# acappemin/Video-to-Audio-and-Piano-RP

Measured on AMD Instinct MI355X. Metric: mel-frames/sec (10s VGGSound shape, 32-step CFM, CFG 2.0), higher is better.
Workload: dtype bf16x3; 1 GPU; BASELINE.json configs[1]: 1 clip(s)/GPU x 750 latent frames x 128 ch, 32-point sway grid = 31 CFG evaluations (62 DiT forwards), T5 context 16 tokens, V2A zero roll; clips_per_gpu=1, global_clips=1, parallelism=clip-sharded x1, 1 all-gather, hipgraph=True, schedule=three streams, side_streams=True, cascade_passes=1

## Files before the change

include/v2a_cfm.h:

```cpp
#ifndef V2A_CFM_H
#define V2A_CFM_H

#include <stdint.h>

#ifdef __cplusplus
extern "C" {
#endif

typedef void* v2a_stream_t;

enum {
  V2A_F32 = 0,
  V2A_BF16 = 1,
  V2A_BF16_SPLIT = 2
};

enum {
  V2A_OK = 0,
  V2A_ERR_ARG = -1,
  V2A_ERR_LAUNCH = -2
};

int v2a_abi_version(void);
const char* v2a_last_error(void);

enum {
  V2A_EPI_STORE = 0,
  V2A_EPI_SIGMOID = 1,
  V2A_EPI_GEGLU = 2,
  V2A_EPI_RESID = 3,
  V2A_EPI_GATE_RESID = 4,
  V2A_EPI_GEGLU_TANH = 5,
  V2A_EPI_GELU = 6,
  V2A_EPI_SWIGLU = 7
};

typedef struct v2a_gemm_args {
  const void* a[3];
  int64_t lda[3];
  int32_t ka[3];
  int32_t nseg;
  int32_t a_dtype;
  const void* w;
  int64_t ldw;
  const float* bias;
  int32_t M, N;
  int32_t compute_dtype;
  int32_t epilogue;
  void* out;
  int64_t ldo;
  int32_t out_dtype;
  void* out_bf16;
  int64_t ld_out_bf16;
  const float* resid;
  int64_t ldr;
  const float* gate;
  const int32_t* step;
  int64_t gate_step_stride, gate_batch_stride;
  int32_t rows_per_batch;
  const float* rope_table;
  int32_t rope_cols, rope_pos_offset;
  int32_t relu;
  const int32_t* a_row_offset;
  const int32_t* a_ktile_offset;
  const int32_t* out_row_offset;
  int32_t tile_hint;
  const float* norm_gamma;
  int64_t norm_step_stride, norm_batch_stride;
  int32_t norm_switch_row, norm_switch_offset;
  float* norm_ssq;
  int64_t ld_norm_ssq;
  const float* row_ssq;
  int64_t ld_row_ssq;
  int32_t row_ssq_parts, row_norm_dim;
  int32_t out_bf16_split;
  int64_t a_lo_offset[3];
  int64_t out_bf16_lo_offset;
} v2a_gemm_args;

int v2a_gemm(const v2a_gemm_args* args, v2a_stream_t stream);
int v2a_gemm_args_size(void);

enum { V2A_GEMM_REGISTER_STAGED = 0, V2A_GEMM_RING = 1, V2A_GEMM_8PHASE = 2 };
typedef struct v2a_gemm_choice {
  int32_t family;
  int32_t split;
  int32_t bm, bn, bk;
  int32_t waves_m, waves_n;
  int32_t stages;
  int32_t tiles;
  int32_t xcd_gm, xcd_gn;
  int32_t vec_epi;
} v2a_gemm_choice;
int v2a_gemm_choose(const v2a_gemm_args* args, v2a_gemm_choice* choice);

typedef struct v2a_tuning {
  int32_t gemm_force_tile;
  int32_t gemm_k_rotation;
  int32_t gemm_8phase;
  int32_t gemm_8phase_min_tiles;
  int32_t dwconv_rows_per_wave;
  int32_t gemm_xcd_order_1x8;
  int32_t attn_one_group_from;
  int32_t reserved[1];
} v2a_tuning;
int v2a_set_tuning(const v2a_tuning* tuning);

int v2a_rmsnorm(const float* x, int64_t ldx, void* y, int64_t ldy, int32_t y_dtype,
                int64_t rows, int32_t d,
                const float* gamma, const int32_t* step, int64_t gamma_step_stride,
                int64_t gamma_batch_stride, int32_t rows_per_batch, v2a_stream_t stream);

int v2a_dwconv_silu_residual(const float* x, float* out, const float* wt, const float* bias,
                             int32_t B, int32_t N, int32_t d, int32_t ksize,
                             const int32_t* len, v2a_stream_t stream);
typedef struct v2a_dwconv_norm {
  void* out_bf16;
  int64_t ld_out_bf16;
  const float* norm_gamma;
  const int32_t* step;
  int64_t norm_step_stride, norm_batch_stride;
  float* norm_ssq;
  int64_t ld_norm_ssq;
  int32_t split;
  int32_t reserved;
} v2a_dwconv_norm;
int v2a_dwconv_silu_residual_norm(const float* x, float* out, const float* wt, const float* bias,
                                  int32_t B, int32_t N, int32_t d, int32_t ksize,
                                  const int32_t* len, const v2a_dwconv_norm* norm, v2a_stream_t stream);

int v2a_rope_inplace(void* qk, int32_t dtype, int64_t rows, int64_t row_stride, int32_t nheads,
                     int32_t rows_per_batch, int32_t pos_offset, const float* cs_table,
                     int32_t layout, v2a_stream_t stream);

typedef struct v2a_attn_args {
  const void *q, *k, *v, *gate;
  void* out;
  int64_t q_row_stride, k_row_stride, v_row_stride, gate_row_stride, out_row_stride;
  int64_t q_batch_stride, k_batch_stride, v_batch_stride, gate_batch_stride, out_batch_stride;
  int32_t B, H, Nq, Nk;
  const int32_t* kv_len;
  const int32_t* q_len;
  float scale, softclamp;
  int32_t dtype;
  int32_t out_split;
} v2a_attn_args;

int v2a_attention(const v2a_attn_args* args, v2a_stream_t stream);
int v2a_qproj_xattn(const v2a_gemm_args* gemm, const v2a_attn_args* attn, v2a_stream_t stream);

typedef struct v2a_xattn_prepare_args {
  const float* ctx_kv;
  int64_t ctx_ld;
  int32_t k_col, v_col;
  const float* wq;
  const float* wo;
  void* wqk;
  void* wvo;
  int32_t B, L, H, D, nc, KP;
} v2a_xattn_prepare_args;
int v2a_xattn_absorb_prepare(const v2a_xattn_prepare_args* args, v2a_stream_t stream);

typedef struct v2a_xattn_absorbed_args {
  const void* a;
  int64_t lda;
  int32_t K, M;
  const void* wqk;
  int64_t ldw, w_batch_stride;
  const float* gate_bias;
  void* out;
  int64_t ldo;
  int32_t rows_per_batch, B, H, KP;
  const int32_t* kv_len;
  const int32_t* q_len;
  float scale, softclamp;
  const float* row_ssq;
  int64_t ld_row_ssq;
  int32_t row_ssq_parts, row_norm_dim;
} v2a_xattn_absorbed_args;
int v2a_xattn_absorbed(const v2a_xattn_absorbed_args* args, v2a_stream_t stream);

int v2a_linear_small(const float* a, int64_t M, int32_t K, const float* wt, const float* bias,
                     const float* add, int32_t T, float* out, int64_t out_batch_stride,
                     int32_t row_off, int32_t d, int32_t dup_batch_offset,
                     const float* regs ,
                     void* out_bf16 , v2a_stream_t stream);

int v2a_fill_registers(float* out, int64_t out_batch_stride, const float* regs, int32_t B,
                       int32_t R, int32_t d, v2a_stream_t stream);

int v2a_time_cond(const float* t, int32_t S, const float* fourier_w, const float* wt,
                  const float* bias, float* out, int32_t d, v2a_stream_t stream);

int v2a_apg_reduce(const float* pred, double* apg, int32_t B, int32_t T, int32_t C,
                   int64_t pred_batch_stride, int32_t row_off,
                   const int32_t* valid_rows ,
                   v2a_stream_t stream);
int v2a_cfg_euler(float* y, const float* pred, int32_t B, int32_t T, int32_t C,
                  int64_t pred_batch_stride, int32_t row_off, float cfg_strength,
                  const float* dt, const int32_t* step, const double* apg,
                  float keep_parallel_frac, v2a_stream_t stream);
int v2a_split_bf16(const float* x, int64_t ldx, void* y, int64_t ldy, int64_t rows, int32_t d, v2a_stream_t stream);
int v2a_cast_bf16(const float* x, void* y, int64_t n, v2a_stream_t stream);
int v2a_step_advance(int32_t* step, v2a_stream_t stream);


int v2a_im2col(const float* x, int32_t B, int32_t H, int32_t W, int32_t C, int32_t kh, int32_t kw, int32_t stride,
               int32_t pad, int32_t Ho, int32_t Wo, void* col, int64_t ldo, int32_t out_dtype, int32_t window_t,
               int32_t window_first, v2a_stream_t stream);

int v2a_frames_pack(const float* frames, void* out, int32_t T, int32_t H, int32_t W, int32_t kw, int32_t stride, int32_t pad,
                    int32_t Wo, v2a_stream_t stream);
int v2a_frames_pack_split(const float* frames, void* out, int64_t lo_offset, int32_t T, int32_t H, int32_t W, int32_t kw,
                          int32_t stride, int32_t pad, int32_t Wo, v2a_stream_t stream);

int v2a_pool2d(const float* x, float* out, void* out_bf16, int32_t B, int32_t H, int32_t W, int32_t C, int32_t k,
               int32_t stride, int32_t pad, int32_t mode, int32_t Ho, int32_t Wo, int32_t in_border, int32_t out_border,
               v2a_stream_t stream);
int v2a_pool2d_split(const float* x, float* out, void* out_split, int64_t lo_offset, int32_t B, int32_t H, int32_t W, int32_t C,
                     int32_t k, int32_t stride, int32_t pad, int32_t mode, int32_t Ho, int32_t Wo, int32_t in_border,
                     int32_t out_border, v2a_stream_t stream);

typedef struct v2a_roll_head_args {
  const float *x2, *x3, *x4, *x5;
  int32_t B, P;
  const float *frb4_w1t, *frb4_b1, *frb4_w2t, *frb4_b2;
  const float *frb3_w1t, *frb3_b1, *frb3_w2t, *frb3_b2;
  const float *frb2_w1t, *frb2_b1, *frb2_w2t, *frb2_b2;
  const float *conv2_wt, *conv2_b;
  const float *fc_wt, *fc_b;
  int32_t notes;
  int32_t apply_sigmoid;
  float* out;
} v2a_roll_head_args;
int v2a_roll_head(const v2a_roll_head_args* args, v2a_stream_t stream);

int v2a_roll_expand(const float* roll, float* out, int32_t B, int32_t t, int32_t notes, int32_t rep, int32_t l,
                    v2a_stream_t stream);

int v2a_roll_expand_ratio(const float* roll, float* out, int32_t B, int32_t t, int32_t notes, int32_t rep, int32_t group, int32_t l,
                          v2a_stream_t stream);


int v2a_elu_pad(const float* x, float* out, int64_t T, int32_t C, int32_t pad, int32_t reflect, int32_t act,
                v2a_stream_t stream);

int v2a_lstm_layer(const float* gates_x, const float* w_hh, float* h, const float* resid, float* y, int32_t T, int32_t H,
                   int32_t* workspace, v2a_stream_t stream);

int v2a_lstm2(const float* gates_x0, const float* w_hh0, const float* w_ih1, const float* bias1, const float* w_hh1,
              const float* resid, float* y, int32_t T, int32_t H, int32_t* workspace, v2a_stream_t stream);


int v2a_elu_pad_lr(const float* x, float* out, int64_t T, int32_t C, int32_t pad_left, int32_t pad_right, int32_t act,
                   v2a_stream_t stream);

int v2a_encodec_stage0(const float* wave, const float* params, float* out, int64_t n, v2a_stream_t stream);


int v2a_t5_rmsnorm(const float* x, int64_t ldx, const int32_t* ids, int32_t vocab, float* resid, int64_t ldr, float* y, int64_t ldy,
                   int64_t rows, int32_t d, const float* w, float eps, v2a_stream_t stream);

typedef struct v2a_t5_attn_args {
  const float *q, *k, *v;
  float* out;
  int64_t q_row_stride, k_row_stride, v_row_stride, out_row_stride;
  int64_t q_batch_stride, k_batch_stride, v_batch_stride, out_batch_stride;
  int32_t B, H, N, d_kv;
  const float* bias;
  const int32_t* key_mask;
} v2a_t5_attn_args;
int v2a_t5_attention(const v2a_t5_attn_args* args, v2a_stream_t stream);

int v2a_gemm_skinny_f32(const v2a_gemm_args* args, v2a_stream_t stream);


int v2a_clip_resize_h(const uint8_t* frames, int32_t F, int32_t H, int32_t W, uint8_t* tmp, int32_t y0, int32_t rows, int32_t S,
                      const int32_t* bounds, const int32_t* coef, int32_t ksize, v2a_stream_t stream);
int v2a_clip_resize_v(const uint8_t* tmp, int32_t F, int32_t rows, int32_t S, int32_t P, const int32_t* bounds, const int32_t* coef,
                      int32_t ksize, const float* lut, void* patches, int64_t ldp, int32_t out_dtype, int64_t lo_offset, uint8_t* crop,
                      v2a_stream_t stream);
int v2a_clip_embed_init(float* h, int64_t ldh, int64_t rows, int32_t T, int32_t d, const float* cls, const float* pos,
                        v2a_stream_t stream);
int v2a_clip_layernorm(const float* x, int64_t ldx, void* y, int64_t ldy, int32_t y_dtype, int64_t rows, int32_t d, const float* gamma,
                       const float* beta, float eps, v2a_stream_t stream);
typedef struct v2a_clip_attn_args {
  const float *q, *k, *v;
  void* out;
  int64_t row_stride, batch_stride;
  int64_t out_row_stride, out_batch_stride;
  int32_t B, H, N, d_head;
  float scale;
  int32_t out_split;
} v2a_clip_attn_args;
int v2a_clip_attention(const v2a_clip_attn_args* args, v2a_stream_t stream);


int v2a_piano_resize_h(const uint8_t* frames, int32_t F, int32_t H, int32_t W, const int32_t* sel, int32_t n, uint8_t* tmp, int32_t ldt,
                       int32_t y0, int32_t rows, int32_t Wo, const int32_t* bounds, const int32_t* coef, int32_t ksize,
                       v2a_stream_t stream);
int v2a_piano_resize_v(const uint8_t* tmp, int32_t n, int32_t rows, int32_t ldt, int32_t Ho, int32_t Wo, const int32_t* bounds,
                       const int32_t* coef, int32_t ksize, const float* lut, float* out, v2a_stream_t stream);
int v2a_piano_resize_vt(const uint8_t* tmp, int32_t n, int32_t rows, int32_t ldt, int32_t Ho, int32_t Wo, const int32_t* bounds,
                        const int32_t* coef, int32_t ksize, const float* lut, float* out, v2a_stream_t stream);


int v2a_encodec_rvq_encode(const float* x, int64_t batch_stride, int64_t frame_stride, int64_t chan_stride, int32_t B, int32_t T,
                           const float* codebooks, const float* norms, int32_t S, int32_t Kc, int32_t D, int32_t n_q, int64_t* codes,
                           v2a_stream_t stream);
int v2a_encodec_rvq_decode(const int64_t* codes, int32_t n_q, int32_t B, int32_t T, const float* codebooks, int32_t S, int32_t Kc, int32_t D,
                           float* out, int64_t batch_stride, int64_t frame_stride, int64_t chan_stride, v2a_stream_t stream);


#define V2A_LOSS_MAX_PARTS 256

int v2a_cfm_interp(const float* x0, const float* x1, const float* t, const uint8_t* span, float* w, float* flow, float* cond, int32_t B,
                   int32_t T, int32_t C, v2a_stream_t stream);
int v2a_masked_sqerr(const float* pred, const float* target, const uint8_t* mask, int32_t B, int32_t T, int32_t C, double* scratch,
                     double* out, v2a_stream_t stream);
int v2a_roll_metrics(const float* roll, const float* midis, const uint8_t* mask, int32_t B, int32_t T, int32_t notes, double* scratch,
                     double* out, v2a_stream_t stream);


#define V2A_WAVE_MAX_PARTS 256
#define V2A_WAVE_LDS_BYTES (128 * 1024)
#define V2A_WAVE_TABLE_MAX (1 << 22)

int v2a_wave_resample(const float* x, int64_t L, const float* table, int32_t o, int32_t n, int32_t K, int32_t width, float* y,
                      int64_t out_len, void* parts, int32_t* n_parts, v2a_stream_t stream);
int v2a_wave_stats(const float* x, int64_t n, void* parts, int32_t* n_parts, v2a_stream_t stream);
int v2a_wave_normalize(const float* x, int64_t n, const void* parts, int32_t n_parts, float* out, int64_t n_out, float* stats,
                       v2a_stream_t stream);


int v2a_roll2midi_stem(const float* x, const float* wt, int32_t n, int32_t H, int32_t W, int32_t co, float* out, void* shadow,
                       int32_t shadow_mode, int64_t lo_offset, int64_t pitch, int32_t border, v2a_stream_t stream);
int v2a_leaky_shadow(float* x, void* shadow, int32_t shadow_mode, int64_t lo_offset, int32_t n, int32_t H, int32_t W, int32_t C,
                     int64_t pitch, int32_t border, v2a_stream_t stream);
int v2a_roll2midi_head(const float* u, int64_t u_pitch, int32_t nu, const float* d, int64_t d_pitch, int32_t nd, const float* w,
                       float bias, float threshold, int32_t n, int32_t H, int32_t W, int32_t border, float* logits, float* probs,
                       uint8_t* midi, v2a_stream_t stream);
int v2a_roll2midi_gate(float* x0, int64_t pitch0, int32_t C0, void* shadow0, int64_t lo_offset0, float* x1, int64_t pitch1, int32_t C1,
                       void* shadow1, int64_t lo_offset1, const float* w, float bias, int32_t shadow_mode, int32_t n, int32_t H, int32_t W,
                       int32_t border, float* logits, float* alpha, v2a_stream_t stream);


#define V2A_ROLL_NOTES_MAX_KEYS 128
#define V2A_ROLL_NOTES_TILE 256
#define V2A_ROLL_NOTES_MAX_FRAMES (1 << 24)

int v2a_roll_notes(const void* roll, int32_t elem_bytes, int64_t batch_stride, int64_t frame_stride, int64_t key_stride, float threshold,
                   int32_t B, int32_t T, int32_t keys, const int32_t* lens, int32_t* counts, int32_t* totals, int32_t* notes, int32_t cap,
                   int8_t* onset, v2a_stream_t stream);

#ifdef __cplusplus
}
#endif
#endif
```

video-to-audio-and-piano-rp_amd/_lib.py:

```python
from __future__ import annotations

import ctypes as C
import os
import subprocess
from typing import NamedTuple

import torch

_HERE = os.path.dirname(os.path.abspath(__file__))
LIB_PATH = os.path.join(_HERE, "libv2a_cfm.so")
CSRC = os.path.join(_HERE, "csrc")

F32, BF16, BF16_SPLIT = 0, 1, 2
EPI_STORE, EPI_SIGMOID, EPI_GEGLU, EPI_RESID, EPI_GATE_RESID = 0, 1, 2, 3, 4
EPI_GEGLU_TANH = 5
EPI_GELU = 6
EPI_SWIGLU = 7

_lib = None


class V2AError(RuntimeError):
    pass


class GemmArgs(C.Structure):
    _fields_ = [
        ("a", C.c_void_p * 3), ("lda", C.c_int64 * 3), ("ka", C.c_int32 * 3),
        ("nseg", C.c_int32), ("a_dtype", C.c_int32),
        ("w", C.c_void_p), ("ldw", C.c_int64), ("bias", C.c_void_p),
        ("M", C.c_int32), ("N", C.c_int32), ("compute_dtype", C.c_int32), ("epilogue", C.c_int32),
        ("out", C.c_void_p), ("ldo", C.c_int64), ("out_dtype", C.c_int32),
        ("out_bf16", C.c_void_p), ("ld_out_bf16", C.c_int64),
        ("resid", C.c_void_p), ("ldr", C.c_int64),
        ("gate", C.c_void_p), ("step", C.c_void_p),
        ("gate_step_stride", C.c_int64), ("gate_batch_stride", C.c_int64), ("rows_per_batch", C.c_int32),
        ("rope_table", C.c_void_p), ("rope_cols", C.c_int32), ("rope_pos_offset", C.c_int32), ("relu", C.c_int32),
        ("a_row_offset", C.c_void_p), ("a_ktile_offset", C.c_void_p), ("out_row_offset", C.c_void_p),
        ("tile_hint", C.c_int32),
        ("norm_gamma", C.c_void_p), ("norm_step_stride", C.c_int64), ("norm_batch_stride", C.c_int64),
        ("norm_switch_row", C.c_int32), ("norm_switch_offset", C.c_int32),
        ("norm_ssq", C.c_void_p), ("ld_norm_ssq", C.c_int64),
        ("row_ssq", C.c_void_p), ("ld_row_ssq", C.c_int64), ("row_ssq_parts", C.c_int32), ("row_norm_dim", C.c_int32),
        ("out_bf16_split", C.c_int32),
        ("a_lo_offset", C.c_int64 * 3), ("out_bf16_lo_offset", C.c_int64),
    ]


class GemmChoice(C.Structure):
    _fields_ = [(n, C.c_int32) for n in ("family", "split", "bm", "bn", "bk", "waves_m", "waves_n", "stages", "tiles", "xcd_gm", "xcd_gn",
                                         "vec_epi")]


GEMM_REGISTER_STAGED, GEMM_RING, GEMM_8PHASE = 0, 1, 2

TILE_128x128, TILE_8PHASE, TILE_128x128_8WAVES, TILE_128x64_8WAVES = 1, 6, 12, 14
SPLIT_TILE_8PHASE, SPLIT_TILE_128x256_K32 = 5, 6


class DwconvNorm(C.Structure):
    _fields_ = [("out_bf16", C.c_void_p), ("ld_out_bf16", C.c_int64), ("norm_gamma", C.c_void_p), ("step", C.c_void_p),
                ("norm_step_stride", C.c_int64), ("norm_batch_stride", C.c_int64), ("norm_ssq", C.c_void_p), ("ld_norm_ssq", C.c_int64),
                ("split", C.c_int32), ("reserved", C.c_int32)]


class Tuning(C.Structure):
    _fields_ = [("gemm_force_tile", C.c_int32), ("gemm_k_rotation", C.c_int32), ("gemm_8phase", C.c_int32),
                ("gemm_8phase_min_tiles", C.c_int32), ("dwconv_rows_per_wave", C.c_int32), ("gemm_xcd_order_1x8", C.c_int32),
                ("attn_one_group_from", C.c_int32), ("reserved", C.c_int32 * 1)]


class AttnArgs(C.Structure):
    _fields_ = [
        ("q", C.c_void_p), ("k", C.c_void_p), ("v", C.c_void_p), ("gate", C.c_void_p), ("out", C.c_void_p),
        ("q_row_stride", C.c_int64), ("k_row_stride", C.c_int64), ("v_row_stride", C.c_int64),
        ("gate_row_stride", C.c_int64), ("out_row_stride", C.c_int64),
        ("q_batch_stride", C.c_int64), ("k_batch_stride", C.c_int64), ("v_batch_stride", C.c_int64),
        ("gate_batch_stride", C.c_int64), ("out_batch_stride", C.c_int64),
        ("B", C.c_int32), ("H", C.c_int32), ("Nq", C.c_int32), ("Nk", C.c_int32),
        ("kv_len", C.c_void_p), ("q_len", C.c_void_p),
        ("scale", C.c_float), ("softclamp", C.c_float), ("dtype", C.c_int32), ("out_split", C.c_int32),
    ]


class XattnPrepareArgs(C.Structure):
    _fields_ = [("ctx_kv", C.c_void_p), ("ctx_ld", C.c_int64), ("k_col", C.c_int32), ("v_col", C.c_int32),
                ("wq", C.c_void_p), ("wo", C.c_void_p), ("wqk", C.c_void_p), ("wvo", C.c_void_p)] + \
               [(n, C.c_int32) for n in ("B", "L", "H", "D", "nc", "KP")]


class XattnAbsorbedArgs(C.Structure):
    _fields_ = [("a", C.c_void_p), ("lda", C.c_int64), ("K", C.c_int32), ("M", C.c_int32),
                ("wqk", C.c_void_p), ("ldw", C.c_int64), ("w_batch_stride", C.c_int64), ("gate_bias", C.c_void_p),
                ("out", C.c_void_p), ("ldo", C.c_int64),
                ("rows_per_batch", C.c_int32), ("B", C.c_int32), ("H", C.c_int32), ("KP", C.c_int32),
                ("kv_len", C.c_void_p), ("q_len", C.c_void_p), ("scale", C.c_float), ("softclamp", C.c_float),
                ("row_ssq", C.c_void_p), ("ld_row_ssq", C.c_int64), ("row_ssq_parts", C.c_int32), ("row_norm_dim", C.c_int32)]


class T5AttnArgs(C.Structure):
    _fields_ = [
        ("q", C.c_void_p), ("k", C.c_void_p), ("v", C.c_void_p), ("out", C.c_void_p),
        ("q_row_stride", C.c_int64), ("k_row_stride", C.c_int64), ("v_row_stride", C.c_int64), ("out_row_stride", C.c_int64),
        ("q_batch_stride", C.c_int64), ("k_batch_stride", C.c_int64), ("v_batch_stride", C.c_int64), ("out_batch_stride", C.c_int64),
        ("B", C.c_int32), ("H", C.c_int32), ("N", C.c_int32), ("d_kv", C.c_int32),
        ("bias", C.c_void_p), ("key_mask", C.c_void_p),
    ]


class ClipAttnArgs(C.Structure):
    _fields_ = [("q", C.c_void_p), ("k", C.c_void_p), ("v", C.c_void_p), ("out", C.c_void_p),
                ("row_stride", C.c_int64), ("batch_stride", C.c_int64), ("out_row_stride", C.c_int64), ("out_batch_stride", C.c_int64),
                ("B", C.c_int32), ("H", C.c_int32), ("N", C.c_int32), ("d_head", C.c_int32), ("scale", C.c_float), ("out_split", C.c_int32)]


class RollHeadArgs(C.Structure):
    _fields_ = ([(n, C.c_void_p) for n in ("x2", "x3", "x4", "x5")] + [("B", C.c_int32), ("P", C.c_int32)] +
                [(f"frb{i}_{n}", C.c_void_p) for i in (4, 3, 2) for n in ("w1t", "b1", "w2t", "b2")] +
                [(n, C.c_void_p) for n in ("conv2_wt", "conv2_b", "fc_wt", "fc_b")] +
                [("notes", C.c_int32), ("apply_sigmoid", C.c_int32), ("out", C.c_void_p)])


EXPORTS = [
    "v2a_abi_version", "v2a_last_error", "v2a_gemm", "v2a_gemm_args_size", "v2a_gemm_choose", "v2a_set_tuning", "v2a_rmsnorm", "v2a_dwconv_silu_residual", "v2a_dwconv_silu_residual_norm",
    "v2a_rope_inplace", "v2a_attention", "v2a_qproj_xattn", "v2a_linear_small", "v2a_fill_registers", "v2a_time_cond",
    "v2a_apg_reduce", "v2a_cfg_euler", "v2a_step_advance", "v2a_cast_bf16", "v2a_split_bf16",
    "v2a_im2col", "v2a_frames_pack", "v2a_pool2d", "v2a_roll_head", "v2a_roll_expand", "v2a_frames_pack_split", "v2a_pool2d_split",
    "v2a_elu_pad", "v2a_lstm_layer", "v2a_lstm2", "v2a_t5_rmsnorm", "v2a_t5_attention", "v2a_gemm_skinny_f32",
    "v2a_clip_resize_h", "v2a_clip_resize_v", "v2a_clip_embed_init", "v2a_clip_layernorm", "v2a_clip_attention",
    "v2a_elu_pad_lr", "v2a_encodec_stage0", "v2a_piano_resize_h", "v2a_piano_resize_v",
    "v2a_encodec_rvq_encode", "v2a_encodec_rvq_decode", "v2a_cfm_interp", "v2a_masked_sqerr", "v2a_roll_metrics",
    "v2a_wave_resample", "v2a_wave_stats", "v2a_wave_normalize",
    "v2a_roll2midi_stem", "v2a_leaky_shadow", "v2a_roll2midi_head", "v2a_roll2midi_gate",
    "v2a_xattn_absorb_prepare", "v2a_xattn_absorbed",
    "v2a_roll_expand_ratio", "v2a_piano_resize_vt",
    "v2a_roll_notes",
]


def build(force: bool = False, verbose: bool = False) -> str:
    if force:
        for f in os.listdir(os.path.join(CSRC, "build")) if os.path.isdir(os.path.join(CSRC, "build")) else []:
            os.remove(os.path.join(CSRC, "build", f))
    r = subprocess.run(["bash", os.path.join(CSRC, "build.sh")], capture_output=True, text=True)
    if verbose or r.returncode != 0:
        print(r.stdout[-4000:])
        print(r.stderr[-8000:])
    if r.returncode != 0:
        raise V2AError("hipcc build of libv2a_cfm.so failed")
    return LIB_PATH


ABI_VERSION = 9


def _declare(lib):
    vp, i32, i64, f32 = C.c_void_p, C.c_int32, C.c_int64, C.c_float
    lib.v2a_abi_version.restype = C.c_int
    lib.v2a_last_error.restype = C.c_char_p
    lib.v2a_gemm.argtypes = [C.POINTER(GemmArgs), vp]
    lib.v2a_gemm_args_size.restype = C.c_int
    lib.v2a_gemm_choose.argtypes = [C.POINTER(GemmArgs), C.POINTER(GemmChoice)]
    lib.v2a_set_tuning.argtypes = [C.POINTER(Tuning)]
    lib.v2a_attention.argtypes = [C.POINTER(AttnArgs), vp]
    lib.v2a_qproj_xattn.argtypes = [C.POINTER(GemmArgs), C.POINTER(AttnArgs), vp]
    lib.v2a_xattn_absorb_prepare.argtypes = [C.POINTER(XattnPrepareArgs), vp]
    lib.v2a_xattn_absorbed.argtypes = [C.POINTER(XattnAbsorbedArgs), vp]
    lib.v2a_rmsnorm.argtypes = [vp, i64, vp, i64, i32, i64, i32, vp, vp, i64, i64, i32, vp]
    lib.v2a_dwconv_silu_residual.argtypes = [vp, vp, vp, vp, i32, i32, i32, i32, vp, vp]
    lib.v2a_dwconv_silu_residual_norm.argtypes = [vp, vp, vp, vp, i32, i32, i32, i32, vp, C.POINTER(DwconvNorm), vp]
    lib.v2a_rope_inplace.argtypes = [vp, i32, i64, i64, i32, i32, i32, vp, i32, vp]
    lib.v2a_linear_small.argtypes = [vp, i64, i32, vp, vp, vp, i32, vp, i64, i32, i32, i32, vp, vp, vp]
    lib.v2a_fill_registers.argtypes = [vp, i64, vp, i32, i32, i32, vp]
    lib.v2a_time_cond.argtypes = [vp, i32, vp, vp, vp, vp, i32, vp]
    lib.v2a_apg_reduce.argtypes = [vp, vp, i32, i32, i32, i64, i32, vp, vp]
    lib.v2a_cfg_euler.argtypes = [vp, vp, i32, i32, i32, i64, i32, f32, vp, vp, vp, f32, vp]
    lib.v2a_step_advance.argtypes = [vp, vp]
    lib.v2a_cast_bf16.argtypes = [vp, vp, i64, vp]
    lib.v2a_split_bf16.argtypes = [vp, i64, vp, i64, i64, i32, vp]
    lib.v2a_im2col.argtypes = [vp, i32, i32, i32, i32, i32, i32, i32, i32, i32, i32, vp, i64, i32, i32, i32, vp]
    lib.v2a_frames_pack.argtypes = [vp, vp, i32, i32, i32, i32, i32, i32, i32, vp]
    lib.v2a_pool2d.argtypes = [vp, vp, vp, i32, i32, i32, i32, i32, i32, i32, i32, i32, i32, i32, i32, vp]
    lib.v2a_frames_pack_split.argtypes = [vp, vp, i64, i32, i32, i32, i32, i32, i32, i32, vp]
    lib.v2a_pool2d_split.argtypes = [vp, vp, vp, i64, i32, i32, i32, i32, i32, i32, i32, i32, i32, i32, i32, i32, vp]
    lib.v2a_roll_head.argtypes = [C.POINTER(RollHeadArgs), vp]
    lib.v2a_roll_expand.argtypes = [vp, vp, i32, i32, i32, i32, i32, vp]
    lib.v2a_roll_expand_ratio.argtypes = [vp, vp, i32, i32, i32, i32, i32, i32, vp]
    lib.v2a_elu_pad.argtypes = [vp, vp, i64, i32, i32, i32, i32, vp]
    lib.v2a_lstm_layer.argtypes = [vp, vp, vp, vp, vp, i32, i32, vp, vp]
    lib.v2a_lstm2.argtypes = [vp, vp, vp, vp, vp, vp, vp, i32, i32, vp, vp]
    lib.v2a_t5_rmsnorm.argtypes = [vp, i64, vp, i32, vp, i64, vp, i64, i64, i32, vp, f32, vp]
    lib.v2a_t5_attention.argtypes = [C.POINTER(T5AttnArgs), vp]
    lib.v2a_gemm_skinny_f32.argtypes = [C.POINTER(GemmArgs), vp]
    lib.v2a_clip_resize_h.argtypes = [vp, i32, i32, i32, vp, i32, i32, i32, vp, vp, i32, vp]
    lib.v2a_clip_resize_v.argtypes = [vp, i32, i32, i32, i32, vp, vp, i32, vp, vp, i64, i32, i64, vp, vp]
    lib.v2a_clip_embed_init.argtypes = [vp, i64, i64, i32, i32, vp, vp, vp]
    lib.v2a_clip_layernorm.argtypes = [vp, i64, vp, i64, i32, i64, i32, vp, vp, f32, vp]
    lib.v2a_clip_attention.argtypes = [C.POINTER(ClipAttnArgs), vp]
    lib.v2a_elu_pad_lr.argtypes = [vp, vp, i64, i32, i32, i32, i32, vp]
    lib.v2a_encodec_stage0.argtypes = [vp, vp, vp, i64, vp]
    lib.v2a_piano_resize_h.argtypes = [vp, i32, i32, i32, vp, i32, vp, i32, i32, i32, i32, vp, vp, i32, vp]
    lib.v2a_piano_resize_v.argtypes = [vp, i32, i32, i32, i32, i32, vp, vp, i32, vp, vp, vp]
    lib.v2a_piano_resize_vt.argtypes = lib.v2a_piano_resize_v.argtypes
    lib.v2a_encodec_rvq_encode.argtypes = [vp, i64, i64, i64, i32, i32, vp, vp, i32, i32, i32, i32, vp, vp]
    lib.v2a_encodec_rvq_decode.argtypes = [vp, i32, i32, i32, vp, i32, i32, i32, vp, i64, i64, i64, vp]
    lib.v2a_cfm_interp.argtypes = [vp, vp, vp, vp, vp, vp, vp, i32, i32, i32, vp]
    lib.v2a_masked_sqerr.argtypes = [vp, vp, vp, i32, i32, i32, vp, vp, vp]
    lib.v2a_roll_metrics.argtypes = [vp, vp, vp, i32, i32, i32, vp, vp, vp]
    lib.v2a_wave_resample.argtypes = [vp, i64, vp, i32, i32, i32, i32, vp, i64, vp, C.POINTER(i32), vp]
    lib.v2a_wave_stats.argtypes = [vp, i64, vp, C.POINTER(i32), vp]
    lib.v2a_wave_normalize.argtypes = [vp, i64, vp, i32, vp, i64, vp, vp]
    lib.v2a_roll2midi_stem.argtypes = [vp, vp, i32, i32, i32, i32, vp, vp, i32, i64, i64, i32, vp]
    lib.v2a_leaky_shadow.argtypes = [vp, vp, i32, i64, i32, i32, i32, i32, i64, i32, vp]
    lib.v2a_roll2midi_head.argtypes = [vp, i64, i32, vp, i64, i32, vp, f32, f32, i32, i32, i32, i32, vp, vp, vp, vp]
    lib.v2a_roll2midi_gate.argtypes = [vp, i64, i32, vp, i64, vp, i64, i32, vp, i64, vp, f32, i32, i32, i32, i32, i32, vp, vp, vp]
    lib.v2a_roll_notes.argtypes = [vp, i32, i64, i64, i64, f32, i32, i32, i32, vp, vp, vp, vp, i32, vp, vp]
    for name in EXPORTS:
        if name not in ("v2a_abi_version", "v2a_last_error", "v2a_gemm_args_size"):
            getattr(lib, name).restype = C.c_int


def lib():
    global _lib
    if _lib is None:
        if not os.path.exists(LIB_PATH):
            raise V2AError(f"{LIB_PATH} is missing: run `python -c 'import __graft_entry__ as g; g.build()'` "
                           "(hipcc --offload-arch=gfx950).  There is no CPU fallback for the sampler.")
        _lib = C.CDLL(LIB_PATH)
        _declare(_lib)
        if _lib.v2a_abi_version() != ABI_VERSION:
            raise V2AError("libv2a_cfm.so reports ABI version %d, this binding was written for %d: rebuild (csrc/build.sh)"
                           % (_lib.v2a_abi_version(), ABI_VERSION))
        if _lib.v2a_gemm_args_size() != C.sizeof(GemmArgs):
            raise V2AError("libv2a_cfm.so was built with sizeof(v2a_gemm_args) = %d, this binding mirrors %d bytes: rebuild "
                           "(csrc/build.sh)" % (_lib.v2a_gemm_args_size(), C.sizeof(GemmArgs)))
    return _lib


def set_tuning(force_tile: int = -1, k_rotation: bool = False, eight_phase: int | None = None, eight_phase_min_tiles: int = 0,
               dwconv_rows_per_wave: int = 0, xcd_order_1x8: bool = False, attn_one_group_from: int = 0, reserved: int = 0):
    if (force_tile == -1 and not k_rotation and eight_phase is None and eight_phase_min_tiles == 0 and dwconv_rows_per_wave == 0
            and not xcd_order_1x8 and attn_one_group_from == 0 and not reserved):
        check(lib().v2a_set_tuning(None))
        return
    t = Tuning(force_tile, 1 if k_rotation else 0, 1 if eight_phase is None else eight_phase, eight_phase_min_tiles, dwconv_rows_per_wave,
               1 if xcd_order_1x8 else 0, attn_one_group_from, (C.c_int32 * 1)(reserved))
    check(lib().v2a_set_tuning(C.byref(t)))


def check(rc: int):
    if rc != 0:
        raise V2AError(f"v2a_cfm call failed ({rc}): {lib().v2a_last_error().decode()}")


def stream_ptr() -> int:
    return torch.cuda.current_stream().cuda_stream


def dt_code(t: torch.dtype) -> int:
    if t == torch.float32:
        return F32
    if t == torch.bfloat16:
        return BF16
    raise V2AError(f"unsupported dtype {t}")


def _p(t):
    return 0 if t is None else t.data_ptr()


class Operand(NamedTuple):
    t: torch.Tensor
    ld: int
    k: int
    lo: int = 0


def split_planes(w):
    w = w.float()
    hi = w.bfloat16()
    return torch.cat([hi, (w - hi.float()).bfloat16()], 1)


_prof = None


class KernelProfiler:

    def __init__(self, shapes: bool = False, inner: int = 1, external: bool = False):
        self.recs = []
        self.shapes = shapes
        self.inner = inner
        self.external = external
        self.marks, self.end, self.tot = [], None, {}

    def launch(self, key, flops, nbytes, call):
        if self.external:
            e = torch.cuda.Event(enable_timing=True, external=True)
            e.record()
            self.marks.append((key, flops, nbytes, e))
            call()
            return
        n = self.inner if key.startswith("gemm") else 1
        s, e = torch.cuda.Event(enable_timing=True), torch.cuda.Event(enable_timing=True)
        s.record()
        for _ in range(n):
            call()
        e.record()
        self.recs.append((key, flops, nbytes, s, e, n))

    def close(self):
        self.end = torch.cuda.Event(enable_timing=True, external=True)
        self.end.record()

    def collect(self):
        for i, (key, flops, nbytes, e) in enumerate(self.marks):
            nxt = self.marks[i + 1][3] if i + 1 < len(self.marks) else self.end
            a = self.tot.setdefault(key, dict(launches=0, ms=0.0, flops=0.0, bytes=0.0))
            a["launches"] += 1
            a["ms"] += e.elapsed_time(nxt)
            a["flops"] += flops
            a["bytes"] += nbytes

    def summary(self):
        torch.cuda.synchronize()
        if self.external:
            return self.tot
        agg = {}
        for key, flops, nbytes, s, e, n in self.recs:
            a = agg.setdefault(key, dict(launches=0, ms=0.0, flops=0.0, bytes=0.0))
            a["launches"] += 1
            a["ms"] += s.elapsed_time(e) / n
            a["flops"] += flops
            a["bytes"] += nbytes
        return agg


def set_profiler(p):
    global _prof
    _prof = p


def _launch(key, flops, nbytes, call):
    if _prof is None:
        check(call())
    else:
        _prof.launch(key, flops, nbytes, lambda: check(call()))


_EPI_NAMES = {0: "store", 1: "sigmoid", 2: "geglu", 3: "resid", 4: "gate_resid", 5: "geglu_tanh", 6: "gelu", 7: "swiglu"}



def gemm(a_segs, w, out, **kw):
    g, key, flops, nbytes = gemm_args(a_segs, w, out, **kw)
    _launch(key, flops, nbytes, lambda: lib().v2a_gemm(C.byref(g), stream_ptr()))


def gemm_choice(a_segs, w, out, **kw) -> GemmChoice:
    c = GemmChoice()
    check(lib().v2a_gemm_choose(C.byref(gemm_args(a_segs, w, out, **kw)[0]), C.byref(c)))
    return c


def gemm_args(a_segs, w, out, *, M, N, compute, epilogue=EPI_STORE, bias=None, resid=None, gate=None,
         step=None, gate_step_stride=0, gate_batch_stride=0, rows_per_batch=0, ldo=None, ldr=None,
         out_bf16=None, ld_out_bf16=None, rope_table=None, rope_cols=0, rope_pos_offset=0, relu=False,
         a_row_offset=None, a_ktile_offset=None, out_row_offset=None, tile_hint=0,
         norm_gamma=None, norm_step_stride=0, norm_batch_stride=0, norm_switch_row=0, norm_switch_offset=0, norm_ssq=None,
         row_ssq=None, row_norm_dim=0, out_bf16_split=False, a_split=False, out_split=False, out_bf16_lo_offset=0):
    g = GemmArgs()
    a_segs = [Operand(*seg) for seg in a_segs]
    for i, s in enumerate(a_segs):
        g.a[i], g.lda[i], g.ka[i], g.a_lo_offset[i] = s.t.data_ptr(), s.ld, s.k, s.lo
    g.nseg = len(a_segs)
    g.a_dtype = BF16_SPLIT if a_split else dt_code(a_segs[0].t.dtype)
    g.w = w.data_ptr()
    g.ldw = w.stride(0)
    g.bias = _p(bias)
    g.M, g.N = M, N
    g.compute_dtype = compute
    g.epilogue = epilogue
    g.out = out.data_ptr()
    g.ldo = ldo if ldo is not None else out.stride(-2)
    g.out_dtype = BF16_SPLIT if out_split else dt_code(out.dtype)
    g.out_bf16 = _p(out_bf16)
    g.ld_out_bf16 = (ld_out_bf16 if ld_out_bf16 is not None else g.ldo) if out_bf16 is not None else 0
    g.resid = _p(resid)
    g.ldr = (ldr if ldr is not None else (resid.stride(-2) if resid is not None else 0))
    g.gate = _p(gate)
    g.step = _p(step)
    g.gate_step_stride = gate_step_stride
    g.gate_batch_stride = gate_batch_stride
    g.rows_per_batch = rows_per_batch
    g.rope_table = _p(rope_table)
    g.rope_cols, g.rope_pos_offset = rope_cols, rope_pos_offset
    g.relu = 1 if relu else 0
    g.a_row_offset, g.a_ktile_offset, g.out_row_offset = _p(a_row_offset), _p(a_ktile_offset), _p(out_row_offset)
    g.tile_hint = tile_hint if compute == BF16 and g.a_dtype in (BF16, BF16_SPLIT) and epilogue != EPI_SIGMOID else 0
    g.norm_gamma = _p(norm_gamma)
    g.norm_step_stride, g.norm_batch_stride = norm_step_stride, norm_batch_stride
    g.norm_switch_row, g.norm_switch_offset = norm_switch_row, norm_switch_offset
    g.norm_ssq = _p(norm_ssq)
    g.ld_norm_ssq = norm_ssq.stride(-2) if norm_ssq is not None else 0
    g.row_ssq = _p(row_ssq)
    g.ld_row_ssq = row_ssq.stride(-2) if row_ssq is not None else 0
    g.row_ssq_parts = row_norm_dim // 32 if row_ssq is not None else 0
    g.row_norm_dim = row_norm_dim
    g.out_bf16_split = 1 if out_bf16_split else 0
    g.out_bf16_lo_offset = out_bf16_lo_offset
    K = sum(s.k for s in a_segs)
    key = "gemm<%s,%s,%s,%s>" % ("bf16" if compute == BF16 else "f32", "a_f32" if g.a_dtype == F32 else ("a_split" if a_split else "a_bf16"),
                                 _EPI_NAMES[epilogue], "f32" if g.out_dtype == F32 else "bf16")
    esz = 2 if compute == BF16 else 4
    nbytes = M * K * (4 if g.a_dtype == F32 else 2) + N * K * esz + M * (N // 2 if epilogue in (EPI_GEGLU, EPI_SWIGLU) else N) * out.element_size()
    nbytes += (M * N * 4 if resid is not None else 0) + (M * N * 2 if out_bf16 is not None else 0)
    if g.tile_hint:
        key = key[:-1] + ",tile%d>" % (g.tile_hint - 1)
    if _prof is not None and _prof.shapes:
        key += " %dx%dx%d" % (M, N, K)
    return g, key, (6.0 if a_split else 2.0) * M * N * K, nbytes * (2 if a_split else 1)


def rmsnorm(x, y, *, rows, d, gamma, step=None, gamma_step_stride=0, gamma_batch_stride=0, rows_per_batch=0,
            ldx=None, ldy=None, split=False):
    ydt = BF16_SPLIT if split else dt_code(y.dtype)
    if split:
        ldy = ldy or 2 * d
    _launch("rmsnorm<%s>" % ("f32" if y.dtype == torch.float32 else ("bf16x2" if split else "bf16")), 0.0,
            rows * d * (4 + y.element_size() * (2 if split else 1)),
            lambda: lib().v2a_rmsnorm(x.data_ptr(), ldx or d, y.data_ptr(), ldy or d, ydt, rows, d,
                                      gamma.data_ptr(), _p(step), gamma_step_stride, gamma_batch_stride, rows_per_batch,
                                      stream_ptr()))


def _dwconv_norm(norm, d):
    n = DwconvNorm()
    n.out_bf16, n.ld_out_bf16 = norm["out_bf16"].data_ptr(), norm.get("ld_out_bf16", d)
    n.norm_gamma, n.step = norm["gamma"].data_ptr(), _p(norm.get("step"))
    n.norm_step_stride, n.norm_batch_stride = norm.get("step_stride", 0), norm.get("batch_stride", 0)
    n.norm_ssq, n.ld_norm_ssq = norm["ssq"].data_ptr(), norm["ssq"].stride(-2)
    n.split = 1 if norm.get("split") else 0
    if n.split:
        n.ld_out_bf16 = norm.get("ld_out_bf16", 2 * d)
    return n


def dwconv(x, out, wt, bias, *, B, N, d, ksize, lens=None, norm=None):
    if norm is None:
        _launch("dwconv", 2.0 * B * N * d * ksize, B * N * d * 8,
                lambda: lib().v2a_dwconv_silu_residual(x.data_ptr(), out.data_ptr(), wt.data_ptr(), bias.data_ptr(),
                                                       B, N, d, ksize, _p(lens), stream_ptr()))
        return
    n = _dwconv_norm(norm, d)
    _launch("dwconv+norm", 2.0 * B * N * d * ksize, B * N * d * (12 if n.split else 10),
            lambda: lib().v2a_dwconv_silu_residual_norm(x.data_ptr(), out.data_ptr(), wt.data_ptr(), bias.data_ptr(),
                                                        B, N, d, ksize, _p(lens), C.byref(n), stream_ptr()))


def rope(qk, *, rows, row_stride, nheads, rows_per_batch, pos_offset, table, layout):
    _launch("rope<%s>" % ("f32" if qk.dtype == torch.float32 else "bf16"), 0.0, rows * nheads * 64 * 2 * qk.element_size(),
            lambda: lib().v2a_rope_inplace(qk.data_ptr(), dt_code(qk.dtype), rows, row_stride, nheads, rows_per_batch,
                                           pos_offset, table.data_ptr(), layout, stream_ptr()))


def attention(q, k, v, gate, out, **kw):
    a, key, flops, nbytes = attention_args(q, k, v, gate, out, **kw)
    _launch(key, flops, nbytes, lambda: lib().v2a_attention(C.byref(a), stream_ptr()))


def attention_args(q, k, v, gate, out, *, strides, B, H, Nq, Nk, kv_len=None, q_len=None, scale, softclamp, dtype, out_split=False):
    a = AttnArgs()
    a.q, a.k, a.v, a.gate, a.out = q, k, v, gate, out
    (a.q_row_stride, a.k_row_stride, a.v_row_stride, a.gate_row_stride, a.out_row_stride,
     a.q_batch_stride, a.k_batch_stride, a.v_batch_stride, a.gate_batch_stride, a.out_batch_stride) = strides
    a.B, a.H, a.Nq, a.Nk = B, H, Nq, Nk
    a.kv_len, a.q_len = _p(kv_len), _p(q_len)
    a.scale, a.softclamp, a.dtype = scale, softclamp, dtype
    a.out_split = 1 if out_split else 0
    esz = 2 if dtype == BF16 else 4
    return a, "attention<%s>" % {BF16: "bf16", F32: "f32", BF16_SPLIT: "bf16x3"}[dtype], 4.0 * B * H * Nq * Nk * 64, B * H * 64 * (2 * Nq + 2 * Nk) * esz


def qproj_xattn(a, lda, K, w, *, bias, M, N, rows_per_batch, k, v, out, kv_strides, out_strides, B, H, Nk, kv_len=None, q_len=None,
                scale, softclamp, rope_table=None, rope_cols=0, rope_pos_offset=0, row_ssq=None, row_norm_dim=0, split=False):
    g = GemmArgs()
    g.a[0], g.lda[0], g.ka[0], g.nseg = a.data_ptr(), lda, K, 1
    g.compute_dtype = BF16
    g.a_dtype = BF16_SPLIT if split else BF16
    g.w, g.ldw = w.data_ptr(), w.stride(0)
    g.bias = _p(bias)
    g.M, g.N = M, N
    g.epilogue = EPI_STORE
    g.out_dtype = F32 if split else BF16
    g.rows_per_batch = rows_per_batch
    g.rope_table = _p(rope_table)
    g.rope_cols, g.rope_pos_offset = rope_cols, rope_pos_offset
    g.row_ssq = _p(row_ssq)
    g.ld_row_ssq = row_ssq.stride(-2) if row_ssq is not None else 0
    g.row_ssq_parts = row_norm_dim // 32 if row_ssq is not None else 0
    g.row_norm_dim = row_norm_dim
    t = AttnArgs()
    t.k, t.v, t.out = k, v, out
    t.k_row_stride, t.v_row_stride, t.k_batch_stride, t.v_batch_stride = kv_strides
    t.out_row_stride, t.out_batch_stride = out_strides
    t.B, t.H, t.Nq, t.Nk = B, H, rows_per_batch, Nk
    t.kv_len, t.q_len = _p(kv_len), _p(q_len)
    t.scale, t.softclamp, t.dtype = scale, softclamp, (BF16_SPLIT if split else BF16)
    t.out_split = 1 if split else 0
    _launch("qproj_xattn<%s>" % ("bf16x3" if split else "bf16"), (3.0 if split else 1.0) * (2.0 * M * (H * 65) * K + 4.0 * B * H * rows_per_batch * Nk * 64),
            M * K * 2 + H * 65 * K * 2 + M * H * 64 * 2 + 2 * B * Nk * H * 64 * 2,
            lambda: lib().v2a_qproj_xattn(C.byref(g), C.byref(t), stream_ptr()))


def xattn_kp(nc):
    return 16 if nc <= 16 else 32


def xattn_absorb_prepare(ctx_kv, wq, wo, wqk, wvo, *, B, L, H, D, nc, KP, k_col, v_col):
    a = XattnPrepareArgs()
    a.ctx_kv, a.ctx_ld, a.k_col, a.v_col = ctx_kv.data_ptr(), ctx_kv.stride(-2), k_col, v_col
    a.wq, a.wo, a.wqk, a.wvo = wq.data_ptr(), wo.data_ptr(), wqk.data_ptr(), wvo.data_ptr()
    a.B, a.L, a.H, a.D, a.nc, a.KP = B, L, H, D, nc, KP
    _launch("xattn_absorb_prepare", 4.0 * B * L * H * KP * 64 * D,
            L * (2 * H * 64 + H) * D * 4 + B * L * ((H * KP + H) * D + D * H * KP) * 4 + 2 * B * nc * L * H * 64 * 4,
            lambda: lib().v2a_xattn_absorb_prepare(C.byref(a), stream_ptr()))


def xattn_absorbed(a, lda, K, wqk, out, *, ldw, w_batch_stride, ldo, M, rows_per_batch, B, H, KP, kv_len, q_len=None, gate_bias=None,
                   scale, softclamp, row_ssq=None, row_norm_dim=0):
    g = XattnAbsorbedArgs()
    g.a, g.lda, g.K, g.M = a.data_ptr(), lda, K, M
    g.wqk, g.ldw, g.w_batch_stride, g.gate_bias = wqk.data_ptr(), ldw, w_batch_stride, _p(gate_bias)
    g.out, g.ldo = out.data_ptr(), ldo
    g.rows_per_batch, g.B, g.H, g.KP = rows_per_batch, B, H, KP
    g.kv_len, g.q_len = _p(kv_len), _p(q_len)
    g.scale, g.softclamp = scale, softclamp
    g.row_ssq = _p(row_ssq)
    g.ld_row_ssq = row_ssq.stride(-2) if row_ssq is not None else 0
    g.row_ssq_parts = row_norm_dim // 32 if row_ssq is not None else 0
    g.row_norm_dim = row_norm_dim
    n = H * KP + H
    _launch("xattn_absorbed<bf16x3>", 6.0 * M * n * K, (M * K + B * n * K + M * H * KP) * 4,
            lambda: lib().v2a_xattn_absorbed(C.byref(g), stream_ptr()))


def linear_small(a, wt, bias, add, out, *, M, K, T, out_batch_stride, row_off, d, dup=0, regs=None, out_bf16=None):
    _launch("linear_small", 2.0 * M * K * d, M * (K + d) * 4,
            lambda: lib().v2a_linear_small(a.data_ptr(), M, K, wt.data_ptr(), _p(bias), _p(add), T, out.data_ptr(),
                                           out_batch_stride, row_off, d, dup, _p(regs), _p(out_bf16), stream_ptr()))


def fill_registers(out, regs, *, B, R, d, out_batch_stride):
    check(lib().v2a_fill_registers(out.data_ptr(), out_batch_stride, regs.data_ptr(), B, R, d, stream_ptr()))


def time_cond(t, fourier_w, wt, bias, out, *, S, d):
    check(lib().v2a_time_cond(t.data_ptr(), S, fourier_w.data_ptr(), wt.data_ptr(), bias.data_ptr(),
                              out.data_ptr(), d, stream_ptr()))


def apg_reduce(pred, apg, *, B, T, C_, pred_batch_stride, row_off, valid_rows=None):
    check(lib().v2a_apg_reduce(pred.data_ptr(), apg.data_ptr(), B, T, C_, pred_batch_stride, row_off, _p(valid_rows), stream_ptr()))


def cfg_euler(y, pred, *, B, T, C_, pred_batch_stride, row_off, cfg_strength, dt, step=None, apg=None, keep=0.0):
    _launch("cfg_euler", 0.0, 16.0 * B * T * C_,
            lambda: lib().v2a_cfg_euler(y.data_ptr(), pred.data_ptr(), B, T, C_, pred_batch_stride, row_off,
                                        float(cfg_strength), dt.data_ptr(), _p(step), _p(apg), float(keep), stream_ptr()))


def step_advance(step):
    check(lib().v2a_step_advance(step.data_ptr(), stream_ptr()))


def split_bf16(x, y, *, rows, d, ldx=None, ldy=None):
    _launch("split_bf16", 0.0, rows * d * 8, lambda: lib().v2a_split_bf16(x.data_ptr(), ldx or d, y.data_ptr(), ldy or 2 * d, rows, d, stream_ptr()))


def cast_bf16(x, y):
    _launch("cast_bf16", 0.0, x.numel() * 6, lambda: lib().v2a_cast_bf16(x.data_ptr(), y.data_ptr(), x.numel(), stream_ptr()))


def im2col(x, col, *, B, H, W, C_, kh, kw, stride, pad, Ho, Wo, ldo, window_t=0, window_first=0):
    K = kh * kw * C_
    _launch("im2col<%s>" % ("f32" if col.dtype == torch.float32 else "bf16"), 0.0, B * Ho * Wo * (4.0 * K + col.element_size() * ldo),
            lambda: lib().v2a_im2col(x.data_ptr(), B, H, W, C_, kh, kw, stride, pad, Ho, Wo, col.data_ptr(), ldo,
                                     dt_code(col.dtype), window_t, window_first, stream_ptr()))


def frames_pack(frames, out, *, T, H, W, kw, stride, pad, Wo):
    _launch("frames_pack", 0.0, 4.0 * T * H * W + 32.0 * (T + 4) * Wo * (H + 2 * pad),
            lambda: lib().v2a_frames_pack(frames.data_ptr(), out.data_ptr(), T, H, W, kw, stride, pad, Wo, stream_ptr()))


def frames_pack_split(frames, out, *, lo_offset, T, H, W, kw, stride, pad, Wo):
    _launch("frames_pack_split", 0.0, 4.0 * T * H * W + 64.0 * (T + 4) * Wo * (H + 2 * pad),
            lambda: lib().v2a_frames_pack_split(frames.data_ptr(), out.data_ptr(), lo_offset, T, H, W, kw, stride, pad, Wo, stream_ptr()))


def pool2d(x, out, *, B, H, W, C_, k, stride, pad, mode, Ho, Wo, out_bf16=None, in_border=0, out_border=0):
    _launch("pool2d", 0.0, 4.0 * B * C_ * (H * W + Ho * Wo),
            lambda: lib().v2a_pool2d(x.data_ptr(), out.data_ptr(), _p(out_bf16), B, H, W, C_, k, stride, pad, mode, Ho, Wo,
                                     in_border, out_border, stream_ptr()))


def pool2d_split(x, out, out_split, *, lo_offset, B, H, W, C_, k, stride, pad, mode, Ho, Wo, in_border=0, out_border=0):
    _launch("pool2d_split", 0.0, 4.0 * B * C_ * (H * W + 2 * Ho * Wo),
            lambda: lib().v2a_pool2d_split(x.data_ptr(), out.data_ptr(), out_split.data_ptr(), lo_offset, B, H, W, C_, k, stride, pad,
                                           mode, Ho, Wo, in_border, out_border, stream_ptr()))


def roll_head(args: "RollHeadArgs"):
    _launch("roll_head", 0.0, 4.0 * args.B * args.P * (3 * 128 + 64), lambda: lib().v2a_roll_head(C.byref(args), stream_ptr()))


def roll_expand(roll, out, *, B, t, notes, rep, l):
    check(lib().v2a_roll_expand(roll.data_ptr(), out.data_ptr(), B, t, notes, rep, l, stream_ptr()))


def roll_expand_ratio(roll, out, *, B, t, notes, rep, group, l):
    check(lib().v2a_roll_expand_ratio(roll.data_ptr(), out.data_ptr(), B, t, notes, rep, group, l, stream_ptr()))


SH_NONE, SH_BF16, SH_SPLIT = 0, 1, 2


def roll2midi_stem(x, wt, out, shadow, *, n, H, W, co, shadow_mode, lo_offset, pitch, border):
    _launch("roll2midi_stem", 18.0 * n * H * W * co, n * H * W * (4.0 + co * (4 + 2 * shadow_mode)),
            lambda: lib().v2a_roll2midi_stem(x.data_ptr(), wt.data_ptr(), n, H, W, co, out.data_ptr(), _p(shadow), shadow_mode, lo_offset,
                                             pitch, border, stream_ptr()))


def leaky_shadow(x, shadow, *, n, H, W, C_, shadow_mode, lo_offset, pitch, border):
    _launch("leaky_shadow", 0.0, n * H * W * C_ * (8.0 + 2 * shadow_mode),
            lambda: lib().v2a_leaky_shadow(x.data_ptr(), _p(shadow), shadow_mode, lo_offset, n, H, W, C_, pitch, border, stream_ptr()))


def roll2midi_head(u, d, w, *, u_pitch, nu, d_pitch, nd, bias, threshold, n, H, W, border, logits=None, probs=None, midi=None):
    _launch("roll2midi_head", 2.0 * n * H * W * (nu + nd), n * H * W * (4.0 * (nu + nd) + 9),
            lambda: lib().v2a_roll2midi_head(u.data_ptr(), u_pitch, nu, d.data_ptr(), d_pitch, nd, w.data_ptr(), float(bias), float(threshold),
                                             n, H, W, border, _p(logits), _p(probs), _p(midi), stream_ptr()))


def roll2midi_gate(seg0, seg1, w, *, bias, shadow_mode, n, H, W, border, logits=None, alpha=None):
    x0, p0, c0, s0, l0 = seg0
    x1, p1, c1, s1, l1 = seg1 if seg1 is not None else (None, 0, 0, None, 0)
    _launch("roll2midi_gate", 2.0 * n * H * W * (c0 + c1), n * H * W * (c0 + c1) * (8.0 + 2 * shadow_mode) + 4.0 * (c0 + c1),
            lambda: lib().v2a_roll2midi_gate(x0.data_ptr(), p0, c0, _p(s0), l0, _p(x1), p1, c1, _p(s1), l1, w.data_ptr(), float(bias),
                                             shadow_mode, n, H, W, border, _p(logits), _p(alpha), stream_ptr()))


ROLL_NOTES_MAX_KEYS, ROLL_NOTES_TILE, ROLL_NOTES_MAX_FRAMES = 128, 256, 1 << 24


def roll_notes(roll, counts, totals, notes, *, strides, B, T, keys, cap, threshold=0.0, lens=None, onset=None):
    _launch("roll_notes<%s>" % ("f32" if roll.dtype == torch.float32 else "u8"), 0.0, 2.0 * B * T * keys * roll.element_size(),
            lambda: lib().v2a_roll_notes(roll.data_ptr(), roll.element_size(), strides[0], strides[1], strides[2], float(threshold), B, T, keys,
                                         _p(lens), counts.data_ptr(), totals.data_ptr(), _p(notes), cap, _p(onset), stream_ptr()))


def elu_pad(x, out, *, T, C_, pad, reflect, act=True):
    _launch("elu_pad", 0.0, 4.0 * C_ * (2 * T + pad),
            lambda: lib().v2a_elu_pad(x.data_ptr(), out.data_ptr(), T, C_, pad, 1 if reflect else 0, 1 if act else 0, stream_ptr()))


def elu_pad_lr(x, out, *, T, C_, pad_left, pad_right, act=True):
    _launch("elu_pad_lr", 0.0, 4.0 * C_ * (2 * T + pad_left + pad_right),
            lambda: lib().v2a_elu_pad_lr(x.data_ptr(), out.data_ptr(), T, C_, pad_left, pad_right, 1 if act else 0, stream_ptr()))


ENCODEC_STAGE0_PARAMS = 3376


def encodec_stage0(wave, params, out, *, n):
    _launch("encodec_stage0", 2.0 * n * 3744, 4.0 * n * 33,
            lambda: lib().v2a_encodec_stage0(wave.data_ptr(), params.data_ptr(), out.data_ptr(), n, stream_ptr()))


def encodec_rvq_encode(x, strides, codebooks, norms, codes, *, B, T, n_q):
    S, Kc, D = codebooks.shape
    _launch("encodec_rvq_encode", 2.0 * B * T * n_q * Kc * D, 4.0 * (B * T * D + n_q * Kc * D * -(-B * T // 16)) + 8.0 * n_q * B * T,
            lambda: lib().v2a_encodec_rvq_encode(x.data_ptr(), strides[0], strides[1], strides[2], B, T, codebooks.data_ptr(), norms.data_ptr(),
                                                 S, Kc, D, n_q, codes.data_ptr(), stream_ptr()))


def encodec_rvq_decode(codes, codebooks, out, strides, *, B, T, n_q):
    S, Kc, D = codebooks.shape
    _launch("encodec_rvq_decode", 1.0 * B * T * n_q * D, B * T * (4.0 * D * (n_q + 1) + 8.0 * n_q),
            lambda: lib().v2a_encodec_rvq_decode(codes.data_ptr(), n_q, B, T, codebooks.data_ptr(), S, Kc, D, out.data_ptr(),
                                                 strides[0], strides[1], strides[2], stream_ptr()))


LOSS_MAX_PARTS = 256


def cfm_interp(x0, x1, t, span, w, flow, cond=None):
    B, T, C_ = x1.shape
    _launch("cfm_interp", 4.0 * B * T * C_, 4.0 * B * T * C_ * (4 if cond is None else 5),
            lambda: lib().v2a_cfm_interp(x0.data_ptr(), x1.data_ptr(), t.data_ptr(), _p(span), w.data_ptr(), flow.data_ptr(), _p(cond),
                                         B, T, C_, stream_ptr()))


def masked_sqerr(pred, target, mask, out):
    B, T, C_ = pred.shape
    scratch = torch.empty(LOSS_MAX_PARTS * 2, dtype=torch.float64, device=pred.device)
    _launch("masked_sqerr", 3.0 * B * T * C_, 8.0 * B * T * C_,
            lambda: lib().v2a_masked_sqerr(pred.data_ptr(), target.data_ptr(), mask.data_ptr(), B, T, C_, scratch.data_ptr(), out.data_ptr(),
                                           stream_ptr()))


def roll_metrics(roll, midis, mask, out):
    B, T, notes = roll.shape
    scratch = torch.empty(LOSS_MAX_PARTS * 6, dtype=torch.float64, device=roll.device)
    _launch("roll_metrics", 5.0 * B * T * notes, 16.0 * B * T * notes,
            lambda: lib().v2a_roll_metrics(roll.data_ptr(), midis.data_ptr(), mask.data_ptr(), B, T, notes, scratch.data_ptr(), out.data_ptr(),
                                           stream_ptr()))


def lstm_layer(gates_x, w_hh, h, workspace, *, T, H, resid=None, y=None):
    _launch("lstm_layer", 2.0 * T * 4 * H * H, 4.0 * T * 6 * H,
            lambda: lib().v2a_lstm_layer(gates_x.data_ptr(), w_hh.data_ptr(), h.data_ptr(), _p(resid), _p(y), T, H,
                                         workspace.data_ptr(), stream_ptr()))


def lstm2(gates_x0, w_hh0, w_ih1, bias1, w_hh1, y, workspace, *, T, H, resid=None):
    _launch("lstm2", 2.0 * T * 4 * H * H * 3, 4.0 * T * 6 * H,
            lambda: lib().v2a_lstm2(gates_x0.data_ptr(), w_hh0.data_ptr(), w_ih1.data_ptr(), bias1.data_ptr(), w_hh1.data_ptr(),
                                    _p(resid), y.data_ptr(), T, H, workspace.data_ptr(), stream_ptr()))


def t5_rmsnorm(x, y, w, *, rows, d, eps, ids=None, vocab=0, resid=None, ldx=None, ldy=None):
    _launch("t5_rmsnorm%s" % ("+gather" if ids is not None else ""), 0.0, rows * d * (12 if ids is not None else 8),
            lambda: lib().v2a_t5_rmsnorm(x.data_ptr(), ldx or d, _p(ids), vocab, _p(resid), d, y.data_ptr(), ldy or d, rows, d,
                                         w.data_ptr(), float(eps), stream_ptr()))


def t5_attention(qkv, out, bias, key_mask, *, B, H, N, inner):
    a = T5AttnArgs()
    base, ld = qkv.data_ptr(), qkv.stride(0)
    a.q, a.k, a.v, a.out = base, base + 4 * inner, base + 8 * inner, out.data_ptr()
    a.q_row_stride = a.k_row_stride = a.v_row_stride = ld
    a.out_row_stride = out.stride(0)
    a.q_batch_stride = a.k_batch_stride = a.v_batch_stride = N * ld
    a.out_batch_stride = N * out.stride(0)
    a.B, a.H, a.N, a.d_kv = B, H, N, 64
    a.bias, a.key_mask = bias.data_ptr(), key_mask.data_ptr()
    _launch("t5_attention", 4.0 * B * H * N * N * 64, 4.0 * B * N * (4 * inner),
            lambda: lib().v2a_t5_attention(C.byref(a), stream_ptr()))


def gemm_skinny(a, w, out, *, M, N, K, epilogue=EPI_STORE, resid=None, bias=None):
    g = GemmArgs()
    g.a[0], g.lda[0], g.ka[0], g.nseg = a.data_ptr(), a.stride(0), K, 1
    g.a_dtype = g.compute_dtype = g.out_dtype = F32
    g.w, g.ldw = w.data_ptr(), w.stride(0)
    g.bias = _p(bias)
    g.M, g.N, g.epilogue = M, N, epilogue
    g.out, g.ldo = out.data_ptr(), out.stride(0)
    g.resid, g.ldr = _p(resid), (resid.stride(0) if resid is not None else 0)
    key = "gemm_skinny<f32,%s>" % _EPI_NAMES[epilogue]
    if _prof is not None and _prof.shapes:
        key += " %dx%dx%d" % (M, N, K)
    nbytes = 4.0 * (M * K + N * K + M * (N // 2 if epilogue == EPI_GEGLU_TANH else N) * (2 if resid is not None else 1))
    _launch(key, 2.0 * M * N * K, nbytes, lambda: lib().v2a_gemm_skinny_f32(C.byref(g), stream_ptr()))
```

video-to-audio-and-piano-rp_amd/csrc/rowops.hip:

```cpp
#include "v2a_common.h"
#include <utility>

namespace v2a_detail { extern int g_dwconv_rows_per_wave; extern int g_dwconv_stream; }

thread_local char v2a_err_buf[512] = {0};

extern "C" int v2a_abi_version(void) { return 9; }
extern "C" const char* v2a_last_error(void) { return v2a_err_buf; }

namespace {

template <typename OutT, int VPL , bool SPLIT = false >
__global__ __launch_bounds__(256) void rmsnorm_kernel(const float* __restrict__ x, int64_t ldx, OutT* __restrict__ y,
                                                      int64_t ldy, int64_t rows, int d, const float* gamma,
                                                      const int32_t* step, int64_t gss, int64_t gbs, int rpb) {
  const int lane = threadIdx.x & 63;
  const int64_t row = (int64_t)blockIdx.x * 4 + (threadIdx.x >> 6);
  if (row >= rows) return;
  const float* xr = x + row * ldx;
  const float* g = step_vec(gamma, step, gss, gbs, row / rpb);
  const int nvec = d >> 2;
  f32x4 v[VPL];
  float ss = 0.f;
#pragma unroll
// ... 182 lines not shown
                                                        int B, int N, int d, const int32_t* len, int P, int walkers, v2a_dwconv_norm nrm) {
  const int CB = gridDim.x;
  const int flat = blockIdx.y * CB + blockIdx.x;
  const int xcd = flat & 7, slot = flat >> 3;
  const int cblk = slot % CB, walker = slot / CB;
  dwconv_body<KS, TN, NORM>(x, out, wt, bias, B, N, d, len, P, walkers, nrm, xcd, cblk, walker);
}

template <int KS, bool NORM, int NCW>
__global__ __launch_bounds__(64 * (NCW + 1)) void dwconv_stream_kernel(const float* __restrict__ x, float* __restrict__ out,
                                                            const float* __restrict__ wt, const float* __restrict__ bias,
                                                            int B, int N, int d, const int32_t* len, int SEG, int nseg, int CB,
                                                            v2a_dwconv_norm nrm) {
  constexpr int TO = 16 / NCW;
  constexpr int HALF = KS / 2, CH = 16, RING_ROWS = 128, WIN = TO + KS - 1;
  constexpr int KR = 24;
  static_assert(HALF < CH && WIN <= 3 * CH, "window must fit three chunks");
  extern __shared__ __attribute__((aligned(16))) char ring[];
  char* tapl = ring + RING_ROWS * 1024;
  const int lane = threadIdx.x & 63;
  const int wave = __builtin_amdgcn_readfirstlane(threadIdx.x >> 6);
  int item = blockIdx.x;
  const int cblk = item % CB;
  item /= CB;
  const int seg = item % nseg, b = item / nseg;
  const int p0 = seg * SEG, p1 = min(p0 + SEG, N);
  const int nch = (p1 - p0 + CH - 1) / CH;
  const int w0 = p0 - CH;
  const int c4 = cblk * 64 + lane;
  const bool cok = c4 * 4 < d;
  const int cc = cok ? c4 : d / 4 - 1;
  const int L = len ? min(len[b], N) : N;
  const float* xb = x + (int64_t)b * N * d;

  if (wave == NCW) {
    const uint32_t loff = (uint32_t)cc * 16u;
    auto issue = [&](int j) {
#pragma unroll
      for (int r = 0; r < CH; ++r) {
        int row = w0 + CH * j + r;
        row = row < 0 ? 0 : (row >= N ? N - 1 : row);
        const char* src = reinterpret_cast<const char*>(xb + (int64_t)row * d) + loff;
        __builtin_amdgcn_global_load_lds((const __attribute__((address_space(1))) void*)src,
                                         (__attribute__((address_space(3))) void*)(ring + (((CH * j + r) & (RING_ROWS - 1)) << 10)), 16, 0, 0);
      }
    };
    const int last = nch + 1;
    issue(0);
    issue(1);
    issue(2);
    asm volatile("s_waitcnt vmcnt(0)" ::: "memory");
    __builtin_amdgcn_s_barrier();
    for (int j = 3; j <= 5; ++j)
      if (j <= last) issue(j);
    for (int i = 1; i < nch; ++i) {
      if (i + 4 <= last) asm volatile("s_waitcnt vmcnt(32)" ::: "memory");
      else asm volatile("s_waitcnt vmcnt(0)" ::: "memory");
      __builtin_amdgcn_s_barrier();
      if (i + 5 <= last) issue(i + 5);
    }
    return;
  }

  for (int k = KR + wave; k < KS; k += NCW)
    *reinterpret_cast<f32x4*>(tapl + (k - KR) * 1024 + lane * 16) = *reinterpret_cast<const f32x4*>(wt + (int64_t)k * d + 4 * cc);
  f32x4 tap[KR];
#pragma unroll
  for (int k = 0; k < KR; ++k) tap[k] = *reinterpret_cast<const f32x4*>(wt + (int64_t)k * d + 4 * cc);
  const f32x4 bv = *reinterpret_cast<const f32x4*>(bias + 4 * cc);
  const float* gmp = NORM ? step_vec(nrm.norm_gamma, nrm.step, nrm.norm_step_stride, nrm.norm_batch_stride, b) + 4 * cc : nullptr;
  float* ob = out + (int64_t)b * N * d;
  const char* lbase = ring + lane * 16;
  const char* tbase = tapl + lane * 16;
  asm volatile("s_waitcnt lgkmcnt(0)" ::: "memory");
  for (int i = 0; i < nch; ++i) {
    __builtin_amdgcn_s_barrier();
    const int q0 = p0 + CH * i + TO * wave;
    const int r0 = q0 - HALF;
    const int rr0 = r0 - w0;
    f32x4 acc[TO];
#pragma unroll
    for (int t = 0; t < TO; ++t) acc[t] = bv;
    auto fma_row = [&](auto jc, const f32x4& v) {
      constexpr int j = decltype(jc)::value;
#pragma unroll
      for (int t = 0; t < TO; ++t) {
        constexpr int dummy = 0; (void)dummy;
        const int k = j - t;
        if (k >= 0 && k < KS) {
          const f32x4 w = k < KR ? tap[k < KR ? k : 0] : *reinterpret_cast<const f32x4*>(tbase + ((k < KR ? 0 : k - KR) << 10));
          acc[t] = w * v + acc[t];
        }
      }
    };
    if (r0 >= 0 && r0 + WIN <= L) {
      constexpr int RB = 8;
      auto batch = [&](auto b0c) {
        constexpr int B0 = decltype(b0c)::value;
        f32x4 v[RB];
        [&]<int... U>(std::integer_sequence<int, U...>) {
          ((B0 + U < WIN ? (void)(v[U] = *reinterpret_cast<const f32x4*>(lbase + (((rr0 + B0 + U) & (RING_ROWS - 1)) << 10))) : (void)0), ...);
        }(std::make_integer_sequence<int, RB>{});
        __builtin_amdgcn_sched_barrier(0);
        [&]<int... U>(std::integer_sequence<int, U...>) {
          ((B0 + U < WIN ? fma_row(std::integral_constant<int, (B0 + U < WIN ? B0 + U : 0)>{}, v[U]) : (void)0), ...);
        }(std::make_integer_sequence<int, RB>{});
        __builtin_amdgcn_sched_barrier(0);
      };
      [&]<int... Bk>(std::integer_sequence<int, Bk...>) {
        (batch(std::integral_constant<int, Bk * RB>{}), ...);
      }(std::make_integer_sequence<int, (WIN + RB - 1) / RB>{});
    } else {
      [&]<int... J>(std::integer_sequence<int, J...>) {
        ((r0 + J >= 0 && r0 + J < L
              ? fma_row(std::integral_constant<int, J>{}, *reinterpret_cast<const f32x4*>(lbase + (((rr0 + J) & (RING_ROWS - 1)) << 10)))
              : (void)0), ...);
      }(std::make_integer_sequence<int, WIN>{});
    }
    if (cok) {
      f32x4 gm = {1.f, 1.f, 1.f, 1.f};
      if constexpr (NORM) gm = *reinterpret_cast<const f32x4*>(gmp);
#pragma unroll
      for (int t = 0; t < TO; ++t) {
        const int n = q0 + t;
        if (n < p1) {
          f32x4 o = *reinterpret_cast<const f32x4*>(lbase + (((rr0 + HALF + t) & (RING_ROWS - 1)) << 10));
          if (n < L) {
#pragma unroll
            for (int e = 0; e < 4; ++e) o[e] += acc[t][e] * __builtin_amdgcn_rcpf(1.0f + __expf(-acc[t][e]));
          }
          *reinterpret_cast<f32x4*>(ob + (int64_t)n * d + 4 * cc) = o;
          if constexpr (NORM) {
            const int64_t row = (int64_t)b * N + n;
            bf16x4 obf;
#pragma unroll
            for (int e = 0; e < 4; ++e) obf[e] = (bf16_t)(o[e] * gm[e]);
            *reinterpret_cast<bf16x4*>(reinterpret_cast<bf16_t*>(nrm.out_bf16) + row * nrm.ld_out_bf16 + 4 * cc) = obf;
            if (nrm.split) {
              bf16x4 ol;
#pragma unroll
              for (int e = 0; e < 4; ++e) ol[e] = (bf16_t)(o[e] * gm[e] - (float)obf[e]);
              *reinterpret_cast<bf16x4*>(reinterpret_cast<bf16_t*>(nrm.out_bf16) + row * nrm.ld_out_bf16 + d + 4 * cc) = ol;
            }
            const float ss = octet_sum(o[0] * o[0] + o[1] * o[1] + o[2] * o[2] + o[3] * o[3]);
            if ((lane & 7) == 0) nrm.norm_ssq[row * nrm.ld_norm_ssq + (cc >> 3)] = ss;
          }
        }
      }
    }
  }
}

template <typename T>
__global__ __launch_bounds__(256) void rope_kernel(T* __restrict__ qk, int64_t rows, int64_t row_stride, int nheads,
                                                   int rpb, int pos_offset, const float* __restrict__ cs, int layout) {
  const int64_t idx = (int64_t)blockIdx.x * blockDim.x + threadIdx.x;
  const int64_t per_row = (int64_t)nheads * 8;
  if (idx >= rows * per_row) return;
  const int64_t row = idx / per_row;
  const int rem = (int)(idx % per_row);
  const int head = rem >> 3, quad = rem & 7;
  const int pos = pos_offset + (int)(row % rpb);
  T* base = qk + row * row_stride + head * 64;
  const float* c = cs + ((int64_t)pos * 32 + quad * 4) * 2;
  float a[4], b[4];
  if (layout == 0) {
#pragma unroll
    for (int i = 0; i < 4; ++i) {
      a[i] = to_f32(base[quad * 8 + 2 * i]);
      b[i] = to_f32(base[quad * 8 + 2 * i + 1]);
    }
  } else {
#pragma unroll
    for (int i = 0; i < 4; ++i) {
      a[i] = to_f32(base[quad * 4 + i]);
      b[i] = to_f32(base[32 + quad * 4 + i]);
    }
  }
#pragma unroll
  for (int i = 0; i < 4; ++i) {
    const float co = c[2 * i], si = c[2 * i + 1];
    const float ra = a[i] * co - b[i] * si;
    const float rb = b[i] * co + a[i] * si;
    a[i] = ra;
    b[i] = rb;
  }
  if (layout == 0) {
#pragma unroll
    for (int i = 0; i < 4; ++i) {
      base[quad * 8 + 2 * i] = from_f32<T>(a[i]);
      base[quad * 8 + 2 * i + 1] = from_f32<T>(b[i]);
    }
  } else {
#pragma unroll
    for (int i = 0; i < 4; ++i) {
      base[quad * 4 + i] = from_f32<T>(a[i]);
      base[32 + quad * 4 + i] = from_f32<T>(b[i]);
    }
  }
}

template <int ROWS>
__global__ __launch_bounds__(256) void linear_small_kernel(const float* __restrict__ a, int K, const float* __restrict__ wt,
                                                           const float* __restrict__ bias, const float* __restrict__ add,
                                                           int T, float* __restrict__ out, int64_t obs, int row_off, int d,
                                                           int dup, const float* __restrict__ regs, bf16_t* __restrict__ out2) {
  extern __shared__ __attribute__((aligned(16))) char smem_raw[];
  typedef float f32x2 __attribute__((ext_vector_type(2)));
  f32x2* as = reinterpret_cast<f32x2*>(smem_raw);
  const int b = blockIdx.y;
  const int fill = regs ? row_off : 0;
  const int rr0 = blockIdx.x * ROWS;
  for (int i = threadIdx.x; i < ROWS * K; i += blockDim.x) {
    const int t = rr0 + i / K - fill;
    const float v = (t >= 0 && t < T) ? a[((int64_t)b * T + t) * K + (i % K)] : 0.f;
    as[i] = f32x2{v, v};
  }
  __syncthreads();
  for (int n = threadIdx.x * 4; n < d; n += blockDim.x * 4) {
    f32x2 acc2[ROWS][2];
#pragma unroll
    for (int r = 0; r < ROWS; ++r) acc2[r][0] = acc2[r][1] = f32x2{0.f, 0.f};
#pragma unroll 8
    for (int k = 0; k < K; ++k) {
      const f32x4 w = *reinterpret_cast<const f32x4*>(wt + (int64_t)k * d + n);
      const f32x2 w0 = {w[0], w[1]}, w1 = {w[2], w[3]};
#pragma unroll
      for (int r = 0; r < ROWS; ++r) {
        const f32x2 aa = as[r * K + k];
        acc2[r][0] += aa * w0;
        acc2[r][1] += aa * w1;
      }
    }
    f32x4 acc[ROWS];
#pragma unroll
    for (int r = 0; r < ROWS; ++r) acc[r] = f32x4{acc2[r][0][0], acc2[r][0][1], acc2[r][1][0], acc2[r][1][1]};
    f32x4 bv = {0.f, 0.f, 0.f, 0.f};
    if (bias) bv = *reinterpret_cast<const f32x4*>(bias + n);
#pragma unroll
    for (int r = 0; r < ROWS; ++r) {
      const int rr = rr0 + r;
      if (rr >= fill + T) break;
      f32x4 v;
      int orow;
      if (rr < fill) {
        v = *reinterpret_cast<const f32x4*>(regs + (int64_t)rr * d + n);
        orow = rr;
      } else {
        const int t = rr - fill;
        v = acc[r];
#pragma unroll
        for (int e = 0; e < 4; ++e) v[e] += bv[e];
        if (add) {
          const f32x4 ad = *reinterpret_cast<const f32x4*>(add + (int64_t)t * d + n);
#pragma unroll
          for (int e = 0; e < 4; ++e) v[e] += ad[e];
        }
        orow = row_off + t;
      }
      bf16x4 o2;
#pragma unroll
      for (int e = 0; e < 4; ++e) o2[e] = (bf16_t)v[e];
      for (int h = 0; h < (dup > 0 ? 2 : 1); ++h) {
        const int64_t off = (int64_t)(b + h * dup) * obs + (int64_t)orow * d + n;
        *reinterpret_cast<f32x4*>(out + off) = v;
        if (out2) *reinterpret_cast<bf16x4*>(out2 + off) = o2;
      }
    }
  }
}

__global__ void fill_registers_kernel(float* __restrict__ out, int64_t obs, const float* __restrict__ regs, int B, int R,
                                      int d) {
  const int64_t idx = (int64_t)blockIdx.x * blockDim.x + threadIdx.x;
  const int64_t per = (int64_t)R * d;
  if (idx >= per * B) return;
  const int64_t b = idx / per, r = idx % per;
  out[b * obs + r] = regs[r];
}

__global__ __launch_bounds__(256) void time_cond_kernel(const float* __restrict__ t, const float* __restrict__ fw,
                                                        const float* __restrict__ wt, const float* __restrict__ bias,
                                                        float* __restrict__ out, int d) {
  extern __shared__ __attribute__((aligned(16))) char smem_raw[];
  float* e = reinterpret_cast<float*>(smem_raw);
  const int s = blockIdx.x;
  const float ts = t[s];
  const int half = d / 2;
  if (threadIdx.x == 0) e[0] = ts;
  for (int i = threadIdx.x; i < half; i += blockDim.x) {
    const float f = ts * fw[i] * 2.0f * 3.14159265358979323846f;
    e[1 + i] = sinf(f);
    e[1 + half + i] = cosf(f);
  }
  __syncthreads();
  const int n = blockIdx.y * blockDim.x + threadIdx.x;
  if (n >= d) return;
  float acc = bias[n];
#pragma unroll 8
  for (int k = 0; k < d + 1; ++k) acc += e[k] * wt[(int64_t)k * d + n];
  out[(int64_t)s * d + n] = silu_f(acc);
}

__global__ __launch_bounds__(256) void cfg_euler_kernel(float* __restrict__ y, const float* __restrict__ pred, int B,
                                                        int T, int C, int64_t pbs, int row_off, float s,
                                                        const float* __restrict__ dt, const int32_t* step,
                                                        const double* apg, float keep) {
  const int64_t idx4 = (int64_t)blockIdx.x * blockDim.x + threadIdx.x;
  const int64_t per_b = (int64_t)T * C;
  const int64_t total4 = (int64_t)B * per_b / 4;
  if (idx4 >= total4) return;
  const int64_t e = idx4 * 4;
  const int64_t b = e / per_b, r = e % per_b;
  const float h = dt[step ? step[0] : 0];
  const f32x4 pc = *reinterpret_cast<const f32x4*>(pred + b * pbs + (int64_t)row_off * C + r);
  const f32x4 pn = *reinterpret_cast<const f32x4*>(pred + (b + B) * pbs + (int64_t)row_off * C + r);
  f32x4 yv = *reinterpret_cast<const f32x4*>(y + e);
  float coef = 0.f;
  if (apg) {
    const double dot = apg[2 * b], nn = apg[2 * b + 1];
    const double nrm = sqrt(nn) > 1e-12 ? sqrt(nn) : 1e-12;
    coef = (float)(dot / (nrm * nrm));
  }
#pragma unroll
  for (int j = 0; j < 4; ++j) {
    float upd = pc[j] - pn[j];
    if (apg) {
      const float par = coef * pc[j];
      upd = (upd - par) + par * keep;
    }
    yv[j] += h * (pc[j] + upd * s);
  }
  *reinterpret_cast<f32x4*>(y + e) = yv;
}

__global__ __launch_bounds__(256) void apg_reduce_kernel(const float* __restrict__ pred, double* __restrict__ apg, int B,
                                                         int T, int C, int64_t pbs, int row_off, const int32_t* __restrict__ valid_rows) {
  const int b = blockIdx.y;
  int rows = T;
  if (valid_rows) rows = min(T, max(0, valid_rows[0]));
  const int64_t per_b = (int64_t)rows * C;
  double dot = 0.0, nn = 0.0;
  const float* pc = pred + (int64_t)b * pbs + (int64_t)row_off * C;
  const float* pn = pred + (int64_t)(b + B) * pbs + (int64_t)row_off * C;
  for (int64_t i = (int64_t)blockIdx.x * blockDim.x + threadIdx.x; i < per_b; i += (int64_t)gridDim.x * blockDim.x) {
    const double c = pc[i], n = pn[i];
    dot += (c - n) * c;
    nn += c * c;
  }
  __shared__ double sd[256], sn[256];
  sd[threadIdx.x] = dot;
  sn[threadIdx.x] = nn;
  __syncthreads();
  for (int o = 128; o > 0; o >>= 1) {
    if (threadIdx.x < o) {
      sd[threadIdx.x] += sd[threadIdx.x + o];
      sn[threadIdx.x] += sn[threadIdx.x + o];
    }
    __syncthreads();
  }
  if (threadIdx.x == 0) {
    atomicAdd(&apg[2 * b], sd[0]);
    atomicAdd(&apg[2 * b + 1], sn[0]);
  }
}

__global__ void step_advance_kernel(int32_t* step) { step[0] += 1; }

__global__ __launch_bounds__(256) void split_bf16_kernel(const float* __restrict__ x, int64_t ldx, bf16_t* __restrict__ y, int64_t ldy,
                                                         int64_t rows, int d) {
  const int64_t i = (int64_t)blockIdx.x * blockDim.x + threadIdx.x;
  const int per = d >> 2;
  if (i >= rows * per) return;
  const int64_t r = i / per;
  const int c = (int)(i % per) * 4;
  const f32x4 v = *reinterpret_cast<const f32x4*>(x + r * ldx + c);
  bf16x4 hi, lo;
#pragma unroll
  for (int j = 0; j < 4; ++j) {
    hi[j] = (bf16_t)v[j];
    lo[j] = (bf16_t)(v[j] - (float)hi[j]);
  }
  *reinterpret_cast<bf16x4*>(y + r * ldy + c) = hi;
  *reinterpret_cast<bf16x4*>(y + r * ldy + d + c) = lo;
}

__global__ __launch_bounds__(256) void cast_bf16_kernel(const float* __restrict__ x, bf16_t* __restrict__ y, int64_t n4) {
  const int64_t i = (int64_t)blockIdx.x * blockDim.x + threadIdx.x;
  if (i >= n4) return;
  const f32x4 v = *reinterpret_cast<const f32x4*>(x + 4 * i);
  bf16x4 o;
#pragma unroll
  for (int j = 0; j < 4; ++j) o[j] = (bf16_t)v[j];
  *reinterpret_cast<bf16x4*>(y + 4 * i) = o;
}

}

extern "C" int v2a_rmsnorm(const float* x, int64_t ldx, void* y, int64_t ldy, int32_t y_dtype, int64_t rows, int32_t d,
                           const float* gamma, const int32_t* step, int64_t gss, int64_t gbs, int32_t rpb,
                           v2a_stream_t stream) {
  V2A_REQUIRE(x && y && gamma, "v2a_rmsnorm: null pointer");
  V2A_REQUIRE(rows > 0 && d > 0 && d % 4 == 0 && d <= 2048, "v2a_rmsnorm: d=%d (need d %% 4 == 0, d <= 2048)", d);
  V2A_REQUIRE(ldx % 4 == 0 && ldy % 4 == 0 && gss % 4 == 0 && gbs % 4 == 0, "v2a_rmsnorm: strides must be multiples of 4");
  V2A_REQUIRE(y_dtype == V2A_F32 || y_dtype == V2A_BF16 || y_dtype == V2A_BF16_SPLIT, "v2a_rmsnorm: y dtype %d", y_dtype);
  V2A_REQUIRE(y_dtype != V2A_BF16_SPLIT || ldy >= 2 * (int64_t)d, "v2a_rmsnorm: split output needs ldy >= 2*d");
  if (rpb <= 0) rpb = (int32_t)rows;
  hipStream_t s = (hipStream_t)stream;
  const dim3 grid((unsigned)((rows + 3) / 4)), block(256);
  const int vpl = (d / 4 + 63) / 64;
#define V2A_RMS(OT, V) \
  hipLaunchKernelGGL((rmsnorm_kernel<OT, V>), grid, block, 0, s, x, ldx, (OT*)y, ldy, rows, d, gamma, step, gss, gbs, rpb)
  if (y_dtype == V2A_BF16_SPLIT) {
#define V2A_RMS_S(V) hipLaunchKernelGGL((rmsnorm_kernel<bf16_t, V, true>), grid, block, 0, s, x, ldx, (bf16_t*)y, ldy, rows, d, gamma, step, gss, gbs, rpb)
    if (vpl <= 1) V2A_RMS_S(1); else if (vpl <= 2) V2A_RMS_S(2); else if (vpl <= 3) V2A_RMS_S(3); else if (vpl <= 4) V2A_RMS_S(4);
    else if (vpl <= 5) V2A_RMS_S(5); else if (vpl <= 6) V2A_RMS_S(6); else V2A_RMS_S(8);
#undef V2A_RMS_S
  } else if (y_dtype == V2A_F32) {
    if (vpl <= 1) V2A_RMS(float, 1); else if (vpl <= 2) V2A_RMS(float, 2); else if (vpl <= 3) V2A_RMS(float, 3); else if (vpl <= 4) V2A_RMS(float, 4);
    else if (vpl <= 5) V2A_RMS(float, 5); else if (vpl <= 6) V2A_RMS(float, 6); else V2A_RMS(float, 8);
  } else {
    if (vpl <= 1) V2A_RMS(bf16_t, 1); else if (vpl <= 2) V2A_RMS(bf16_t, 2); else if (vpl <= 3) V2A_RMS(bf16_t, 3); else if (vpl <= 4) V2A_RMS(bf16_t, 4);
    else if (vpl <= 5) V2A_RMS(bf16_t, 5); else if (vpl <= 6) V2A_RMS(bf16_t, 6); else V2A_RMS(bf16_t, 8);
  }
#undef V2A_RMS
  return v2a_check_launch("v2a_rmsnorm");
}

static int dwconv_launch(const float* x, float* out, const float* wt, const float* bias, int32_t B, int32_t N, int32_t d, int32_t ksize,
                         const int32_t* len, const v2a_dwconv_norm* norm, v2a_stream_t stream) {
  V2A_REQUIRE(x && out && wt && bias, "v2a_dwconv: null pointer");
  V2A_REQUIRE(x != out, "v2a_dwconv: out must not alias x (halo reads)");
  V2A_REQUIRE(ksize == 31, "v2a_dwconv: kernel_size %d (only 31 is built, x3:726)", ksize);
  V2A_REQUIRE(d % 4 == 0 && B > 0 && N > 0, "v2a_dwconv: B=%d N=%d d=%d", B, N, d);
  if (norm)
    V2A_REQUIRE(norm->out_bf16 && norm->norm_gamma && norm->norm_ssq && d % 32 == 0 && norm->ld_out_bf16 % 4 == 0 && norm->ld_out_bf16 >= d &&
                    ((uintptr_t)norm->out_bf16 & 7) == 0 && ((uintptr_t)norm->norm_gamma & 15) == 0 && norm->norm_step_stride % 4 == 0 &&
                    norm->norm_batch_stride % 4 == 0 && norm->ld_norm_ssq >= d / 32 && (!norm->split || norm->ld_out_bf16 >= 2 * (int64_t)d),
                "v2a_dwconv: the folded norm needs out_bf16, norm_gamma, norm_ssq, d %% 32 == 0 (d=%d) and aligned rows", d);
  const int cb = (d / 4 + 63) / 64;
  hipStream_t s = (hipStream_t)stream;
  {
    int nseg = (256 + B * cb - 1) / (B * cb);
    nseg = nseg < 1 ? 1 : nseg;
    int SEG = ((N + nseg - 1) / nseg + 15) / 16 * 16;
    if (SEG < 96) SEG = 96;
    nseg = (N + SEG - 1) / SEG;
    const int64_t blocks = (int64_t)B * cb * nseg;
    const int64_t rounds = (blocks + 255) / 256;
    if (v2a_detail::g_dwconv_stream && blocks >= 192 && blocks * 100 >= rounds * 256 * 97 && SEG <= 256) {
      const v2a_dwconv_norm none{};
      constexpr size_t smem = (128 + 31 - 24) * 1024;
      if (norm) {
        static std::atomic<uint64_t> lds_set{0};
        if (int rc = v2a_enable_lds(reinterpret_cast<const void*>(dwconv_stream_kernel<31, true, 8>), smem, lds_set, "v2a_dwconv(stream)")) return rc;
        hipLaunchKernelGGL((dwconv_stream_kernel<31, true, 8>), dim3((unsigned)blocks), dim3(576), smem, s, x, out, wt, bias, B, N, d, len, SEG, nseg, cb, *norm);
      } else {
        static std::atomic<uint64_t> lds_set{0};
        if (int rc = v2a_enable_lds(reinterpret_cast<const void*>(dwconv_stream_kernel<31, false, 8>), smem, lds_set, "v2a_dwconv(stream)")) return rc;
        hipLaunchKernelGGL((dwconv_stream_kernel<31, false, 8>), dim3((unsigned)blocks), dim3(576), smem, s, x, out, wt, bias, B, N, d, len, SEG, nseg, cb, none);
      }
      return v2a_check_launch("v2a_dwconv_silu_residual(stream)");
    }
  }
  const int TN = norm ? 4 : v2a_detail::g_dwconv_rows_per_wave;
  const int P = (N + 4 * TN - 1) / (4 * TN);
  const int items = P * B, ipx = (items + 7) / 8;
  const int cap = max(1, (TN == 4 ? 3 : 2) * 256 / 8 / cb);
  const int rounds = (ipx + cap - 1) / cap;
  const int walkers = (ipx + rounds - 1) / rounds;
  V2A_REQUIRE(walkers >= 1 && (int64_t)walkers * 8 <= 65535 && (int64_t)walkers * rounds * 8 >= items,
              "v2a_dwconv: grid does not cover the work (items=%d walkers=%d rounds=%d)", items, walkers, rounds);
  dim3 grid(cb, walkers * 8), block(256);
  const v2a_dwconv_norm none{};
  auto launchable = [&](const void* kern, std::atomic<uint64_t>& done, const char* what) -> int {
    int dev = 0;
    if (hipGetDevice(&dev) != hipSuccess) dev = 0;
    const uint64_t bit = 1ull << (dev & 63);
    if (done.load(std::memory_order_acquire) & bit) return V2A_OK;
    hipFuncAttributes fa{};
    const hipError_t e = hipFuncGetAttributes(&fa, kern);
    if (e != hipSuccess) return v2a_fail(V2A_ERR_LAUNCH, "v2a_dwconv(%s): hipFuncGetAttributes: %s", what, hipGetErrorString(e));
    if (fa.maxThreadsPerBlock < 256 || fa.sharedSizeBytes > 64 * 1024)
      return v2a_fail(V2A_ERR_ARG, "v2a_dwconv(%s): kernel variant not launchable with 256 threads (max threads %d, %d VGPRs, %zu bytes of LDS)", what,
                      fa.maxThreadsPerBlock, fa.numRegs, (size_t)fa.sharedSizeBytes);
    done.fetch_or(bit, std::memory_order_release);
    return V2A_OK;
  };
  if (norm) {
    static std::atomic<uint64_t> ok{0};
    if (int rc = launchable(reinterpret_cast<const void*>(dwconv_kernel<31, 4, true>), ok, "rows 4, folded norm")) return rc;
    hipLaunchKernelGGL((dwconv_kernel<31, 4, true>), grid, block, 0, s, x, out, wt, bias, B, N, d, len, P, walkers, *norm);
  } else if (TN == 6) {
    static std::atomic<uint64_t> ok{0};
    if (int rc = launchable(reinterpret_cast<const void*>(dwconv_kernel<31, 6, false>), ok, "rows 6")) return rc;
    hipLaunchKernelGGL((dwconv_kernel<31, 6, false>), grid, block, 0, s, x, out, wt, bias, B, N, d, len, P, walkers, none);
  } else {
    static std::atomic<uint64_t> ok{0};
    if (int rc = launchable(reinterpret_cast<const void*>(dwconv_kernel<31, 4, false>), ok, "rows 4")) return rc;
    hipLaunchKernelGGL((dwconv_kernel<31, 4, false>), grid, block, 0, s, x, out, wt, bias, B, N, d, len, P, walkers, none);
  }
  return v2a_check_launch("v2a_dwconv_silu_residual");
}

extern "C" int v2a_dwconv_silu_residual(const float* x, float* out, const float* wt, const float* bias, int32_t B,
                                        int32_t N, int32_t d, int32_t ksize, const int32_t* len, v2a_stream_t stream) {
  return dwconv_launch(x, out, wt, bias, B, N, d, ksize, len, nullptr, stream);
}

extern "C" int v2a_dwconv_silu_residual_norm(const float* x, float* out, const float* wt, const float* bias, int32_t B, int32_t N, int32_t d,
                                             int32_t ksize, const int32_t* len, const v2a_dwconv_norm* norm, v2a_stream_t stream) {
  V2A_REQUIRE(norm != nullptr, "v2a_dwconv_silu_residual_norm: null norm arguments");
  return dwconv_launch(x, out, wt, bias, B, N, d, ksize, len, norm, stream);
}

extern "C" int v2a_rope_inplace(void* qk, int32_t dtype, int64_t rows, int64_t row_stride, int32_t nheads,
                                int32_t rpb, int32_t pos_offset, const float* cs, int32_t layout, v2a_stream_t stream) {
  V2A_REQUIRE(qk && cs, "v2a_rope: null pointer");
  V2A_REQUIRE(rows > 0 && nheads > 0 && rpb > 0, "v2a_rope: rows=%lld nheads=%d rpb=%d", (long long)rows, nheads, rpb);
  V2A_REQUIRE(layout == 0 || layout == 1, "v2a_rope: layout %d", layout);
  const int64_t total = rows * nheads * 8;
  dim3 grid((unsigned)((total + 255) / 256)), block(256);
  hipStream_t s = (hipStream_t)stream;
  if (dtype == V2A_F32)
    hipLaunchKernelGGL((rope_kernel<float>), grid, block, 0, s, (float*)qk, rows, row_stride, nheads, rpb, pos_offset, cs, layout);
  else if (dtype == V2A_BF16)
    hipLaunchKernelGGL((rope_kernel<bf16_t>), grid, block, 0, s, (bf16_t*)qk, rows, row_stride, nheads, rpb, pos_offset, cs, layout);
  else
    return v2a_fail(V2A_ERR_ARG, "v2a_rope: dtype %d", dtype);
  return v2a_check_launch("v2a_rope_inplace");
}

extern "C" int v2a_linear_small(const float* a, int64_t M, int32_t K, const float* wt, const float* bias,
                                const float* add, int32_t T, float* out, int64_t obs, int32_t row_off, int32_t d,
                                int32_t dup, const float* regs, void* out_bf16, v2a_stream_t stream) {
  V2A_REQUIRE(a && wt && out, "v2a_linear_small: null pointer");
  V2A_REQUIRE(M > 0 && K > 0 && K <= 2048 && T > 0 && d > 0 && d % 4 == 0 && M % T == 0, "v2a_linear_small: M=%lld K=%d T=%d d=%d",
              (long long)M, K, T, d);
  V2A_REQUIRE(obs % 4 == 0 && (((uintptr_t)out | (uintptr_t)wt | (uintptr_t)bias | (uintptr_t)add | (uintptr_t)regs) & 15) == 0 &&
                  ((uintptr_t)out_bf16 & 7) == 0, "v2a_linear_small: 16-byte alignment");
  const int rows = (regs ? row_off : 0) + T;
  const int64_t nb8 = (int64_t)((rows + 7) / 8) * (M / T);
  if (nb8 >= 512) {
    const size_t smem = 2 * 8 * (size_t)K * sizeof(float);
    if (smem > 64 * 1024) {
      static std::atomic<uint64_t> lds_set{0};
      if (int rc = v2a_enable_lds(reinterpret_cast<const void*>(linear_small_kernel<8>), 2 * 8 * 2048 * sizeof(float), lds_set, "v2a_linear_small")) return rc;
    }
    dim3 grid((unsigned)((rows + 7) / 8), (unsigned)(M / T)), block(256);
    hipLaunchKernelGGL((linear_small_kernel<8>), grid, block, smem, (hipStream_t)stream, a, K, wt, bias, add,
                       T, out, obs, row_off, d, dup, regs, (bf16_t*)out_bf16);
  } else {
    dim3 grid((unsigned)((rows + 1) / 2), (unsigned)(M / T)), block(256);
    hipLaunchKernelGGL((linear_small_kernel<2>), grid, block, 2 * 2 * K * sizeof(float), (hipStream_t)stream, a, K, wt, bias, add,
                       T, out, obs, row_off, d, dup, regs, (bf16_t*)out_bf16);
  }
  return v2a_check_launch("v2a_linear_small");
}

extern "C" int v2a_fill_registers(float* out, int64_t obs, const float* regs, int32_t B, int32_t R, int32_t d,
                                  v2a_stream_t stream) {
  V2A_REQUIRE(out && regs && B > 0 && R > 0 && d > 0, "v2a_fill_registers: bad args");
  const int64_t total = (int64_t)B * R * d;
  hipLaunchKernelGGL(fill_registers_kernel, dim3((unsigned)((total + 255) / 256)), dim3(256), 0, (hipStream_t)stream, out,
                     obs, regs, B, R, d);
  return v2a_check_launch("v2a_fill_registers");
}

extern "C" int v2a_time_cond(const float* t, int32_t S, const float* fw, const float* wt, const float* bias, float* out,
                             int32_t d, v2a_stream_t stream) {
  V2A_REQUIRE(t && fw && wt && bias && out, "v2a_time_cond: null pointer");
  V2A_REQUIRE(S > 0 && d > 0 && d % 2 == 0, "v2a_time_cond: S=%d d=%d", S, d);
  hipLaunchKernelGGL(time_cond_kernel, dim3(S, (d + 255) / 256), dim3(256), (d + 1) * sizeof(float), (hipStream_t)stream, t, fw,
                     wt, bias, out, d);
  return v2a_check_launch("v2a_time_cond");
}

extern "C" int v2a_apg_reduce(const float* pred, double* apg, int32_t B, int32_t T, int32_t C, int64_t pbs,
                              int32_t row_off, const int32_t* valid_rows, v2a_stream_t stream) {
  V2A_REQUIRE(pred && apg && B > 0 && T > 0 && C > 0, "v2a_apg_reduce: bad args");
  hipStream_t s = (hipStream_t)stream;
  hipError_t e = hipMemsetAsync(apg, 0, sizeof(double) * 2 * B, s);
  if (e != hipSuccess) return v2a_fail(V2A_ERR_LAUNCH, "v2a_apg_reduce memset: %s", hipGetErrorString(e));
  const int64_t per_b = (int64_t)T * C;
  int chunks = (int)((per_b + 256 * 8 - 1) / (256 * 8));
  if (chunks > 64) chunks = 64;
  hipLaunchKernelGGL(apg_reduce_kernel, dim3(chunks, B), dim3(256), 0, s, pred, apg, B, T, C, pbs, row_off, valid_rows);
  return v2a_check_launch("v2a_apg_reduce");
}

extern "C" int v2a_cfg_euler(float* y, const float* pred, int32_t B, int32_t T, int32_t C, int64_t pbs, int32_t row_off,
                             float cfg_strength, const float* dt, const int32_t* step, const double* apg, float keep,
                             v2a_stream_t stream) {
  V2A_REQUIRE(y && pred && dt, "v2a_cfg_euler: null pointer");
  V2A_REQUIRE(B > 0 && T > 0 && C > 0 && C % 4 == 0 && pbs % 4 == 0, "v2a_cfg_euler: B=%d T=%d C=%d", B, T, C);
  const int64_t total4 = (int64_t)B * T * C / 4;
  hipLaunchKernelGGL(cfg_euler_kernel, dim3((unsigned)((total4 + 255) / 256)), dim3(256), 0, (hipStream_t)stream, y, pred,
                     B, T, C, pbs, row_off, cfg_strength, dt, step, apg, keep);
  return v2a_check_launch("v2a_cfg_euler");
}

extern "C" int v2a_step_advance(int32_t* step, v2a_stream_t stream) {
  V2A_REQUIRE(step, "v2a_step_advance: null pointer");
  hipLaunchKernelGGL(step_advance_kernel, dim3(1), dim3(1), 0, (hipStream_t)stream, step);
  return v2a_check_launch("v2a_step_advance");
}

extern "C" int v2a_split_bf16(const float* x, int64_t ldx, void* y, int64_t ldy, int64_t rows, int32_t d, v2a_stream_t stream) {
  V2A_REQUIRE(x && y && rows > 0 && d > 0 && d % 4 == 0, "v2a_split_bf16: bad args (d %% 4 must be 0)");
  V2A_REQUIRE(ldx % 4 == 0 && ldy % 4 == 0 && ldy >= 2 * (int64_t)d && ((uintptr_t)x & 15) == 0 && ((uintptr_t)y & 7) == 0,
              "v2a_split_bf16: strides / alignment (ldy >= 2*d)");
  const int64_t n4 = rows * (d / 4);
  hipLaunchKernelGGL(split_bf16_kernel, dim3((unsigned)((n4 + 255) / 256)), dim3(256), 0, (hipStream_t)stream, x, ldx, (bf16_t*)y, ldy, rows, d);
  return v2a_check_launch("v2a_split_bf16");
}

extern "C" int v2a_cast_bf16(const float* x, void* y, int64_t n, v2a_stream_t stream) {
  V2A_REQUIRE(x && y && n > 0 && n % 4 == 0, "v2a_cast_bf16: bad args (n %% 4 must be 0)");
  hipLaunchKernelGGL(cast_bf16_kernel, dim3((unsigned)((n / 4 + 255) / 256)), dim3(256), 0, (hipStream_t)stream, x, (bf16_t*)y, n / 4);
  return v2a_check_launch("v2a_cast_bf16");
}
```

video-to-audio-and-piano-rp_amd/dit.py:

```python
from __future__ import annotations

import math
import os
from collections import OrderedDict
from dataclasses import dataclass, asdict
from typing import NamedTuple

import torch

from . import _lib as L

NOTES = 51


@dataclass
class DiTConfig:
    dim: int = 1024
    dim_text: int = 1280
    dim_frames: int = 512
    depth: int = 12
    heads: int = 16
    dim_head: int = 64
    frames_heads: int = 8
    ff_mult: int = 4
    kernel_size: int = 31
    num_registers: int = 32
    num_channels: int = 128
    notes: int = NOTES
    max_seq_len: int = 8192
    dim_context: int | None = None
    cond_proj_in: bool = False

    @property
    def ctx_dim(self):
        return self.dim if self.dim_context is None else self.dim_context

    def to_dict(self):
        return asdict(self)


def _ru(x, m):
    return (x + m - 1) // m * m


class _Stream(NamedTuple):
    x: torch.Tensor
    sh: L.Operand | None

    @property
    def op(self):
        return self.sh if self.sh is not None else L.Operand(self.x, self.x.shape[-1], self.x.shape[-1])


class _Wide(NamedTuple):
    whole: L.Operand
    x: L.Operand
    skip: L.Operand


def pack_weight(w, dev, cd, split=False):
    if not split:
        return w.float().to(dev, cd).contiguous()
    return L.split_planes(w).contiguous().to(dev)


class _Attn:

    def __init__(self, sd, prefix, dim, heads, dh, cd, dev, cross=False, split=False):
        inner = heads * dh
        wq, wk, wv = sd[f"{prefix}.to_q.weight"], sd[f"{prefix}.to_k.weight"], sd[f"{prefix}.to_v.weight"]
        wg, bg = sd[f"{prefix}.to_v_head_gate.weight"], sd[f"{prefix}.to_v_head_gate.bias"]
        self.heads, self.inner = heads, inner
        parts = [wq, wg] if cross else [wq, wk, wv, wg]
        n = sum(p.shape[0] for p in parts)
        self.n_pad = _ru(n, 16)
        w = torch.zeros(self.n_pad, dim, dtype=torch.float32)
        w[:n] = torch.cat([p.float() for p in parts], 0)
        b = torch.zeros(self.n_pad, dtype=torch.float32)
        self.gate_col = n - heads
        b[self.gate_col:n] = bg.float()
        self.w_in = pack_weight(w, dev, cd, split)
        self.b_in = b.to(dev)
        self.w_out = pack_weight(sd[f"{prefix}.to_out.weight"], dev, cd, split)
        self.wk, self.wv = (wk, wv) if cross else (None, None)
        self.wq32, self.wo32 = (torch.cat([wq.float(), wg.float()], 0), sd[f"{prefix}.to_out.weight"].float()) if cross and split else (None, None)


class _FF:

    def __init__(self, sd, prefix, dim, cd, dev, split=False):
        w1, b1 = sd[f"{prefix}.ff.0.proj.weight"].float(), sd[f"{prefix}.ff.0.proj.bias"].float()
        inner = w1.shape[0] // 2
        assert inner % 16 == 0
        self.inner = inner
        wv, wg = w1[:inner].reshape(inner // 16, 1, 16, dim), w1[inner:].reshape(inner // 16, 1, 16, dim)
        self.w1 = pack_weight(torch.cat([wv, wg], 1).reshape(2 * inner, dim), dev, cd, split)
        bv, bgt = b1[:inner].reshape(inner // 16, 1, 16), b1[inner:].reshape(inner // 16, 1, 16)
        self.b1 = torch.cat([bv, bgt], 1).reshape(2 * inner).to(dev).contiguous()
        self.w2 = pack_weight(sd[f"{prefix}.ff.2.weight"], dev, cd, split)
        self.b2 = sd[f"{prefix}.ff.2.bias"].float().to(dev).contiguous()


class _Conv:
    def __init__(self, sd, prefix, dev):
        w = sd[f"{prefix}.dw_conv1d.0.weight"].float()
        self.k = w.shape[-1]
        self.wt = w[:, 0, :].t().contiguous().to(dev)
        self.b = sd[f"{prefix}.dw_conv1d.0.bias"].float().to(dev).contiguous()


class PackedWeights:

    def __init__(self, cfg: DiTConfig, sd: dict, dev, cd: torch.dtype, split: bool = False):
        c = cfg
        pk = lambda w: pack_weight(w, dev, cd, split)
        T = "transformer"
        f32 = lambda k: sd[k].float().to(dev).contiguous()
        self.pos_emb = f32(f"{T}.abs_pos_emb.weight")
        self.regs = f32(f"{T}.registers")
        self.text_regs = f32(f"{T}.text_registers")
        self.frames_regs = f32(f"{T}.frames_registers")
        self.fourier_w = f32(f"{T}.time_cond_mlp.0.weights")
        self.time_wt = sd[f"{T}.time_cond_mlp.1.weight"].float().t().contiguous().to(dev)
        self.time_b = f32(f"{T}.time_cond_mlp.1.bias")
        self.final_g = f32(f"{T}.final_norm.g")
        self.pin_wt = sd["proj_in.weight"].float().t().contiguous().to(dev)
        self.pin_b = f32("proj_in.bias")
        self.pf_wt = sd["proj_frames.weight"].float().t().contiguous().to(dev)
        self.pf_b = f32("proj_frames.bias")
        self.pred_w = pk(sd["to_pred.weight"])
        self.pred_b = f32("to_pred.bias")
        if c.cond_proj_in:
            wc = sd["cond_proj_in.weight"].float()
            self.cond_k = _ru(c.num_channels, 64)
            wp = torch.zeros(wc.shape[0], self.cond_k)
            wp[:, :c.num_channels] = wc
            self.cond_w = pk(wp)
            self.cond_b = (sd["cond_proj_in.bias"].float() if "cond_proj_in.bias" in sd else torch.zeros(wc.shape[0])).to(dev).contiguous()
        self.layers = []
        ng, gw, gb, kw, vw = [], [], [], [], []
        for i in range(c.depth):
            P = f"{T}.layers.{i}"
            ly = {}
            if i >= c.depth // 2:
                ly["skip"] = pk(sd[f"{P}.0.0.weight"])
                if cd == torch.bfloat16:
                    ws = sd[f"{P}.0.0.weight"].double()
                    w1 = sd[f"{P}.1.5.text_frames_to_audio.weight"].double()
                    wsx, wss = ws[:, :c.dim], ws[:, c.dim:]
                    fused = torch.cat([wsx @ w1[:, :c.dim] + wsx, wss, wsx @ w1[:, c.dim:c.dim + c.dim_text], wsx @ w1[:, c.dim + c.dim_text:]], 1)
                    ly["x_skip"] = pk(fused.float())
            ly["a_conv"] = _Conv(sd, f"{P}.0.1", dev)
            ly["a_attn"] = _Attn(sd, f"{P}.0.3", c.dim, c.heads, c.dim_head, cd, dev, split=split)
            ly["a_attn2"] = _Attn(sd, f"{P}.0.6", c.dim, c.heads, c.dim_head, cd, dev, cross=True, split=split)
            ly["a_ff"] = _FF(sd, f"{P}.0.9", c.dim, cd, dev, split)
            ng += [sd[f"{P}.0.2.to_gamma.weight"], sd[f"{P}.0.5.to_gamma.weight"], sd[f"{P}.0.8.to_gamma.weight"]]
            gw += [sd[f"{P}.0.4.to_gamma.weight"], sd[f"{P}.0.7.to_gamma.weight"], sd[f"{P}.0.10.to_gamma.weight"]]
            gb += [sd[f"{P}.0.4.to_gamma.bias"], sd[f"{P}.0.7.to_gamma.bias"], sd[f"{P}.0.10.to_gamma.bias"]]
            kw.append(ly["a_attn2"].wk)
            vw.append(ly["a_attn2"].wv)
            ly["t_conv"] = _Conv(sd, f"{P}.1.0", dev)
            ly["t_g1"] = f32(f"{P}.1.1.g")
            ly["t_attn"] = _Attn(sd, f"{P}.1.2", c.dim_text, c.heads, c.dim_head, cd, dev, split=split)
            ly["t_g2"] = f32(f"{P}.1.3.g")
            ly["t_ff"] = _FF(sd, f"{P}.1.4", c.dim_text, cd, dev, split)
            ly["x_tfa"] = pk(sd[f"{P}.1.5.text_frames_to_audio.weight"])
            if i != c.depth - 1:
                ly["x_at"] = pk(sd[f"{P}.1.5.audio_to_text.weight"])
                ly["x_af"] = pk(sd[f"{P}.1.5.audio_to_frames.weight"])
            ly["f_conv"] = _Conv(sd, f"{P}.2.0", dev)
            ly["f_g1"] = f32(f"{P}.2.1.g")
            ly["f_attn"] = _Attn(sd, f"{P}.2.2", c.dim_frames, c.frames_heads, c.dim_head, cd, dev, split=split)
            ly["f_g2"] = f32(f"{P}.2.3.g")
            ly["f_ff"] = _FF(sd, f"{P}.2.4", c.dim_frames, cd, dev, split)
            self.layers.append(ly)
        self.norm_gamma_w = torch.cat([w.float() for w in ng], 0).to(dev).contiguous()
        self.norm_gamma_b = torch.ones(self.norm_gamma_w.shape[0], device=dev)
        self.gate_w = torch.cat([w.float() for w in gw], 0).to(dev).contiguous()
        self.gate_b = torch.cat([b.float() for b in gb], 0).to(dev).contiguous()
        self.ctx_kv_w = pk(torch.cat([w.float() for w in kw] + [w.float() for w in vw], 0))
        self.xattn_wq = self.xattn_wo = None
        if split:
            self.xattn_wq = torch.stack([ly["a_attn2"].wq32 for ly in self.layers]).to(dev).contiguous()
            self.xattn_wo = torch.stack([ly["a_attn2"].wo32 for ly in self.layers]).to(dev).contiguous()
        for ly in self.layers:
            ly["a_attn2"].wk = ly["a_attn2"].wv = ly["a_attn2"].wq32 = ly["a_attn2"].wo32 = None


SHIPPED_WIDTHS = (1024, 1280, 512, 4)
_R2, _R3 = "profiles/r02 A/B runs (DESIGN.md appendix A, `scripts/gpu_ci.sh sidetiles`)", "profiles/r03_tile_sweep.txt"
_R5 = "profiles/r05_bf16x3_tile_sweeps.txt"
_W8, _NARROW, _PH8 = L.TILE_128x128_8WAVES, L.TILE_128x64_8WAVES, L.TILE_8PHASE
_S_PH8, _S_FAT = L.SPLIT_TILE_8PHASE, L.SPLIT_TILE_128x256_K32
TUNED_TILES = {
    ("bf16", 0, SHIPPED_WIDTHS): {
        ("t", "cross"): (_W8, _R3), ("t", "out"): (_W8, _R3), ("t", "ff2"): (_W8, _R3), ("t", "ff1"): (_PH8, _R2),
        ("f", "cross"): (_W8, _R3), ("f", "out"): (_W8, _R3), ("f", "ff2"): (_W8, _R3), ("f", "ff1"): (_PH8, _R2), ("f", "qkv"): (_PH8, _R2),
        ("a", "x_tfa"): (_NARROW, _R3), ("a", "skip"): (_NARROW, _R3), ("a", "out"): (_NARROW, _R3), ("a", "out2"): (_NARROW, _R3),
        ("a", "ff2"): (_NARROW, _R3), ("a", "qkv"): (L.TILE_128x128, _R2), ("a", "ff1"): (_PH8, _R2),
    },
    ("bf16", 1, SHIPPED_WIDTHS): {},
    ("bf16", 2, SHIPPED_WIDTHS): {},
    ("bf16x3", 0, SHIPPED_WIDTHS): {("a", "qkv"): (_S_PH8, "profiles/r04_bf16x3_qkv_8phase_ab.txt"), ("t", "qkv"): (_S_PH8, "profiles/r04_bf16x3_qkv_8phase_ab.txt"),
                                    ("f", "qkv"): (_S_PH8, _R5), ("f", "ff1"): (_S_PH8, _R5), ("f", "cross"): (_S_FAT, _R5), ("f", "out"): (_S_FAT, _R5),
                                    ("f", "ff2"): (_S_FAT, _R5)},
    ("bf16x3", 2, SHIPPED_WIDTHS): {},
}


def tuned_tiles(mode: str, regime: int, widths) -> dict:
    return {k: v[0] for k, v in TUNED_TILES.get((mode, regime, tuple(widths)), {}).items()}


_STREAMS: dict = {}


def process_streams(dev):
    dev = torch.device(dev)
    key = (dev.type, dev.index if dev.index is not None else torch.cuda.current_device())
    s = _STREAMS.get(key)
    if s is None:
        s = _STREAMS[key] = tuple(torch.cuda.Stream(device=dev) for _ in range(3))
        assert len({x.cuda_stream for x in s}) == 3
    return s


class DiTEngine:

    def __init__(self, cfg: DiTConfig, state_dict: dict, device="cuda", compute: str = "bf16",
                 rope_layout: str = "interleaved", rope_cross: bool = False,
                 zero_masked_queries: bool = True, softclamp: float = 50.0, multi_stream: bool = True):
        assert compute in ("bf16", "fp32", "bf16x3")
        self.split = compute == "bf16x3"
        self.multi_stream = multi_stream
        self.side_tile = 0 if multi_stream else -1
        self.fuse_skip = True
        widths = (cfg.dim, cfg.dim_text, cfg.dim_frames, cfg.ff_mult)
        one_clip = tuned_tiles("bf16", 0, widths)
        self.side_tiles = {k: v for k, v in one_clip.items() if not (k[0] == "a" and v == _NARROW)}
        self.main_tile = _NARROW if any(k[0] == "a" and v == _NARROW for k, v in one_clip.items()) else -1
        self.big_tiles = tuned_tiles("bf16", 2, widths)
        self.split_tiles = tuned_tiles("bf16x3", 0, widths)
        self.split_big_tiles = tuned_tiles("bf16x3", 2, widths)
        self.fold_norm = True
        self.fold_gemm_all = False
        self.fuse_xattn = True
        self.absorb_xattn = os.environ.get("V2A_ABSORB_XATTN", "1") != "0"
        self.cross_on_main = False
        self.interleave_capture = False
        self._fuse_rope = compute != "fp32" and rope_layout == "interleaved"
        assert cfg.dim_head == 64, "kernels are built for dim_head = 64 (x3:717)"
        self.cfg = cfg
        self.dev = torch.device(device)
        self.cd = torch.float32 if compute == "fp32" else torch.bfloat16
        self.cdc = L.F32 if compute == "fp32" else L.BF16
        self.ad = torch.bfloat16 if compute == "bf16" else torch.float32
        self.adc = {"bf16": L.BF16, "fp32": L.F32, "bf16x3": L.BF16_SPLIT}[compute]
        self.rope_layout = {"interleaved": 0, "half": 1}[rope_layout]
        self.rope_cross = rope_cross
        self.zero_masked_queries = zero_masked_queries
        self.softclamp = float(softclamp)
        L.lib()
        self.W = PackedWeights(cfg, state_dict, self.dev, self.cd, self.split)
        self.plans: OrderedDict = OrderedDict()
        self.max_plans = 4
        self.plan = None

    def setup(self, B: int, T: int, nc: int, S: int, cfg_mode: bool = True):
        key = (B, T, nc, S, cfg_mode)
        p = self.plans.get(key)
        if p is not None:
            self.plans.move_to_end(key)
            self.plan = p
            self._alloc_absorbed(p)
            return p
        c, dev, cd = self.cfg, self.dev, self.cd
        R = c.num_registers
        N = T + R
        if T > c.max_seq_len:
            raise ValueError(f"{T} latent frames exceed max_seq_len = {c.max_seq_len} of the position table")
        Bt = 2 * B if cfg_mode else B
        rows = Bt * N
        e = lambda *s, dt=torch.float32: torch.empty(*s, dtype=dt, device=dev)
        p = dict(key=key, B=B, Bt=Bt, T=T, N=N, nc=nc, S=S, rows=rows, cfg_mode=cfg_mode, graphs={})
        D, Dt, Df = c.dim, c.dim_text, c.dim_frames
        w2 = 2 if self.split else 1
        bf = cd == torch.bfloat16

        def stream(d):
            return _Stream(e(Bt, N, d), L.Operand(e(Bt, N, w2 * d, dt=cd), w2 * d, d) if bf else None)

        ld, lo = w2 * 2 * D, 2 * D if self.split else 0
        wide = [e(Bt, N, ld, dt=cd) for _ in range(c.depth // 2)] if bf else []
        p["wide"] = [_Wide(L.Operand(w, ld, 2 * D, lo), L.Operand(w[..., :D], ld, D, lo), L.Operand(w[..., D:2 * D], ld, D, lo)) for w in wide]
        p["skips"] = [_Stream(e(Bt, N, D), p["wide"][j].skip if bf else None) for j in range(c.depth // 2)]
        p["xA"], p["xB"], p["xS"] = stream(D), stream(D), e(Bt, N, D)
        p["tA"], p["tB"], p["t0"], p["tL0"] = stream(Dt), stream(Dt), e(Bt, N, Dt), stream(Dt)
        p["fA"], p["fB"], p["f0"], p["fL0"] = stream(Df), stream(Df), e(Bt, N, Df), stream(Df)
        W0 = self.W.layers[0]
        for s, d, attn, ff in (("a", D, W0["a_attn"], W0["a_ff"]), ("t", Dt, W0["t_attn"], W0["t_ff"]),
                               ("f", Df, W0["f_attn"], W0["f_ff"])):
            p[f"hn_{s}"] = e(rows, w2 * d, dt=cd)
            p[f"ssq_{s}"] = torch.zeros(rows, (d // 32 + 3) // 4 * 4, device=dev)
            p[f"qkv_{s}"] = e(rows, attn.n_pad, dt=self.ad)
            p[f"ao_{s}"] = e(rows, w2 * attn.inner, dt=cd)
            p[f"ffh_{s}"] = e(rows, w2 * ff.inner, dt=cd)
        p["q2"] = e(B * N, W0["a_attn2"].n_pad, dt=self.ad)
        inner = c.heads * c.dim_head
        p["ctx_kv"] = e(B * nc, 2 * c.depth * inner, dt=self.ad)
        p["xattn_kp"] = 0
        self._alloc_absorbed(p)
        p["ctx"] = e(B * nc, w2 * c.ctx_dim, dt=cd)
        p["ctx_len"] = torch.full((B,), nc, dtype=torch.int32, device=dev)
        p["pred"] = e(Bt, N, c.num_channels)
        p["tc"] = e(S, D)
        p["norm_tab"] = e(S, c.depth, 3, D)
        p["gate_tab"] = e(S, c.depth, 3, D)
        p["t_pts"] = e(S)
        p["dt"] = e(S)
        p["step"] = torch.zeros(1, dtype=torch.int32, device=dev)
        p["apg"] = torch.zeros(2 * B, dtype=torch.float64, device=dev)
        p["valid_T"] = torch.full((1,), T, dtype=torch.int32, device=dev)
        p["seq_len"] = torch.full((Bt,), N, dtype=torch.int32, device=dev)
        p["ragged"] = False
        inv = 1.0 / (10000 ** (torch.arange(0, c.dim_head, 2).float() / c.dim_head))
        ang = torch.arange(N + nc).float()[:, None] * inv[None, :]
        p["rope"] = torch.stack((ang.cos(), ang.sin()), -1).contiguous().to(dev)
        p["per_sample_t"] = False
        p["has_cond"] = False
        if c.cond_proj_in:
            p["condbuf"] = torch.zeros(B * N, w2 * self.W.cond_k, dtype=cd, device=dev)
            p["padd"] = e(T, D)
        if self.dev.type == "cuda" and self.multi_stream:
            p["st"], p["sf"], _ = process_streams(self.dev)
        self.plan = p
        self.plans[key] = p
        while len(self.plans) > max(1, self.max_plans):
            self.plans.popitem(last=False)
        return p

    def launch_signature(self):
        p = self.plan
        return (p["ragged"], p["has_cond"], p["per_sample_t"], self.multi_stream, self.side_tile, tuple(sorted(self.side_tiles.items())),
                tuple(sorted(self.big_tiles.items())), tuple(sorted(self.split_tiles.items())), tuple(sorted(self.split_big_tiles.items())), self.main_tile, self.fold_norm, self.fold_gemm_all, self.fuse_skip, self.fuse_xattn, self.cross_on_main,
                self.interleave_capture, self.rope_cross, self.zero_masked_queries, self.absorb_xattn, p["xattn_kp"])

    def _rows(self, t):
        return L.Operand(t, t.stride(-2), t.shape[-1] // (2 if self.split else 1))

    def _mm(self, segs, W, out, shadow=None, **kw):
        if shadow is not None:
            kw.update(out_bf16=shadow.t, ld_out_bf16=shadow.ld)
            if self.split:
                kw.update(out_bf16_split=True, out_bf16_lo_offset=shadow.lo)
        if self.split:
            return L.gemm(segs, W, out, compute=L.BF16, a_split=True, **kw)
        return L.gemm(segs, W, out, compute=self.cdc, **kw)

    def _norm_plain(self, x, hn, rows, d, g):
        L.rmsnorm(x, hn, rows=rows, d=d, gamma=g, split=self.split)

    def _norm_ada(self, x, hn, rows, d, layer, slot):
        p = self.plan
        tab = p["norm_tab"][0, layer, slot]
        ss = p["norm_tab"].stride(0)
        if p["per_sample_t"]:
            L.rmsnorm(x, hn, rows=rows, d=d, gamma=tab, gamma_batch_stride=ss, rows_per_batch=p["N"], split=self.split)
        else:
            L.rmsnorm(x, hn, rows=rows, d=d, gamma=tab, step=p["step"], gamma_step_stride=ss, rows_per_batch=p["N"], split=self.split)

    def _fuse_skip(self):
        return self.fuse_skip and self.cd == torch.bfloat16 and "x_skip" in self.W.layers[-1]

    def _fold(self):
        c = self.cfg
        return (self.fold_norm and self.cd == torch.bfloat16
                and all(d % 32 == 0 and d <= 1280 for d in (c.dim, c.dim_text, c.dim_frames)))

    def _regime(self):
        c = self.cfg
        tiles = -(-self.plan["rows"] // 128) * max(1, c.dim // 128)
        return 0 if tiles <= 140 else (1 if tiles <= 281 else 2)

    def _tuned_dims(self):
        c = self.cfg
        return ("bf16", 0, (c.dim, c.dim_text, c.dim_frames, c.ff_mult)) in TUNED_TILES

    def _fold_gemm(self):
        return self._fold() and (self._regime() < 2 or self.fold_gemm_all)

    def _nprod_ada(self, layer, slot, switch_row=0):
        p, D = self.plan, self.cfg.dim
        ss = p["norm_tab"].stride(0)
        kw = dict(norm_gamma=p["norm_tab"][0, layer, slot], norm_ssq=p["ssq_a"], shadow=self._rows(p["hn_a"]))
        kw["norm_batch_stride" if p["per_sample_t"] else "norm_step_stride"] = ss
        if switch_row:
            kw.update(norm_switch_row=switch_row, norm_switch_offset=D)
        return kw

    def _ncons(self, s, d):
        return dict(row_ssq=self.plan[f"ssq_{s}"], row_norm_dim=d) if self._fold() else {}

    def _gate_kw(self, layer, slot):
        p = self.plan
        tab = p["gate_tab"][0, layer, slot]
        ss = p["gate_tab"].stride(0)
        if p["per_sample_t"]:
            return dict(gate=tab, gate_batch_stride=ss, rows_per_batch=p["N"])
        return dict(gate=tab, step=p["step"], gate_step_stride=ss, rows_per_batch=p["N"])

    def _self_attn(self, A: _Attn, x, s, nseq, d, out_kw, in_kw={}):
        p = self.plan
        N, rows = p["N"], nseq * p["N"]
        hn, qkv, ao = p[f"hn_{s}"], p[f"qkv_{s}"], p[f"ao_{s}"]
        if self._fuse_rope:
            self._mm([self._rows(hn)], A.w_in, qkv, M=rows, N=A.n_pad, bias=A.b_in, ldo=A.n_pad,
                     rope_table=p["rope"], rope_cols=2 * A.inner, rope_pos_offset=0, rows_per_batch=N, **in_kw)
        else:
            self._mm([self._rows(hn)], A.w_in, qkv, M=rows, N=A.n_pad, bias=A.b_in, ldo=A.n_pad, **in_kw)
            L.rope(qkv, rows=rows, row_stride=A.n_pad, nheads=2 * A.heads, rows_per_batch=N, pos_offset=0,
                   table=p["rope"], layout=self.rope_layout)
        es = qkv.element_size()
        base = qkv.data_ptr()
        lens = p["seq_len"] if p["ragged"] else None
        aw = ao.stride(-2)
        L.attention(base, base + A.inner * es, base + 2 * A.inner * es, base + A.gate_col * es, ao.data_ptr(),
                    strides=(A.n_pad, A.n_pad, A.n_pad, A.n_pad, aw,
                             N * A.n_pad, N * A.n_pad, N * A.n_pad, N * A.n_pad, N * aw),
                    B=nseq, H=A.heads, Nq=N, Nk=N, kv_len=lens,
                    q_len=lens if self.zero_masked_queries else None,
                    scale=self.cfg.dim_head ** -0.5, softclamp=self.softclamp, dtype=self.adc, out_split=self.split)
        self._mm([self._rows(ao)], A.w_out, x, M=rows, N=d, resid=x, ldo=d, ldr=d, **out_kw)

    def _ff(self, Fw: _FF, x, s, nseq, d, out_kw, in_kw={}):
        p = self.plan
        rows = nseq * p["N"]
        hn, ffh = p[f"hn_{s}"], p[f"ffh_{s}"]
        self._mm([self._rows(hn)], Fw.w1, ffh, M=rows, N=2 * Fw.inner, epilogue=L.EPI_GEGLU, bias=Fw.b1, ldo=ffh.stride(-2),
                 **(dict(out_split=True) if self.split else {}), **in_kw)
        self._mm([self._rows(ffh)], Fw.w2, x, M=rows, N=d, bias=Fw.b2, resid=x, ldo=d, ldr=d, **out_kw)

    def _tile_hint(self, stream, op):
        r = self._regime()
        if self.split:
            return (self.split_big_tiles if r == 2 else self.split_tiles).get((stream, op), 0)
        side = stream != "a"
        if side and self.side_tile < 0:
            return 0
        if r == 2:
            return self.big_tiles.get((stream, op), -1) + 1
        if r == 1 or not self._tuned_dims():
            return self.side_tile + 1 if side else 0
        narrow = self.main_tile if op in ("x_tfa", "skip", "out", "out2", "ff2") else -1
        return max(self.side_tiles.get((stream, op), self.side_tile if side else narrow), -1) + 1

    def _side_block(self, ly, s, src, dst, nseq, d, parts=(0, 1, 2)):
        p = self.plan
        N, rows = p["N"], nseq * p["N"]
        lens = p["seq_len"] if p["ragged"] else None
        cv = ly[f"{s}_conv"]
        hq, ho, h1, h2 = (self._tile_hint(s, op) for op in ("qkv", "out", "ff1", "ff2"))
        fold, fold2 = self._fold(), self._fold_gemm()
        hn, ssq = p[f"hn_{s}"], p[f"ssq_{s}"]
        nc = self._ncons(s, d)
        cons = dict(tile_hint=hq, **nc)
        cons2 = dict(tile_hint=h1, **(nc if fold2 else {}))
        x = dst.x
        if 0 in parts:
            if fold:
                L.dwconv(src, x, cv.wt, cv.b, B=nseq, N=N, d=d, ksize=cv.k, lens=lens,
                         norm=dict(out_bf16=hn, ld_out_bf16=hn.stride(-2), gamma=ly[f"{s}_g1"], ssq=ssq, split=self.split))
            else:
                L.dwconv(src, x, cv.wt, cv.b, B=nseq, N=N, d=d, ksize=cv.k, lens=lens)
                self._norm_plain(x, hn, rows, d, ly[f"{s}_g1"])
        if 1 in parts:
            prod = dict(shadow=self._rows(hn), norm_gamma=ly[f"{s}_g2"], norm_ssq=ssq) if fold2 else {}
            self._self_attn(ly[f"{s}_attn"], x, s, nseq, d, dict(epilogue=L.EPI_RESID, tile_hint=ho, **prod), cons)
        if 2 in parts:
            if not fold2:
                self._norm_plain(x, hn, rows, d, ly[f"{s}_g2"])
            self._ff(ly[f"{s}_ff"], x, s, nseq, d, dict(epilogue=L.EPI_RESID, tile_hint=h2, shadow=dst.sh), cons2)

    def _absorb(self, B, N, nc):
        c = self.cfg
        A2 = self.W.layers[0]["a_attn2"]
        return (self.absorb_xattn and self.split and not self.rope_cross and 0 < nc <= 32 and (c.heads * L.xattn_kp(nc)) % 64 == 0
                and c.dim % 512 == 0 and c.dim <= 2048 and A2.gate_col == A2.inner and B * -(-N // 64) * A2.heads <= 704)

    def _alloc_absorbed(self, p):
        c = self.cfg
        if p["xattn_kp"] or not self._absorb(p["B"], p["N"], p["nc"]):
            return
        kp = p["xattn_kp"] = L.xattn_kp(p["nc"])
        e = lambda *s: torch.empty(*s, dtype=self.cd, device=self.dev)
        p["wqk"] = e(p["B"], c.depth, c.heads * kp + c.heads, 2 * c.dim)
        p["wvo"] = e(p["B"], c.depth, c.dim, 2 * c.heads * kp)
        p["xp"] = e(p["B"] * p["N"], 2 * c.heads * kp)

    def _audio_cross_attention_absorbed(self, i, ly, x, nctx, cons2, fold2, lens):
        p, c = self.plan, self.cfg
        N, D, H, kp = p["N"], c.dim, c.heads, p["xattn_kp"]
        A2 = ly["a_attn2"]
        r2 = nctx * N
        if not fold2:
            self._norm_ada(x, p["hn_a"], r2, D, i, 1)
        nk = dict(row_ssq=cons2["row_ssq"], row_norm_dim=cons2["row_norm_dim"]) if cons2 else {}
        wqk, wvo, xp = p["wqk"], p["wvo"], p["xp"]
        L.xattn_absorbed(p["hn_a"], p["hn_a"].stride(-2), D, wqk[0, i], xp, ldw=wqk.stride(-2), w_batch_stride=wqk.stride(0), ldo=xp.stride(-2),
                         M=r2, rows_per_batch=N, B=nctx, H=H, KP=kp, kv_len=p["ctx_len"], q_len=lens if self.zero_masked_queries else None,
                         gate_bias=A2.b_in[A2.gate_col:], scale=c.dim_head ** -0.5, softclamp=self.softclamp, **nk)
        xr, hn = x.reshape(-1, D), p["hn_a"]
        for b in range(nctx):
            rows = slice(b * N, (b + 1) * N)
            kw = dict(self._gate_kw(i, 1))
            if fold2:
                kw.update(self._nprod_ada(i, 2))
                kw.update(norm_ssq=p["ssq_a"][rows], shadow=self._rows(hn[rows]))
            if p["per_sample_t"]:
                kw["gate"] = p["gate_tab"][b, i, 1]
                if fold2:
                    kw["norm_gamma"] = p["norm_tab"][b, i, 2]
            self._mm([self._rows(xp[rows])], wvo[b, i], xr[rows], M=N, N=D, resid=xr[rows], ldo=D, ldr=D, epilogue=L.EPI_GATE_RESID,
                     tile_hint=self._tile_hint("a", "out2"), **kw)

    def _audio_cross_attention(self, i, ly, x, nctx, cons2, fold2, lens):
        p, c, W = self.plan, self.cfg, self.W
        N, D = p["N"], c.dim
        if p["xattn_kp"] and self.absorb_xattn:
            return self._audio_cross_attention_absorbed(i, ly, x, nctx, cons2, fold2, lens)
        inner = c.heads * c.dim_head
        nkv = 2 * c.depth * inner
        r2 = nctx * N
        A2 = ly["a_attn2"]
        if not fold2:
            self._norm_ada(x, p["hn_a"], r2, D, i, 1)
        q2 = p["q2"]
        es = q2.element_size()
        kb = p["ctx_kv"].data_ptr() + i * inner * es
        vb = p["ctx_kv"].data_ptr() + (c.depth + i) * inner * es
        aw = p["ao_a"].stride(-2)
        one_launch = (self.fuse_xattn and self.adc in (L.BF16, L.BF16_SPLIT) and nctx * -(-N // 64) * A2.heads <= 704 and p["nc"] <= 64 and D % 512 == 0
                      and A2.gate_col == A2.inner and (self._fuse_rope or not self.rope_cross))
        if one_launch:
            rk = dict(rope_table=p["rope"], rope_cols=A2.inner, rope_pos_offset=0) if self.rope_cross else {}
            nk = dict(row_ssq=cons2["row_ssq"], row_norm_dim=cons2["row_norm_dim"]) if cons2 else {}
            L.qproj_xattn(p["hn_a"], p["hn_a"].stride(-2), D, A2.w_in, bias=A2.b_in, M=r2, N=A2.n_pad, rows_per_batch=N,
                          k=kb, v=vb, out=p["ao_a"].data_ptr(), split=self.split,
                          kv_strides=(nkv, nkv, p["nc"] * nkv, p["nc"] * nkv), out_strides=(aw, N * aw), B=nctx, H=A2.heads, Nk=p["nc"],
                          kv_len=p["ctx_len"], q_len=lens if self.zero_masked_queries else None, scale=c.dim_head ** -0.5,
                          softclamp=self.softclamp, **rk, **nk)
        elif self.rope_cross and self._fuse_rope:
            self._mm([self._rows(p["hn_a"])], A2.w_in, q2, M=r2, N=A2.n_pad, bias=A2.b_in, ldo=A2.n_pad, rope_table=p["rope"],
                     rope_cols=A2.inner, rope_pos_offset=0, rows_per_batch=N, tile_hint=self._tile_hint("a", "q2"), **cons2)
        else:
            self._mm([self._rows(p["hn_a"])], A2.w_in, q2, M=r2, N=A2.n_pad, bias=A2.b_in, ldo=A2.n_pad,
                     tile_hint=self._tile_hint("a", "q2"), **cons2)
            if self.rope_cross:
                L.rope(q2, rows=r2, row_stride=A2.n_pad, nheads=A2.heads, rows_per_batch=N, pos_offset=0,
                       table=p["rope"], layout=self.rope_layout)
        if not one_launch:
            L.attention(q2.data_ptr(), kb, vb, q2.data_ptr() + A2.gate_col * es, p["ao_a"].data_ptr(),
                        strides=(A2.n_pad, nkv, nkv, A2.n_pad, aw,
                                 N * A2.n_pad, p["nc"] * nkv, p["nc"] * nkv, N * A2.n_pad, N * aw),
                        B=nctx, H=A2.heads, Nq=N, Nk=p["nc"], kv_len=p["ctx_len"],
                        q_len=lens if self.zero_masked_queries else None,
                        scale=c.dim_head ** -0.5, softclamp=self.softclamp, dtype=self.adc, out_split=self.split)
        self._mm([self._rows(p["ao_a"])], A2.w_out, x, M=r2, N=D, resid=x, ldo=D, ldr=D, epilogue=L.EPI_GATE_RESID,
                 tile_hint=self._tile_hint("a", "out2"), **self._gate_kw(i, 1), **(self._nprod_ada(i, 2) if fold2 else {}))

    def prepare(self, text, frames_roll, context, context_mask, t_points, *, lens=None,
                drop_text=None, drop_ctx=None, dt=None, step_cond=None, rope_len=None, rope_ctx_len=None):
        p, c, W, dev = self.plan, self.cfg, self.W, self.dev
        B, Bt, T, N, nc, S = p["B"], p["Bt"], p["T"], p["N"], p["nc"], p["S"]
        R, D, Dt, Df = c.num_registers, c.dim, c.dim_text, c.dim_frames
        assert text.shape == (B, T, Dt) and frames_roll.shape == (B, T, c.notes) and context.shape == (B, nc, c.ctx_dim)
        p["valid_T"].fill_(T if rope_len is None else min(T, int(rope_len) - R))
        p["t_pts"].copy_(t_points.to(dev, torch.float32))
        if dt is not None:
            p["dt"].copy_(dt.to(dev, torch.float32))
        p["step"].zero_()
        L.time_cond(p["t_pts"], W.fourier_w, W.time_wt, W.time_b, p["tc"], S=S, d=D)
        nt = c.depth * 3 * D
        L.gemm([(p["tc"], D, D)], W.norm_gamma_w, p["norm_tab"], M=S, N=nt, compute=L.F32, bias=W.norm_gamma_b, ldo=nt)
        L.gemm([(p["tc"], D, D)], W.gate_w, p["gate_tab"], M=S, N=nt, compute=L.F32, epilogue=L.EPI_SIGMOID,
               bias=W.gate_b, ldo=nt)
        if lens is not None and not bool((torch.as_tensor(lens) == T).all()):
            sl = (torch.as_tensor(lens).to(torch.int32) + R).to(dev)
            p["seq_len"].copy_(sl.repeat(Bt // B))
            p["ragged"] = True
        else:
            p["seq_len"].fill_(N)
            p["ragged"] = False
        if drop_text is None:
            drop_text = [False] * B + [True] * (Bt - B)
        if drop_ctx is None:
            drop_ctx = [False] * B
        L.fill_registers(p["t0"], W.text_regs, B=Bt, R=R, d=Dt, out_batch_stride=N * Dt)
        L.fill_registers(p["f0"], W.frames_regs, B=Bt, R=R, d=Df, out_batch_stride=N * Df)
        tx = text.to(dev, torch.float32)
        for s in range(Bt):
            if drop_text[s]:
                p["t0"][s, R:].zero_()
            else:
                p["t0"][s, R:].copy_(tx[s % B])
        fr = frames_roll.to(dev, torch.float32).contiguous()
        L.linear_small(fr, W.pf_wt, W.pf_b, None, p["f0"], M=B * T, K=c.notes, T=T, out_batch_stride=N * Df,
                       row_off=R, d=Df, dup=(B if Bt > B else 0))
        p["has_cond"] = step_cond is not None
        if step_cond is not None:
            assert c.cond_proj_in, "step_cond needs cond_proj_in weights (E2TTS(if_cond_proj_in=True))"
            assert step_cond.shape == (B, T, c.num_channels)
            cb = torch.zeros(B, N, W.cond_k, device=dev)
            cb[:, R:, :c.num_channels] = step_cond.to(dev, torch.float32)
            cb = cb.reshape(B * N, W.cond_k)
            if self.split:
                L.split_bf16(cb, p["condbuf"], rows=B * N, d=W.cond_k)
            else:
                p["condbuf"].copy_(cb)
            p["padd"].copy_(W.pos_emb[:T] + W.cond_b)
        cx = context.to(dev, torch.float32).clone()
        for b in range(B):
            if drop_ctx[b]:
                cx[b] = 0
        if self.split:
            L.split_bf16(cx.reshape(B * nc, -1).contiguous(), p["ctx"], rows=B * nc, d=c.ctx_dim)
        else:
            p["ctx"].copy_(cx.reshape(B * nc, -1))
        cm = context_mask.to(torch.bool).cpu()
        cl = cm.sum(-1).to(torch.int32)
        assert bool((cm == (torch.arange(nc)[None] < cl[:, None])).all()), "context_mask must be a prefix mask"
        p["ctx_len"].copy_(cl)
        inner = c.heads * c.dim_head
        nkv = 2 * c.depth * inner
        self._mm([self._rows(p["ctx"])], W.ctx_kv_w, p["ctx_kv"], M=B * nc, N=nkv, ldo=nkv)
        if self.rope_cross:
            off = (N if rope_len is None else int(rope_len)) - (nc if rope_ctx_len is None else int(rope_ctx_len))
            assert 0 <= off and off + nc <= p["rope"].shape[0], (off, nc, N)
            L.rope(p["ctx_kv"], rows=B * nc, row_stride=nkv, nheads=c.depth * c.heads, rows_per_batch=nc,
                   pos_offset=off, table=p["rope"], layout=self.rope_layout)
        if p["xattn_kp"] and self.absorb_xattn:
            L.xattn_absorb_prepare(p["ctx_kv"], W.xattn_wq, W.xattn_wo, p["wqk"], p["wvo"], B=B, L=c.depth, H=c.heads, D=D, nc=nc,
                                   KP=p["xattn_kp"], k_col=0, v_col=c.depth * inner)
        ly = W.layers[0]
        self._side_block(ly, "t", p["t0"], p["tL0"], Bt, Dt)
        self._side_block(ly, "f", p["f0"], p["fL0"], Bt, Df)

    def embed(self, y):
        p, c, W = self.plan, self.cfg, self.W
        B, Bt, T, N, D = p["B"], p["Bt"], p["T"], p["N"], c.dim
        x = p["xA"]
        L.linear_small(y, W.pin_wt, W.pin_b, p["padd"] if p["has_cond"] else W.pos_emb, x.x, M=B * T, K=c.num_channels, T=T,
                       out_batch_stride=N * D, row_off=c.num_registers, d=D, dup=(B if Bt > B else 0),
                       regs=W.regs, out_bf16=None if self.split or x.sh is None else x.sh.t)
        if self.split:
            L.split_bf16(x.x, x.sh.t, rows=Bt * N, d=D)
        if p["has_cond"]:
            self._mm([self._rows(p["condbuf"])], W.cond_w, x.x, M=B * N, N=D, epilogue=L.EPI_RESID, resid=x.x,
                     ldo=D, ldr=D, shadow=x.sh)

    def forward(self, n_ctx_seqs: int | None = None):
        p, c, W = self.plan, self.cfg, self.W
        B, Bt, N, rows = p["B"], p["Bt"], p["N"], p["rows"]
        D, Dt, Df = c.dim, c.dim_text, c.dim_frames
        nctx = B if n_ctx_seqs is None else n_ctx_seqs
        lens = p["seq_len"] if p["ragged"] else None
        half = c.depth // 2
        fz = self._fuse_skip()
        inner = c.heads * c.dim_head
        nkv = 2 * c.depth * inner
        xc, xo = p["xA"], p["xB"]
        tc_, fc_ = p["tL0"], p["fL0"]
        tbuf, fbuf = [p["tA"], p["tB"]], [p["fA"], p["fB"]]

        main = torch.cuda.current_stream() if self.dev.type == "cuda" else None
        st, sf = (p.get("st"), p.get("sf")) if main is not None else (None, None)
        multi = st is not None

        class _On:
            def __init__(self, s):
                self.s = s
            def __enter__(self):
                if multi:
                    self.ctx = torch.cuda.stream(self.s)
                    self.ctx.__enter__()
            def __exit__(self, *a):
                if multi:
                    self.ctx.__exit__(*a)

        def rec(stream):
            if not multi:
                return None
            e = torch.cuda.Event()
            e.record(stream)
            return e

        def wait(stream, *evs):
            if multi:
                for e in evs:
                    if e is not None:
                        stream.wait_event(e)

        eT = eF = None
        eA = rec(main) if not self.cross_on_main else None
        for i, ly in enumerate(W.layers):
            last = i == c.depth - 1
            wait(main, eT, eF)
            xn = p["skips"][i] if i < half else xo
            ax, at_, af_ = xc.op, tc_.op, fc_.op
            fused = fz and i >= half
            if fused:
                wd = p["wide"][c.depth - 1 - i]
                ax = wd.x
                self._mm([wd.whole, at_, af_], ly["x_skip"], p["xS"], M=rows, N=D, ldo=D, tile_hint=self._tile_hint("a", "x_tfa"))
            else:
                self._mm([ax, at_, af_], ly["x_tfa"], xn.x, M=rows, N=D, epilogue=L.EPI_RESID, resid=xc.x, ldo=D, ldr=D,
                         shadow=xn.sh, tile_hint=self._tile_hint("a", "x_tfa"))
            if not last:
                nxt = W.layers[i + 1]
                on_side = multi and not self.cross_on_main
                hint_t = self._tile_hint("t", "cross") if on_side else 0
                hint = self._tile_hint("f", "cross") if on_side else 0
                def cross_t():
                    self._mm([ax, at_], ly["x_at"], tbuf[0].x, M=rows, N=Dt,
                             epilogue=L.EPI_RESID, resid=tc_.x, ldo=Dt, ldr=Dt, tile_hint=hint_t)
                def cross_f():
                    self._mm([ax, af_], ly["x_af"], fbuf[0].x, M=rows, N=Df,
                             epilogue=L.EPI_RESID, resid=fc_.x, ldo=Df, ldr=Df, tile_hint=hint)
                if self.cross_on_main or not multi:
                    cross_t()
                    cross_f()
                    eX = rec(main)
                else:
                    eX = rec(main)
                    with _On(st):
                        wait(st, eA)
                        cross_t()
                    with _On(sf):
                        wait(sf, eA)
                        cross_f()
            src = xn.x if i < half else p["xS"]
            if i >= half and not fused:
                self._mm([xn.op, p["skips"][c.depth - 1 - i].op], ly["skip"], src, M=rows, N=D, ldo=D, tile_hint=self._tile_hint("a", "skip"))
            cv = ly["a_conv"]
            fold, fold2 = self._fold(), self._fold_gemm()
            cons = self._ncons("a", D)
            cons2 = cons if fold2 else {}
            x = xo.x
            r2 = nctx * N
            prod1 = {}
            if fold:
                ps, ss = p["per_sample_t"], p["norm_tab"].stride(0)
                L.dwconv(src, x, cv.wt, cv.b, B=Bt, N=N, d=D, ksize=cv.k, lens=lens,
                         norm=dict(out_bf16=p["hn_a"], ld_out_bf16=p["hn_a"].stride(-2), gamma=p["norm_tab"][0, i, 0], ssq=p["ssq_a"],
                                   split=self.split, **(dict(batch_stride=ss) if ps else dict(step=p["step"], step_stride=ss))))
            else:
                L.dwconv(src, x, cv.wt, cv.b, B=Bt, N=N, d=D, ksize=cv.k, lens=lens)
                self._norm_ada(x, p["hn_a"], rows, D, i, 0)
            if fold2:
                prod1 = self._nprod_ada(i, 1, switch_row=r2 if r2 < rows else 0) if nctx > 0 else self._nprod_ada(i, 2)
            self._self_attn(ly["a_attn"], x, "a", Bt, D, dict(epilogue=L.EPI_GATE_RESID, tile_hint=self._tile_hint("a", "out"),
                                                            **self._gate_kw(i, 0), **prod1), dict(tile_hint=self._tile_hint("a", "qkv"), **cons))
            if not last and self.interleave_capture:
                for part in (0, 1):
                    with _On(st):
                        if part == 0:
                            wait(st, eX)
                        self._side_block(nxt, "t", tbuf[0].x, tbuf[1], Bt, Dt, (part,))
                    with _On(sf):
                        if part == 0:
                            wait(sf, eX)
                        self._side_block(nxt, "f", fbuf[0].x, fbuf[1], Bt, Df, (part,))
            if nctx > 0:
                self._audio_cross_attention(i, ly, x, nctx, cons2, fold2, lens)
            if not fold2:
                self._norm_ada(x, p["hn_a"], rows, D, i, 2)
            xsh = dict(shadow=p["wide"][c.depth - 2 - i].x if (fz and half <= i + 1 < c.depth) else xo.sh)
            if last and fold2:
                xsh = dict(shadow=self._rows(p["hn_a"]), norm_gamma=W.final_g, norm_ssq=p["ssq_a"])
            self._ff(ly["a_ff"], x, "a", Bt, D, dict(epilogue=L.EPI_GATE_RESID, tile_hint=self._tile_hint("a", "ff2"), **self._gate_kw(i, 2), **xsh),
                     dict(tile_hint=self._tile_hint("a", "ff1"), **cons2))
            if not last:
                if not self.cross_on_main:
                    eA = rec(main)
                rest = (2,) if self.interleave_capture else (0, 1, 2)
                with _On(st):
                    if not self.interleave_capture:
                        wait(st, eX)
                    self._side_block(nxt, "t", tbuf[0].x, tbuf[1], Bt, Dt, rest)
                    eT = rec(st)
                with _On(sf):
                    if not self.interleave_capture:
                        wait(sf, eX)
                    self._side_block(nxt, "f", fbuf[0].x, fbuf[1], Bt, Df, rest)
                    eF = rec(sf)
                tc_, fc_ = tbuf[1], fbuf[1]
            xc, xo = xo, xc
        if self._fold_gemm():
            self._mm([self._rows(p["hn_a"])], W.pred_w, p["pred"], M=rows, N=c.num_channels, bias=W.pred_b, ldo=c.num_channels,
                     **self._ncons("a", D))
        else:
            L.rmsnorm(xc.x, p["hn_a"], rows=rows, d=D, gamma=W.final_g, split=self.split)
            self._mm([self._rows(p["hn_a"])], W.pred_w, p["pred"], M=rows, N=c.num_channels, bias=W.pred_b, ldo=c.num_channels)
        return p["pred"]

    def euler_step(self, y, cfg_strength: float, remove_parallel_component: bool = False, keep_parallel_frac: float = 0.0):
        p, c = self.plan, self.cfg
        self.embed(y)
        self.forward()
        kw = dict(B=p["B"], T=p["T"], C_=c.num_channels, pred_batch_stride=p["N"] * c.num_channels, row_off=c.num_registers)
        apg = None
        if remove_parallel_component:
            L.apg_reduce(p["pred"], p["apg"], valid_rows=p["valid_T"], **kw)
            apg = p["apg"]
        L.cfg_euler(y, p["pred"], cfg_strength=cfg_strength, dt=p["dt"], step=p["step"], apg=apg, keep=keep_parallel_frac, **kw)
        L.step_advance(p["step"])
```

video-to-audio-and-piano-rp_amd/e2tts.py:

```python
from __future__ import annotations

import os
from collections import namedtuple
from pathlib import Path
from typing import Callable

import numpy as np
import torch

from . import _lib as L
from .clip import CLIPImageEncoder
from .dinov2 import DINOv2ImageEncoder
from .dit import DiTConfig, DiTEngine, NOTES, process_streams

IMAGE_ENCODERS = {"clip_vit": CLIPImageEncoder, "dinov2": DINOv2ImageEncoder}

LossBreakdown = namedtuple("LossBreakdown", ["flow", "velocity_consistency", "a", "b"])
E2TTSReturn = namedtuple("E2TTS", ["loss", "cond", "pred_flow", "pred_data", "loss_breakdown"])
_IncompatibleKeys = namedtuple("_IncompatibleKeys", ["missing_keys", "unexpected_keys"])
_V2R_PREFIX = "video2roll_net."


def lens_to_mask(t: torch.Tensor, length: int | None = None) -> torch.Tensor:
    if length is None:
# ... 426 lines not shown
        self._clip = enc
        return enc

    def _encode_video_frames(self, clips) -> list:
        out = [None] * len(clips)
        groups: dict[tuple, list[int]] = {}
        arrs = {}
        for i, c in enumerate(clips):
            if c is None:
                continue
            fr = c[0] if torch.is_tensor(c[0]) else torch.from_numpy(np.ascontiguousarray(c[0]))
            arrs[i] = fr
            groups.setdefault(tuple(fr.shape[1:]), []).append(i)
        for idx in groups.values():
            emb = self._clip(torch.cat([arrs[i] for i in idx], 0)).cpu()
            o = 0
            for i in idx:
                n = arrs[i].shape[0]
                out[i] = (emb[o:o + n], float(clips[i][1]))
                o += n
        return out

    def _get_context(self, prompt, context, context_mask, b, video_drop_prompt=None):
        if context is None:
            if prompt is None:
                raise ValueError("pass `prompt` (with text_encoder_fn) or precomputed `context`/`context_mask`")
            if self.text_encoder_fn is not None:
                context, context_mask = self.text_encoder_fn(list(prompt))
            elif getattr(self, "_t5", None) is not None:
                prompts = list(prompt)
                if video_drop_prompt is not None:
                    prompts = ["the sound of X X" if video_drop_prompt[i] else p for i, p in enumerate(prompts)]
                context, context_mask = self._t5(prompts)
            else:
                raise NotImplementedError("FLAN-T5 encoding is outside the accelerated path (SURVEY 8): supply "
                                          "`context`/`context_mask` or construct with text_encoder_fn=")
        if context_mask is None:
            context_mask = torch.ones(context.shape[:2], dtype=torch.bool)
        assert context.shape[0] == b
        return context, context_mask

    def _clip_conditioning(self, text, video_paths, video_frames, batch: int, n: int):
        cfgm = self.cfg
        if video_paths is not None and self.video_encoder_fn is not None:
            return self.video_encoder_fn(video_paths, n)
        if video_paths is not None:
            from .features import encode_video_cached, feature_cache_path
            encoder_fn = None
            if video_frames is not None:
                if self._clip is None:
                    raise RuntimeError("video_frames needs the CLIP image encoder: call load_image_encoder first")
                if len(video_frames) != len(video_paths):
                    raise ValueError(f"video_frames: {len(video_frames)} entries for {len(video_paths)} video_paths")
                plain = [vp[0] if isinstance(vp, tuple) else vp for vp in video_paths]
                todo = [fr if vp is not None and fr is not None and not os.path.exists(feature_cache_path(vp, self.video_encoder)) else None
                        for vp, fr in zip(plain, video_frames)]
                done = {vp: e for vp, e in zip(plain, self._encode_video_frames(todo)) if e is not None}
                def encoder_fn(vp):
                    if vp not in done:
                        raise FileNotFoundError(f"{feature_cache_path(vp, self.video_encoder)}: no cached CLIP features and no frames for {vp}")
                    return done[vp]
            return encode_video_cached(video_paths, n, dim=cfgm.dim_text, video_encoder=self.video_encoder,
                                       sampling_rate=self.sampling_rate or 24000, frame_size=self.frame_size, encoder_fn=encoder_fn)
        if video_frames is not None:
            if self._clip is None:
                raise RuntimeError("video_frames needs the CLIP image encoder: call load_image_encoder first")
            if len(video_frames) != batch:
                raise ValueError(f"video_frames: {len(video_frames)} entries for a batch of {batch}")
            from .features import resample_clip_features
            rows = []
            for e in self._encode_video_frames(list(video_frames)):
                rows.append(torch.zeros(n, cfgm.dim_text) if e is None else
                            resample_clip_features(e[0], e[1], n, sampling_rate=self.sampling_rate or 24000,
                                                   frame_size=self.frame_size))
            return torch.stack(rows, 0)
        if torch.is_tensor(text) and text.ndim == 3:
            return text
        raise NotImplementedError("pass video_paths (with cached .npz CLIP features), text_embed= (b, n, dim_text) "
                                  "or video_encoder_fn=")

    @torch.no_grad()
    def transformer_with_pred_head(self, x, cond=None, times=None, mask=None, text=None, frames_embed=None,
                                   prompt=None, video_drop_prompt=None, audio_drop_prompt=None,
                                   drop_audio_cond: bool | None = None, drop_text_cond: bool | None = None,
                                   drop_text_prompt: bool | None = None, return_drop_conditions=False,
                                   *, context=None, context_mask=None):
        if cond is not None and not self.cfg.cond_proj_in:
            raise NotImplementedError("cond != None needs cond_proj_in (E2TTS(if_cond_proj_in=True), x3:1365): with the shipped "
                                      "configuration (predict.py:144) the reference has no such layer either (x3:2034)")
        if self.training:
            raise NotImplementedError("training-time random condition dropping is out of scope")
        b, n, _ = x.shape
        dtc, dtp = bool(drop_text_cond), bool(drop_text_prompt)
        eng = self.engine()
        context, context_mask = self._get_context(prompt, context, context_mask, b, video_drop_prompt)
        times = torch.as_tensor(times, dtype=torch.float32)
        if times.ndim == 0:
            times = times.repeat(b)
        eng.setup(b, n, context.shape[1], b, cfg_mode=False)
        p = eng.plan
        p["per_sample_t"] = True
        lens = None if mask is None else _mask_to_lens(mask)
        if frames_embed is None:
            frames_embed = torch.zeros(b, n, self.cfg.notes)
        drop_ctx = [dtp or bool(video_drop_prompt is not None and video_drop_prompt[i]) for i in range(b)]
        step_cond = None
        if cond is not None:
            step_cond = cond.detach().to(torch.float32).clone()
            for i in range(b):
                if bool(drop_audio_cond) or (audio_drop_prompt is not None and audio_drop_prompt[i]):
                    step_cond[i] = 0
        eng.prepare(text, frames_embed, context, context_mask, times, lens=lens,
                    drop_text=[dtc] * b, drop_ctx=drop_ctx, step_cond=step_cond)
        eng.embed(x.to(self._device, torch.float32).contiguous())
        pred = eng.forward(n_ctx_seqs=b)
        out = pred[:, self.cfg.num_registers:, :].to(x.device).clone()
        p["per_sample_t"] = False
        if return_drop_conditions:
            return out, [bool(drop_audio_cond)] * b, dtc, [dtp] * b
        return out

    @torch.no_grad()
    def cfg_transformer_with_pred_head(self, *args, cfg_strength: float = 1.0, remove_parallel_component: bool = True,
                                       keep_parallel_frac: float = 0.0, **kwargs):
        pred = self.transformer_with_pred_head(*args, drop_audio_cond=False, drop_text_cond=False, drop_text_prompt=False, **kwargs)
        if cfg_strength < 1e-5:
            return pred
        null = self.transformer_with_pred_head(*args, drop_audio_cond=True, drop_text_cond=True, drop_text_prompt=True, **kwargs)
        upd = pred - null
        if remove_parallel_component:
            shp = upd.shape
            xd, yd = upd.reshape(shp[0], -1).double(), pred.reshape(shp[0], -1).double()
            unit = torch.nn.functional.normalize(yd, dim=-1)
            par = (xd * unit).sum(-1, keepdim=True) * unit
            upd = ((xd - par) + par * keep_parallel_frac).reshape(shp).to(pred.dtype)
        return pred + upd * cfg_strength

    @torch.no_grad()
    def forward(self, inp, *, text=None, times=None, lens=None, velocity_consistency_model=None, velocity_consistency_delta=1e-3,
                prompt=None, video_drop_prompt=None, audio_drop_prompt=None, val=False, video_paths=None, frames=None, midis=None,
                x0=None, text_embed=None, context=None, context_mask=None, frames_embed=None, video_frames=None):
        if not val:
            raise NotImplementedError("forward(val=False) is the training step (random spans, random condition dropping, gradients): "
                                      "out of scope, only the validation pass val=True is built")
        if velocity_consistency_model is not None:
            raise NotImplementedError("velocity_consistency_model: the velocity consistency loss is a training term (x3:2508-2536)")
        has_cond = not self.audiocond_drop_prob > 1.0
        if has_cond and self.audiocond_snr is not None:
            raise NotImplementedError("audiocond_snr: the reference adds fresh device noise to the audio condition (x3:2115-2125, 2406)")
        self.eval()
        if inp.ndim == 2:
            if self.mel_spec is None:
                raise NotImplementedError("a raw-wave `inp` needs mel_spec_module, which the shipped config does not set "
                                          "(load_audio_encoder sets the Encodec encoder)")
            inp = self.mel_spec(inp).permute(0, 2, 1)
            assert inp.shape[-1] == self.num_channels, (tuple(inp.shape), self.num_channels)
        b, n = inp.shape[:2]
        out_device, dev, C_ = inp.device, self._device, self.num_channels
        if text_embed is None:
            text_embed = self._clip_conditioning(text, video_paths, video_frames, b, n)
        lens = torch.full((b,), n, dtype=torch.long) if lens is None else torch.as_tensor(lens).cpu().long()
        mask = lens_to_mask(lens, n)
        span = val_span_mask(lens, n)
        mask_u8, span_u8 = mask.to(dev, torch.uint8).contiguous(), span.to(dev, torch.uint8).contiguous()
        x1 = inp.detach().to(dev, torch.float32).contiguous()
        if x0 is None:
            x0 = torch.randn(b, n, C_, device=dev, generator=torch.Generator(device=dev).manual_seed(0))
        x0 = x0.to(dev, torch.float32).contiguous()
        assert x0.shape == x1.shape == (b, n, C_), (tuple(x0.shape), tuple(x1.shape))
        if times is None:
            times = torch.rand(b)
        times = torch.as_tensor(times, dtype=torch.float32).cpu()
        times = times.repeat(b) if times.ndim == 0 else times
        assert times.shape == (b,), tuple(times.shape)
        w, flow = torch.empty_like(x1), torch.empty_like(x1)
        cond = torch.empty_like(x1) if has_cond else None
        L.cfm_interp(x0, x1, times.to(dev), span_u8 if has_cond else None, w, flow, cond)
        stats = torch.zeros(8, dtype=torch.float64, device=dev)
        roll = torch.zeros(b, n, self.cfg.notes, device=dev)
        if frames is not None or frames_embed is not None:
            if midis is None:
                raise ValueError("forward: `frames` needs `midis` (bf, n, NOTES), the MIDI ground truth of the same clips")
            if frames_embed is None:
                frames_embed = (self.frames_encoder_fn or self.encode_frames)(frames, n)
            fe = frames_embed.to(dev, torch.float32).contiguous()
            md = midis.to(dev, torch.float32).contiguous()
            bf = fe.shape[0]
            if not (0 < bf <= b and fe.shape == md.shape == (bf, n, self.cfg.notes)):
                raise ValueError(f"forward: roll {tuple(fe.shape)} and midis {tuple(md.shape)}, expected (bf <= {b}, {n}, {self.cfg.notes})")
            L.roll_metrics(fe, md, mask_u8[b - bf:], stats[2:])
            roll[b - bf:] = fe
        pred = self.transformer_with_pred_head(w, cond, times=times, mask=mask, text=text_embed, frames_embed=roll, prompt=prompt,
                                               video_drop_prompt=video_drop_prompt, audio_drop_prompt=audio_drop_prompt,
                                               drop_audio_cond=False, drop_text_cond=False, drop_text_prompt=False,
                                               context=context, context_mask=context_mask)
        L.masked_sqerr(pred, flow, span_u8, stats[:2])
        st = stats.cpu()
        flow_loss = st[0] / st[1]
        roll_loss = st[2] / st[3] if frames_embed is not None else st[2]
        tp, fp, fn, tn = (float(v) for v in st[4:])
        ratio = lambda num, den: num / den if den != 0 else 0.0
        pre, rec, f1, acc = ratio(tp, tp + fp), ratio(tp, tp + fn), ratio(2 * tp, 2 * tp + fp + fn), ratio(tp, tp + fp + fn)
        self.val_stats = dict(flow=float(flow_loss), roll=float(roll_loss), tp=tp, fp=fp, fn=fn, tn=tn)
        f32 = lambda v: torch.as_tensor(v, dtype=torch.float64).to(torch.float32).to(out_device)
        total = f32(flow_loss + 10.0 * roll_loss)
        return E2TTSReturn(total, (cond if has_cond else w).to(out_device), pred.to(out_device), (x0 + pred).to(out_device),
                           LossBreakdown(f32(pre), f32(rec), f32(f1), f32(acc)))

    __call__ = forward

    @torch.no_grad()
    def sample(self, cond, *, text=None, lens=None, duration=None, steps=32, cfg_strength=1.0,
               remove_parallel_component=True, sway_sampling=True, max_duration=4096, vocoder=None,
               return_raw_output=None, save_to_filename=None, prompt=None, video_drop_prompt=None,
               audio_drop_prompt=None, video_paths=None, frames=None, midis=None,
               y0=None, text_embed=None, context=None, context_mask=None, frames_embed=None, trajectory_out=None, video_frames=None,
               piano=False):
        self.eval()
        if cond.ndim == 3 and not (cond.is_floating_point() or cond.is_complex()):
            if self._audio_quantizer is None:
                raise NotImplementedError("an integer `cond` is a prompt of Encodec codes (b, n_q, n) and needs the quantizer: "
                                          "load_audio_quantizer(state_dict)")
            cond = self._audio_quantizer.decode(cond.transpose(0, 1), channels_last=True).to(cond.device)
        if cond.ndim == 2:
            if self.mel_spec is None:
                raise NotImplementedError("raw-wave `cond` needs mel_spec_module, which the shipped config does not set "
                                          "(load_audio_encoder sets the Encodec encoder)")
            cond = self.mel_spec(cond).permute(0, 2, 1)
            assert cond.shape[-1] == self.num_channels, (tuple(cond.shape), self.num_channels)
        batch, cond_seq_len = cond.shape[:2]
        out_device = cond.device
        cfgm = self.cfg
        if frames_embed is None and frames is None and piano and video_frames is not None:
            if len(video_frames) != batch:
                raise ValueError(f"video_frames: {len(video_frames)} entries for a batch of {batch}")
            frames, _ = self.encode_video_frames(video_paths, cond_seq_len, True, video_frames=video_frames)
        if frames_embed is None:
            if frames is None or isinstance(frames, (int, float)):
                frames_embed = torch.zeros(batch, cond_seq_len, cfgm.notes)
            elif self.frames_encoder_fn is not None:
                frames_embed = self.frames_encoder_fn(frames, cond_seq_len)
            elif self._v2r_sd is not None:
                frames_embed = self.encode_frames(frames, cond_seq_len)
            else:
                raise NotImplementedError("`frames` needs the Video2Roll encoder: load a checkpoint holding `video2roll_net.*`, "
                                          "or pass frames_embed= / frames_encoder_fn=")
        if lens is None:
            lens = torch.full((batch,), cond_seq_len, dtype=torch.long)
        lens = torch.as_tensor(lens).cpu().long()
        if text_embed is None:
            text_embed = self._clip_conditioning(text, video_paths, video_frames, batch, cond_seq_len)
        if duration is None:
            duration = lens.clone()
        elif isinstance(duration, int):
            duration = torch.full((batch,), duration, dtype=torch.long)
        duration = torch.maximum(lens, torch.as_tensor(duration).cpu().long()).clamp(max=max_duration)
        assert duration.shape[0] == batch
        n = int(duration.amax())
        if frames_embed.shape[1] < n:
            pad = torch.zeros(batch, n - frames_embed.shape[1], cfgm.notes, dtype=frames_embed.dtype, device=frames_embed.device)
            frames_embed = torch.cat([frames_embed, pad], 1)
        frames_embed = frames_embed[:, :n]
        if text_embed.shape[1] != n:
            raise ValueError(f"text_embed has {text_embed.shape[1]} frames, the longest duration is {n}")
        step_cond = cond_mask = condp = None
        if int(lens[0]) != int(duration[0]):
            if not cfgm.cond_proj_in:
                raise NotImplementedError("lens != duration (audio-prompted infilling) needs cond_proj_in (E2TTS(if_cond_proj_in=True), "
                                          "x3:1365): with the shipped configuration the reference fails at x3:2034 as well")
            if self.audiocond_snr is not None:
                raise NotImplementedError("audiocond_snr: the reference adds fresh device noise to the prompt at every step (x3:2115-2125, 2228)")
            condp = torch.nn.functional.pad(cond.detach().to("cpu", torch.float32)[:, :n], (0, 0, 0, max(0, n - cond_seq_len)))
            cond_mask = lens_to_mask(lens, n)[..., None]
            step_cond = torch.where(cond_mask, condp, torch.zeros_like(condp))
            for i in range(batch):
                if audio_drop_prompt is not None and audio_drop_prompt[i]:
                    step_cond[i] = 0
        elif n != cond_seq_len:
            raise ValueError(f"cond has {cond_seq_len} frames but the longest duration is {n}")
        context, context_mask = self._get_context(prompt, context, context_mask, batch, video_drop_prompt)
        drop_ctx = [bool(video_drop_prompt is not None and video_drop_prompt[i]) for i in range(batch)]
        t = sway_grid(steps, sway_sampling)
        S = steps - 1
        if y0 is None:
            y0 = torch.randn(batch, n, cfgm.num_channels, device=self._device)
        nc = context.shape[1]
        n_plan = -(-n // self.bucket_frames) * self.bucket_frames if self.bucket_frames > 0 else n
        if n_plan > cfgm.max_seq_len:
            n_plan = n
        nc_plan = -(-nc // self.bucket_ctx) * self.bucket_ctx if self.bucket_ctx > 0 else nc
        pad_t = lambda x: x if x is None or x.shape[1] == n_plan else torch.nn.functional.pad(x, (0, 0, 0, n_plan - x.shape[1]))
        if nc_plan != nc:
            context = torch.nn.functional.pad(context, (0, 0, 0, nc_plan - nc))
            context_mask = torch.nn.functional.pad(context_mask.to(torch.bool), (0, nc_plan - nc))
        eng = self.engine()
        eng.setup(batch, n_plan, nc_plan, S, cfg_mode=True)
        p = eng.plan
        if "y" not in p:
            p["y"] = torch.empty(batch, n_plan, cfgm.num_channels, dtype=torch.float32, device=self._device)
        ev = [torch.cuda.Event(enable_timing=True) for _ in range(3)]
        ev[0].record()
        eng.prepare(pad_t(text_embed), pad_t(frames_embed), context, context_mask, t[:-1], lens=duration,
                    drop_ctx=drop_ctx, dt=t[1:] - t[:-1], step_cond=pad_t(step_cond),
                    rope_len=cfgm.num_registers + n, rope_ctx_len=nc)
        ev[1].record()
        self._run_steps(eng, pad_t(y0), S, float(cfg_strength), bool(remove_parallel_component), trajectory_out, n)
        ev[2].record()
        self._phase_events = ev
        out = p["y"][:, :n].to(out_device).clone()
        if step_cond is not None:
            out = torch.where(cond_mask.to(out_device), condp.to(out_device), out)
        if return_raw_output:
            return out
        mask = lens_to_mask(duration)
        if vocoder is not None:
            return vocoder(out.transpose(1, 2))
        if self.vocos is None:
            return out
        audio = [self.vocos.decode(mel[m].transpose(0, 1)[None]).squeeze(0) for mel, m in zip(out, mask)]
        if save_to_filename is not None:
            import torchaudio
            path = Path(save_to_filename)
            path.parents[0].mkdir(exist_ok=True, parents=True)
            for ind, one in enumerate(audio):
                name = path.name if len(audio) == 1 else f"{ind + 1}.{path.name}"
                torchaudio.save(str(path.parents[0] / name), one.detach().cpu()[None], sample_rate=self.sampling_rate)
        return audio

    def phase_ms(self):
        ev = getattr(self, "_phase_events", None)
        if ev is None:
            return None
        ev[2].synchronize()
        return ev[0].elapsed_time(ev[1]), ev[1].elapsed_time(ev[2])

    def _run_steps(self, eng: DiTEngine, y0, S, cfg_strength, apg, traj=None, n_valid=None):
        p = eng.plan
        y = p["y"]
        y.copy_(y0.to(self._device, torch.float32))
        p["step"].zero_()
        if traj is not None:
            traj.append(y[:, :n_valid].clone())
        if not self._use_graph:
            for _ in range(S):
                eng.euler_step(y, cfg_strength, apg)
                if traj is not None:
                    traj.append(y[:, :n_valid].clone())
            return
        key = (cfg_strength, apg, eng.launch_signature())
        g = p["graphs"].get(key)
        if g is None:
            keep = y.clone()
            eng.euler_step(y, cfg_strength, apg)
            torch.cuda.synchronize()
            y.copy_(keep)
            p["step"].zero_()
            g = torch.cuda.CUDAGraph()
            with torch.cuda.graph(g, stream=process_streams(self._device)[2], capture_error_mode="thread_local"):
                eng.euler_step(y, cfg_strength, apg)
            p["graphs"][key] = g
            self.graph_captures += 1
        for _ in range(S):
            g.replay()
            if traj is not None:
                traj.append(y[:, :n_valid].clone())


def _mask_to_lens(mask: torch.Tensor) -> torch.Tensor:
    mask = mask.to(torch.bool).cpu()
    lens = mask.sum(-1)
    if not bool((mask == lens_to_mask(lens, mask.shape[1])).all()):
        raise NotImplementedError("only prefix masks (lens_to_mask form, x3:296-305) are supported")
    return lens
```

Before: 3352 mel-frames/s.

## Fold input embedding into first-layer GEMMs and emit y planes from Euler kernel

```diff
diff --git a/include/v2a_cfm.h b/include/v2a_cfm.h
--- a/include/v2a_cfm.h
+++ b/include/v2a_cfm.h
@@ -200,6 +200,19 @@
                   int64_t pred_batch_stride, int32_t row_off, float cfg_strength,
                   const float* dt, const int32_t* step, const double* apg,
                   float keep_parallel_frac, v2a_stream_t stream);
+typedef struct v2a_y_planes {
+  void* planes;
+  int64_t ld;
+  int64_t lo_offset;
+  int32_t row_off;
+  int32_t rows_per_seq;
+  int32_t copies;
+  int32_t reserved;
+} v2a_y_planes;
+int v2a_cfg_euler_planes(float* y, const float* pred, int32_t B, int32_t T, int32_t C,
+                         int64_t pred_batch_stride, int32_t row_off, float cfg_strength,
+                         const float* dt, const int32_t* step, const double* apg,
+                         float keep_parallel_frac, const v2a_y_planes* planes, v2a_stream_t stream);
 int v2a_split_bf16(const float* x, int64_t ldx, void* y, int64_t ldy, int64_t rows, int32_t d, v2a_stream_t stream);
 int v2a_cast_bf16(const float* x, void* y, int64_t n, v2a_stream_t stream);
 int v2a_step_advance(int32_t* step, v2a_stream_t stream);
diff --git a/video-to-audio-and-piano-rp_amd/_lib.py b/video-to-audio-and-piano-rp_amd/_lib.py
--- a/video-to-audio-and-piano-rp_amd/_lib.py
+++ b/video-to-audio-and-piano-rp_amd/_lib.py
@@ -98,6 +98,11 @@
                 ("row_ssq", C.c_void_p), ("ld_row_ssq", C.c_int64), ("row_ssq_parts", C.c_int32), ("row_norm_dim", C.c_int32)]
 
 
+class YPlanes(C.Structure):
+    _fields_ = [("planes", C.c_void_p), ("ld", C.c_int64), ("lo_offset", C.c_int64), ("row_off", C.c_int32), ("rows_per_seq", C.c_int32),
+                ("copies", C.c_int32), ("reserved", C.c_int32)]
+
+
 class T5AttnArgs(C.Structure):
     _fields_ = [
         ("q", C.c_void_p), ("k", C.c_void_p), ("v", C.c_void_p), ("out", C.c_void_p),
@@ -135,6 +140,7 @@
     "v2a_xattn_absorb_prepare", "v2a_xattn_absorbed",
     "v2a_roll_expand_ratio", "v2a_piano_resize_vt",
     "v2a_roll_notes",
+    "v2a_cfg_euler_planes",
 ]
 
 
@@ -175,6 +181,7 @@
     lib.v2a_time_cond.argtypes = [vp, i32, vp, vp, vp, vp, i32, vp]
     lib.v2a_apg_reduce.argtypes = [vp, vp, i32, i32, i32, i64, i32, vp, vp]
     lib.v2a_cfg_euler.argtypes = [vp, vp, i32, i32, i32, i64, i32, f32, vp, vp, vp, f32, vp]
+    lib.v2a_cfg_euler_planes.argtypes = [vp, vp, i32, i32, i32, i64, i32, f32, vp, vp, vp, f32, C.POINTER(YPlanes), vp]
     lib.v2a_step_advance.argtypes = [vp, vp]
     lib.v2a_cast_bf16.argtypes = [vp, vp, i64, vp]
     lib.v2a_split_bf16.argtypes = [vp, i64, vp, i64, i64, i32, vp]
@@ -564,10 +571,16 @@
     check(lib().v2a_apg_reduce(pred.data_ptr(), apg.data_ptr(), B, T, C_, pred_batch_stride, row_off, _p(valid_rows), stream_ptr()))
 
 
-def cfg_euler(y, pred, *, B, T, C_, pred_batch_stride, row_off, cfg_strength, dt, step=None, apg=None, keep=0.0):
-    _launch("cfg_euler", 0.0, 16.0 * B * T * C_,
-            lambda: lib().v2a_cfg_euler(y.data_ptr(), pred.data_ptr(), B, T, C_, pred_batch_stride, row_off,
-                                        float(cfg_strength), dt.data_ptr(), _p(step), _p(apg), float(keep), stream_ptr()))
+def cfg_euler(y, pred, *, B, T, C_, pred_batch_stride, row_off, cfg_strength, dt, step=None, apg=None, keep=0.0, planes=None):
+    if planes is None:
+        _launch("cfg_euler", 0.0, 16.0 * B * T * C_,
+                lambda: lib().v2a_cfg_euler(y.data_ptr(), pred.data_ptr(), B, T, C_, pred_batch_stride, row_off,
+                                            float(cfg_strength), dt.data_ptr(), _p(step), _p(apg), float(keep), stream_ptr()))
+        return
+    pl = YPlanes(planes["out"].data_ptr(), planes["ld"], planes["lo_offset"], planes["row_off"], planes["rows_per_seq"], planes["copies"], 0)
+    _launch("cfg_euler", 0.0, (16.0 + 4.0 * planes["copies"]) * B * T * C_,
+            lambda: lib().v2a_cfg_euler_planes(y.data_ptr(), pred.data_ptr(), B, T, C_, pred_batch_stride, row_off, float(cfg_strength),
+                                               dt.data_ptr(), _p(step), _p(apg), float(keep), C.byref(pl), stream_ptr()))
 
 
 def step_advance(step):
diff --git a/video-to-audio-and-piano-rp_amd/csrc/rowops.hip b/video-to-audio-and-piano-rp_amd/csrc/rowops.hip
--- a/video-to-audio-and-piano-rp_amd/csrc/rowops.hip
+++ b/video-to-audio-and-piano-rp_amd/csrc/rowops.hip
@@ -508,6 +508,32 @@
   out[(int64_t)s * d + n] = silu_f(acc);
 }
 
+__device__ __forceinline__ f32x4 cfg_euler_update(float* __restrict__ y, const float* __restrict__ pred, int B, int C, int64_t pbs,
+                                                  int row_off, float s, const float* __restrict__ dt, const int32_t* step,
+                                                  const double* apg, float keep, int64_t e, int64_t b, int64_t r) {
+  const float h = dt[step ? step[0] : 0];
+  const f32x4 pc = *reinterpret_cast<const f32x4*>(pred + b * pbs + (int64_t)row_off * C + r);
+  const f32x4 pn = *reinterpret_cast<const f32x4*>(pred + (b + B) * pbs + (int64_t)row_off * C + r);
+  f32x4 yv = *reinterpret_cast<const f32x4*>(y + e);
+  float coef = 0.f;
+  if (apg) {
+    const double dot = apg[2 * b], nn = apg[2 * b + 1];
+    const double nrm = sqrt(nn) > 1e-12 ? sqrt(nn) : 1e-12;
+    coef = (float)(dot / (nrm * nrm));
+  }
+#pragma unroll
+  for (int j = 0; j < 4; ++j) {
+    float upd = pc[j] - pn[j];
+    if (apg) {
+      const float par = coef * pc[j];
+      upd = (upd - par) + par * keep;
+    }
+    yv[j] += h * (pc[j] + upd * s);
+  }
+  *reinterpret_cast<f32x4*>(y + e) = yv;
+  return yv;
+}
+
 __global__ __launch_bounds__(256) void cfg_euler_kernel(float* __restrict__ y, const float* __restrict__ pred, int B,
                                                         int T, int C, int64_t pbs, int row_off, float s,
                                                         const float* __restrict__ dt, const int32_t* step,
@@ -517,27 +543,35 @@
   const int64_t total4 = (int64_t)B * per_b / 4;
   if (idx4 >= total4) return;
   const int64_t e = idx4 * 4;
+  cfg_euler_update(y, pred, B, C, pbs, row_off, s, dt, step, apg, keep, e, e / per_b, e % per_b);
+}
+
+__global__ __launch_bounds__(256) void cfg_euler_planes_kernel(float* __restrict__ y, const float* __restrict__ pred, int B,
+                                                               int T, int C, int64_t pbs, int row_off, float s,
+                                                               const float* __restrict__ dt, const int32_t* step,
+                                                               const double* apg, float keep, bf16_t* __restrict__ planes,
+                                                               int64_t ldp, int64_t lo_off, int plane_row_off, int rows_per_seq, int copies) {
+  const int64_t idx4 = (int64_t)blockIdx.x * blockDim.x + threadIdx.x;
+  const int64_t per_b = (int64_t)T * C;
+  const int64_t total4 = (int64_t)B * per_b / 4;
+  if (idx4 >= total4) return;
+  const int64_t e = idx4 * 4;
   const int64_t b = e / per_b, r = e % per_b;
-  const float h = dt[step ? step[0] : 0];
-  const f32x4 pc = *reinterpret_cast<const f32x4*>(pred + b * pbs + (int64_t)row_off * C + r);
-  const f32x4 pn = *reinterpret_cast<const f32x4*>(pred + (b + B) * pbs + (int64_t)row_off * C + r);
-  f32x4 yv = *reinterpret_cast<const f32x4*>(y + e);
-  float coef = 0.f;
-  if (apg) {
-    const double dot = apg[2 * b], nn = apg[2 * b + 1];
-    const double nrm = sqrt(nn) > 1e-12 ? sqrt(nn) : 1e-12;
-    coef = (float)(dot / (nrm * nrm));
-  }
+  float sv = s;
+  asm volatile("" : "+v"(sv));
+  const f32x4 yv = cfg_euler_update(y, pred, B, C, pbs, row_off, sv, dt, step, apg, keep, e, b, r);
+  bf16x4 hi, lo;
 #pragma unroll
   for (int j = 0; j < 4; ++j) {
-    float upd = pc[j] - pn[j];
-    if (apg) {
-      const float par = coef * pc[j];
-      upd = (upd - par) + par * keep;
-    }
-    yv[j] += h * (pc[j] + upd * s);
-  }
-  *reinterpret_cast<f32x4*>(y + e) = yv;
+    hi[j] = (bf16_t)yv[j];
+    lo[j] = (bf16_t)(yv[j] - (float)hi[j]);
+  }
+  const int64_t t = r / C, c = r % C;
+  for (int k = 0; k < copies; ++k) {
+    bf16_t* row = planes + (((int64_t)k * B + b) * rows_per_seq + plane_row_off + t) * ldp + c;
+    *reinterpret_cast<bf16x4*>(row) = hi;
+    *reinterpret_cast<bf16x4*>(row + lo_off) = lo;
+  }
 }
 
 __global__ __launch_bounds__(256) void apg_reduce_kernel(const float* __restrict__ pred, double* __restrict__ apg, int B,
@@ -806,6 +840,27 @@
   return v2a_check_launch("v2a_cfg_euler");
 }
 
+extern "C" int v2a_cfg_euler_planes(float* y, const float* pred, int32_t B, int32_t T, int32_t C, int64_t pbs, int32_t row_off,
+                                    float cfg_strength, const float* dt, const int32_t* step, const double* apg, float keep,
+                                    const v2a_y_planes* pl, v2a_stream_t stream) {
+  if (!pl || !pl->planes)
+    return v2a_cfg_euler(y, pred, B, T, C, pbs, row_off, cfg_strength, dt, step, apg, keep, stream);
+  V2A_REQUIRE(y && pred && dt, "v2a_cfg_euler_planes: null pointer");
+  V2A_REQUIRE(B > 0 && T > 0 && C > 0 && C % 4 == 0 && pbs % 4 == 0, "v2a_cfg_euler_planes: B=%d T=%d C=%d", B, T, C);
+  V2A_REQUIRE(((uintptr_t)pl->planes & 7) == 0 && pl->ld % 4 == 0 && pl->lo_offset % 4 == 0 && pl->lo_offset >= C &&
+                  pl->ld >= pl->lo_offset + (int64_t)C,
+              "v2a_cfg_euler_planes: planes need 8-byte alignment, lo_offset (%lld) >= C, ld (%lld) >= lo_offset + C, both multiples of 4",
+              (long long)pl->lo_offset, (long long)pl->ld);
+  V2A_REQUIRE(pl->row_off >= 0 && pl->rows_per_seq >= pl->row_off + (int64_t)T && pl->copies >= 1 && pl->copies <= 2,
+              "v2a_cfg_euler_planes: row_off=%d rows_per_seq=%d copies=%d (rows_per_seq >= row_off + T, 1 or 2 copies)", pl->row_off,
+              pl->rows_per_seq, pl->copies);
+  const int64_t total4 = (int64_t)B * T * C / 4;
+  hipLaunchKernelGGL(cfg_euler_planes_kernel, dim3((unsigned)((total4 + 255) / 256)), dim3(256), 0, (hipStream_t)stream, y, pred,
+                     B, T, C, pbs, row_off, cfg_strength, dt, step, apg, keep, (bf16_t*)pl->planes, pl->ld, pl->lo_offset, pl->row_off,
+                     pl->rows_per_seq, pl->copies);
+  return v2a_check_launch("v2a_cfg_euler_planes");
+}
+
 extern "C" int v2a_step_advance(int32_t* step, v2a_stream_t stream) {
   V2A_REQUIRE(step, "v2a_step_advance: null pointer");
   hipLaunchKernelGGL(step_advance_kernel, dim3(1), dim3(1), 0, (hipStream_t)stream, step);
diff --git a/video-to-audio-and-piano-rp_amd/dit.py b/video-to-audio-and-piano-rp_amd/dit.py
--- a/video-to-audio-and-piano-rp_amd/dit.py
+++ b/video-to-audio-and-piano-rp_amd/dit.py
@@ -62,6 +62,27 @@
     if not split:
         return w.float().to(dev, cd).contiguous()
     return L.split_planes(w).contiguous().to(dev)
+
+
+def fold_embed_weights(sd, dim):
+    P = "transformer.layers.0.1.5"
+    w_in = sd["proj_in.weight"].double()
+    tfa, at, af = (sd[f"{P}.{n}.weight"].double()[:, :dim] for n in ("text_frames_to_audio", "audio_to_text", "audio_to_frames"))
+    return w_in + tfa @ w_in, at @ w_in, af @ w_in
+
+
+def y_plane_rows(B, T, N, R, copies=2):
+    seq = torch.arange(copies * B).reshape(copies, B, 1)
+    return seq * N + R + torch.arange(T).reshape(1, 1, T)
+
+
+def same_grid(cached, t_points, dt):
+    if cached is None or t_points.device.type != "cpu" or (dt is not None and dt.device.type != "cpu"):
+        return False
+    ct, cdt = cached
+    if (cdt is None) != (dt is None) or ct.shape != t_points.shape:
+        return False
+    return bool(torch.equal(ct, t_points.to(torch.float32))) and (dt is None or bool(torch.equal(cdt, dt.to(torch.float32))))
 
 
 class _Attn:
@@ -185,6 +206,9 @@
             self.xattn_wo = torch.stack([ly["a_attn2"].wo32 for ly in self.layers]).to(dev).contiguous()
         for ly in self.layers:
             ly["a_attn2"].wk = ly["a_attn2"].wv = ly["a_attn2"].wq32 = ly["a_attn2"].wo32 = None
+        self.fold_g = None
+        if split and c.num_channels % 64 == 0 and c.depth >= 2:
+            self.fold_g = tuple(pk(g.float()) for g in fold_embed_weights(sd, c.dim))
 
 
 SHIPPED_WIDTHS = (1024, 1280, 512, 4)
@@ -246,6 +270,7 @@
         self.fold_gemm_all = False
         self.fuse_xattn = True
         self.absorb_xattn = os.environ.get("V2A_ABSORB_XATTN", "1") != "0"
+        self.fold_embed = os.environ.get("V2A_FOLD_EMBED", "1") != "0"
         self.cross_on_main = False
         self.interleave_capture = False
         self._fuse_rope = compute != "fp32" and rope_layout == "interleaved"
@@ -273,6 +298,7 @@
             self.plans.move_to_end(key)
             self.plan = p
             self._alloc_absorbed(p)
+            self._alloc_folded(p)
             return p
         c, dev, cd = self.cfg, self.dev, self.cd
         R = c.num_registers
@@ -310,6 +336,8 @@
         p["ctx_kv"] = e(B * nc, 2 * c.depth * inner, dt=self.ad)
         p["xattn_kp"] = 0
         self._alloc_absorbed(p)
+        p["armed"], p["c0_ok"], p["grid_host"] = False, False, None
+        self._alloc_folded(p)
         p["ctx"] = e(B * nc, w2 * c.ctx_dim, dt=cd)
         p["ctx_len"] = torch.full((B,), nc, dtype=torch.int32, device=dev)
         p["pred"] = e(Bt, N, c.num_channels)
@@ -343,7 +371,7 @@
         p = self.plan
         return (p["ragged"], p["has_cond"], p["per_sample_t"], self.multi_stream, self.side_tile, tuple(sorted(self.side_tiles.items())),
                 tuple(sorted(self.big_tiles.items())), tuple(sorted(self.split_tiles.items())), tuple(sorted(self.split_big_tiles.items())), self.main_tile, self.fold_norm, self.fold_gemm_all, self.fuse_skip, self.fuse_xattn, self.cross_on_main,
-                self.interleave_capture, self.rope_cross, self.zero_masked_queries, self.absorb_xattn, p["xattn_kp"])
+                self.interleave_capture, self.rope_cross, self.zero_masked_queries, self.absorb_xattn, p["xattn_kp"], self.fold_embed, p["armed"])
 
     def _rows(self, t):
         return L.Operand(t, t.stride(-2), t.shape[-1] // (2 if self.split else 1))
@@ -496,6 +524,20 @@
         p["wqk"] = e(p["B"], c.depth, c.heads * kp + c.heads, 2 * c.dim)
         p["wvo"] = e(p["B"], c.depth, c.dim, 2 * c.heads * kp)
         p["xp"] = e(p["B"] * p["N"], 2 * c.heads * kp)
+
+    def _fold_ok(self, p):
+        return self.fold_embed and self.split and self.W.fold_g is not None and p["cfg_mode"] and not p.get("per_sample_t", False)
+
+    def _alloc_folded(self, p):
+        c = self.cfg
+        if "ybuf" in p or not self._fold_ok(p):
+            return
+        z = lambda *s, dt=torch.float32: torch.zeros(*s, dtype=dt, device=self.dev)
+        C_ = c.num_channels
+        p["ybuf"] = L.Operand(z(p["rows"], 2 * C_, dt=self.cd), 2 * C_, C_)
+        p["y_zero"] = z(p["B"], p["T"], C_)
+        for s, d in (("a", c.dim), ("t", c.dim_text), ("f", c.dim_frames)):
+            p[f"c0_{s}"] = torch.empty(p["Bt"], p["N"], d, dtype=torch.float32, device=self.dev)
 
     def _audio_cross_attention_absorbed(self, i, ly, x, nctx, cons2, fold2, lens):
         p, c = self.plan, self.cfg
@@ -569,21 +611,27 @@
                  tile_hint=self._tile_hint("a", "out2"), **self._gate_kw(i, 1), **(self._nprod_ada(i, 2) if fold2 else {}))
 
     def prepare(self, text, frames_roll, context, context_mask, t_points, *, lens=None,
-                drop_text=None, drop_ctx=None, dt=None, step_cond=None, rope_len=None, rope_ctx_len=None):
+                drop_text=None, drop_ctx=None, dt=None, step_cond=None, rope_len=None, rope_ctx_len=None, fold_embed=False):
         p, c, W, dev = self.plan, self.cfg, self.W, self.dev
         B, Bt, T, N, nc, S = p["B"], p["Bt"], p["T"], p["N"], p["nc"], p["S"]
         R, D, Dt, Df = c.num_registers, c.dim, c.dim_text, c.dim_frames
         assert text.shape == (B, T, Dt) and frames_roll.shape == (B, T, c.notes) and context.shape == (B, nc, c.ctx_dim)
         p["valid_T"].fill_(T if rope_len is None else min(T, int(rope_len) - R))
-        p["t_pts"].copy_(t_points.to(dev, torch.float32))
-        if dt is not None:
-            p["dt"].copy_(dt.to(dev, torch.float32))
+        p["armed"] = p["c0_ok"] = False
+        folding = fold_embed and "ybuf" in p and self._fold_ok(p)
         p["step"].zero_()
-        L.time_cond(p["t_pts"], W.fourier_w, W.time_wt, W.time_b, p["tc"], S=S, d=D)
-        nt = c.depth * 3 * D
-        L.gemm([(p["tc"], D, D)], W.norm_gamma_w, p["norm_tab"], M=S, N=nt, compute=L.F32, bias=W.norm_gamma_b, ldo=nt)
-        L.gemm([(p["tc"], D, D)], W.gate_w, p["gate_tab"], M=S, N=nt, compute=L.F32, epilogue=L.EPI_SIGMOID,
-               bias=W.gate_b, ldo=nt)
+        if not (folding and same_grid(p["grid_host"], t_points, dt)):
+            p["t_pts"].copy_(t_points.to(dev, torch.float32))
+            if dt is not None:
+                p["dt"].copy_(dt.to(dev, torch.float32))
+            L.time_cond(p["t_pts"], W.fourier_w, W.time_wt, W.time_b, p["tc"], S=S, d=D)
+            nt = c.depth * 3 * D
+            L.gemm([(p["tc"], D, D)], W.norm_gamma_w, p["norm_tab"], M=S, N=nt, compute=L.F32, bias=W.norm_gamma_b, ldo=nt)
+            L.gemm([(p["tc"], D, D)], W.gate_w, p["gate_tab"], M=S, N=nt, compute=L.F32, epilogue=L.EPI_SIGMOID,
+                   bias=W.gate_b, ldo=nt)
+        p["grid_host"] = None
+        if folding and t_points.device.type == "cpu" and (dt is None or dt.device.type == "cpu"):
+            p["grid_host"] = (t_points.detach().to(torch.float32).clone(), None if dt is None else dt.detach().to(torch.float32).clone())
         if lens is not None and not bool((torch.as_tensor(lens) == T).all()):
             sl = (torch.as_tensor(lens).to(torch.int32) + R).to(dev)
             p["seq_len"].copy_(sl.repeat(Bt // B))
@@ -644,6 +692,32 @@
         ly = W.layers[0]
         self._side_block(ly, "t", p["t0"], p["tL0"], Bt, Dt)
         self._side_block(ly, "f", p["f0"], p["fL0"], Bt, Df)
+        if folding:
+            self.embed(p["y_zero"])
+            xa, tl, fl = p["xA"], p["tL0"], p["fL0"]
+            rows = p["rows"]
+            ht, hf = self._cross_hints()
+            self._mm([xa.op, tl.op, fl.op], ly["x_tfa"], p["c0_a"], M=rows, N=D, epilogue=L.EPI_RESID, resid=xa.x, ldo=D, ldr=D,
+                     tile_hint=self._tile_hint("a", "x_tfa"))
+            self._mm([xa.op, tl.op], ly["x_at"], p["c0_t"], M=rows, N=Dt, epilogue=L.EPI_RESID, resid=tl.x, ldo=Dt, ldr=Dt, tile_hint=ht)
+            self._mm([xa.op, fl.op], ly["x_af"], p["c0_f"], M=rows, N=Df, epilogue=L.EPI_RESID, resid=fl.x, ldo=Df, ldr=Df, tile_hint=hf)
+            p["c0_ok"] = True
+
+    def begin_steps(self, y0):
+        p, c = self.plan, self.cfg
+        B, T, N, C_ = p["B"], p["T"], p["N"], c.num_channels
+        if "y" not in p:
+            p["y"] = torch.empty(B, T, C_, dtype=torch.float32, device=self.dev)
+        y = p["y"]
+        y.copy_(y0.to(self.dev, torch.float32))
+        p["armed"] = False
+        if p["c0_ok"] and "ybuf" in p and self._fold_ok(p):
+            yb = p["ybuf"]
+            for seq in range(p["Bt"]):
+                r0 = seq * N + c.num_registers
+                L.split_bf16(y[seq % B], yb.t[r0:r0 + T], rows=T, d=C_, ldy=yb.ld)
+            p["armed"] = True
+        return y
 
     def embed(self, y):
         p, c, W = self.plan, self.cfg, self.W
@@ -658,7 +732,11 @@
             self._mm([self._rows(p["condbuf"])], W.cond_w, x.x, M=B * N, N=D, epilogue=L.EPI_RESID, resid=x.x,
                      ldo=D, ldr=D, shadow=x.sh)
 
-    def forward(self, n_ctx_seqs: int | None = None):
+    def _cross_hints(self):
+        on_side = self.dev.type == "cuda" and self.plan.get("st") is not None and not self.cross_on_main
+        return (self._tile_hint("t", "cross"), self._tile_hint("f", "cross")) if on_side else (0, 0)
+
+    def forward(self, n_ctx_seqs: int | None = None, folded: bool = False):
         p, c, W = self.plan, self.cfg, self.W
         B, Bt, N, rows = p["B"], p["Bt"], p["N"], p["rows"]
         D, Dt, Df = c.dim, c.dim_text, c.dim_frames
@@ -708,10 +786,14 @@
             xn = p["skips"][i] if i < half else xo
             ax, at_, af_ = xc.op, tc_.op, fc_.op
             fused = fz and i >= half
+            fold0 = folded and i == 0 and not fused
             if fused:
                 wd = p["wide"][c.depth - 1 - i]
                 ax = wd.x
                 self._mm([wd.whole, at_, af_], ly["x_skip"], p["xS"], M=rows, N=D, ldo=D, tile_hint=self._tile_hint("a", "x_tfa"))
+            elif fold0:
+                self._mm([p["ybuf"]], W.fold_g[0], xn.x, M=rows, N=D, epilogue=L.EPI_RESID, resid=p["c0_a"], ldo=D, ldr=D,
+                         shadow=xn.sh, tile_hint=self._tile_hint("a", "x_tfa"))
             else:
                 self._mm([ax, at_, af_], ly["x_tfa"], xn.x, M=rows, N=D, epilogue=L.EPI_RESID, resid=xc.x, ldo=D, ldr=D,
                          shadow=xn.sh, tile_hint=self._tile_hint("a", "x_tfa"))
@@ -721,9 +803,15 @@
                 hint_t = self._tile_hint("t", "cross") if on_side else 0
                 hint = self._tile_hint("f", "cross") if on_side else 0
                 def cross_t():
+                    if fold0:
+                        return self._mm([p["ybuf"]], W.fold_g[1], tbuf[0].x, M=rows, N=Dt,
+                                        epilogue=L.EPI_RESID, resid=p["c0_t"], ldo=Dt, ldr=Dt, tile_hint=hint_t)
                     self._mm([ax, at_], ly["x_at"], tbuf[0].x, M=rows, N=Dt,
                              epilogue=L.EPI_RESID, resid=tc_.x, ldo=Dt, ldr=Dt, tile_hint=hint_t)
                 def cross_f():
+                    if fold0:
+                        return self._mm([p["ybuf"]], W.fold_g[2], fbuf[0].x, M=rows, N=Df,
+                                        epilogue=L.EPI_RESID, resid=p["c0_f"], ldo=Df, ldr=Df, tile_hint=hint)
                     self._mm([ax, af_], ly["x_af"], fbuf[0].x, M=rows, N=Df,
                              epilogue=L.EPI_RESID, resid=fc_.x, ldo=Df, ldr=Df, tile_hint=hint)
                 if self.cross_on_main or not multi:
@@ -805,12 +893,18 @@
 
     def euler_step(self, y, cfg_strength: float, remove_parallel_component: bool = False, keep_parallel_frac: float = 0.0):
         p, c = self.plan, self.cfg
-        self.embed(y)
-        self.forward()
+        folded = p["armed"] and self._fold_ok(p) and "y" in p and y.data_ptr() == p["y"].data_ptr()
+        if not folded:
+            self.embed(y)
+        self.forward(folded=folded)
         kw = dict(B=p["B"], T=p["T"], C_=c.num_channels, pred_batch_stride=p["N"] * c.num_channels, row_off=c.num_registers)
+        planes = None
+        if folded:
+            yb = p["ybuf"]
+            planes = dict(out=yb.t, ld=yb.ld, lo_offset=yb.k, row_off=c.num_registers, rows_per_seq=p["N"], copies=p["Bt"] // p["B"])
         apg = None
         if remove_parallel_component:
             L.apg_reduce(p["pred"], p["apg"], valid_rows=p["valid_T"], **kw)
             apg = p["apg"]
-        L.cfg_euler(y, p["pred"], cfg_strength=cfg_strength, dt=p["dt"], step=p["step"], apg=apg, keep=keep_parallel_frac, **kw)
+        L.cfg_euler(y, p["pred"], cfg_strength=cfg_strength, dt=p["dt"], step=p["step"], apg=apg, keep=keep_parallel_frac, planes=planes, **kw)
         L.step_advance(p["step"])
diff --git a/video-to-audio-and-piano-rp_amd/e2tts.py b/video-to-audio-and-piano-rp_amd/e2tts.py
--- a/video-to-audio-and-piano-rp_amd/e2tts.py
+++ b/video-to-audio-and-piano-rp_amd/e2tts.py
@@ -752,7 +752,7 @@
         ev[0].record()
         eng.prepare(pad_t(text_embed), pad_t(frames_embed), context, context_mask, t[:-1], lens=duration,
                     drop_ctx=drop_ctx, dt=t[1:] - t[:-1], step_cond=pad_t(step_cond),
-                    rope_len=cfgm.num_registers + n, rope_ctx_len=nc)
+                    rope_len=cfgm.num_registers + n, rope_ctx_len=nc, fold_embed=True)
         ev[1].record()
         self._run_steps(eng, pad_t(y0), S, float(cfg_strength), bool(remove_parallel_component), trajectory_out, n)
         ev[2].record()
@@ -786,8 +786,7 @@
 
     def _run_steps(self, eng: DiTEngine, y0, S, cfg_strength, apg, traj=None, n_valid=None):
         p = eng.plan
-        y = p["y"]
-        y.copy_(y0.to(self._device, torch.float32))
+        y = eng.begin_steps(y0)
         p["step"].zero_()
         if traj is not None:
             traj.append(y[:, :n_valid].clone())
@@ -803,7 +802,7 @@
             keep = y.clone()
             eng.euler_step(y, cfg_strength, apg)
             torch.cuda.synchronize()
-            y.copy_(keep)
+            eng.begin_steps(keep)
             p["step"].zero_()
             g = torch.cuda.CUDAGraph()
             with torch.cuda.graph(g, stream=process_streams(self._device)[2], capture_error_mode="thread_local"):
```

New measurement: 3397 mel-frames/s (median of 6 runs). +1.4%, better.
